# CMU-SAFARI/PyGim

Measured on AMD Instinct MI355X. Metric: SpMM GFLOP/s, Reddit-shaped CSR h=256 fp32, higher is better.
Workload: dtype f32

## Files before the change

### include/pygim_hip.h

```cpp
#ifndef PYGIM_HIP_H
#define PYGIM_HIP_H

#include <stdint.h>

#ifdef __cplusplus
extern "C" {
#endif

typedef enum {
    PYGIM_OK = 0,
    PYGIM_ERR_INVALID = 1,
    PYGIM_ERR_NO_DEVICE = 2,
    PYGIM_ERR_HIP = 3,
    PYGIM_ERR_UNSORTED = 4
} pygim_status;

typedef enum {
    PYGIM_INT8 = 0,
    PYGIM_INT16 = 1,
    PYGIM_INT32 = 2,
    PYGIM_INT64 = 3,
    PYGIM_FLT32 = 4,
    PYGIM_DBL64 = 5
} pygim_dtype;
// ... 3 lines not shown
int pygim_init_ranks(int64_t nr_ranks, int64_t *units_per_rank);
int pygim_init_units(int64_t nr_units, int64_t *units_per_rank, int64_t *nr_ranks_out);
int pygim_release(void);
int64_t pygim_generation(void);
int pygim_group_serial(int64_t handle, int64_t *out);
int pygim_is_initialized(void);
const char *pygim_last_error(void);
int pygim_device_info(char *name, int name_len, int *cu_count, int64_t *hbm_bytes);

int pygim_group_create(int format, int dtype, int n_parts,
                       const int32_t *const *idx0, const int32_t *const *colind,
                       const void *const *values, const int64_t *nrows, const int64_t *ncols,
                       const int64_t *nnz, const int64_t *n_dense, const int64_t *dense_cols,
                       int64_t h_size, int64_t *out_handle);
int pygim_group_free(int64_t handle);
int pygim_group_create_transposed(int format, int dtype, int n_parts,
                                  const int32_t *const *idx0, const int32_t *const *colind,
                                  const void *const *values, const int64_t *nrows, const int64_t *ncols,
                                  const int64_t *nnz, const int64_t *n_dense, const int64_t *dense_cols,
                                  int64_t h_size, int64_t *out_handle);

int pygim_spmm_run_group(int64_t handle, const void *const *B_parts, void *out, void *stream);
int pygim_spmm_run_group_x(int64_t handle, const void *const *B_parts, void *out, int x_unchanged,
                           void *stream);
int pygim_grande_run_group(int64_t handle, const void *const *B_windows, const int64_t *window_ld,
                           void *out, void *stream);
int pygim_spmv_run_group(int64_t handle, const void *const *B_vectors, void *out, void *stream);

int pygim_block_run(int64_t handle, int part, const void *X, int64_t ldx, void *C, int64_t ldc,
                    int64_t width, int accumulate, void *stream);
int pygim_block_run_x(int64_t handle, int part, const void *X, int64_t ldx, void *C, int64_t ldc,
                      int64_t width, int accumulate, int x_unchanged, void *stream);

int pygim_quant_spmm_run(int64_t handle, const float *X, int64_t ldx, float *out, float *scale_out, void *stream);
int pygim_quant_spmm_run_post(int64_t handle, const float *X, int64_t ldx, float *out, float *scale_out,
                              const float *col_mul, const float *col_add, int relu, void *stream);

int pygim_quant_absmax(const float *X, int64_t ldx, int64_t rows, int64_t width, uint32_t *absmax_bits, void *stream);
int pygim_quantize(int dtype, const float *X, int64_t ldx, int64_t rows, int64_t width, const uint32_t *absmax_bits,
                   void *Xq, float *scale_out, void *stream);
int pygim_dequantize(int dtype, const void *Q, int64_t n, const uint32_t *absmax_bits, float *out, void *stream);
int pygim_spmm_run_dequant(int64_t handle, const void *Xq, int64_t ldx, float *out, const uint32_t *absmax_bits, void *stream);

int pygim_sddmm(int dtype, int64_t nrows, const int32_t *rowptr, const int32_t *colind, int64_t nnz, const void *G,
                int64_t ldg, const void *X, int64_t ldx, int64_t h, void *out, void *stream);

int64_t pygim_spmm_values_workspace(int dtype, int64_t nrows, int64_t nnz, int64_t h, int64_t heads);
int pygim_spmm_values(int dtype, int64_t nrows, const int32_t *rowptr, const int32_t *colind, int64_t nnz, const void *values,
                      int64_t heads, const void *X, int64_t ldx, int64_t h, void *out, int64_t ldo, void *workspace,
                      int64_t workspace_bytes, void *stream);
int64_t pygim_edge_softmax_workspace(int dtype, int64_t nrows, int64_t nnz, int64_t heads);
int pygim_edge_softmax(int dtype, int64_t nrows, const int32_t *rowptr, int64_t nnz, const void *scores, int64_t heads, void *out,
                       void *workspace, int64_t workspace_bytes, void *stream);
int pygim_edge_softmax_backward(int dtype, int64_t nrows, const int32_t *rowptr, int64_t nnz, const void *P, const void *dP,
                                int64_t heads, void *out, void *workspace, int64_t workspace_bytes, void *stream);
int64_t pygim_gat_aggregate_workspace(int dtype, int64_t nrows, int64_t nnz, int64_t h, int64_t heads);
int pygim_gat_aggregate(int dtype, int64_t nrows, const int32_t *rowptr, const int32_t *colind, int64_t nnz,
                        const void *a_dst , const void *a_src , int64_t heads,
                        double negative_slope, const void *X, int64_t ldx, int64_t h, void *out, int64_t ldo,
                        void *lse , void *workspace, int64_t workspace_bytes, void *stream);

#define PYGIM_REDUCE_MEAN 1
#define PYGIM_REDUCE_MAX 2
#define PYGIM_REDUCE_MIN 3
int64_t pygim_spmm_reduce_workspace(int dtype, int op, int64_t nrows, int64_t nnz, int64_t h);
int pygim_spmm_reduce(int dtype, int op, int64_t nrows, const int32_t *rowptr, const int32_t *colind, int64_t nnz,
                      const void *values , const void *X, int64_t ldx, int64_t h, void *out, int64_t ldo,
                      int32_t *arg , void *workspace, int64_t workspace_bytes, void *stream);
int pygim_spmm_reduce_backward(int dtype, int64_t ncols, const int32_t *rowptr_t, const int32_t *rows_t, const int32_t *perm,
                               int64_t nnz, const void *values , const void *G, int64_t ldg,
                               const int32_t *arg, int64_t h, void *dX, int64_t ldd, void *stream);

int pygim_group_timers(int64_t handle, double out_ms[5]);
int pygim_group_info(int64_t handle, int64_t out[8]);
int pygim_group_kernel_ms(int64_t handle, double *sum_ms, int64_t *count, int reset);
int pygim_group_kernel_events(int64_t handle, int on);
int pygim_group_plan(int64_t handle, int64_t out[8]);
int pygim_group_lds_plan(int64_t handle, int64_t out[4]);
int pygim_group_lds_code(int64_t handle, int64_t out[4]);
int pygim_group_lds_tiles(int64_t handle, int64_t out[4]);
int pygim_group_lds_runs(int64_t handle, int64_t *out);
int pygim_group_host_windows(int64_t handle, int64_t *windows, int64_t *direct);
int pygim_group_lds_geometry(int64_t handle, int64_t out[8]);
int pygim_group_lds_note(int64_t handle, char *out, int64_t cap);
int64_t pygim_set_tunable(const char *name, int64_t value);

#ifdef __cplusplus
}
#endif
#endif
```

### pygim_amd/_lib.py

```python
import ctypes
import os

_HERE = os.path.dirname(os.path.abspath(__file__))
LIB_PATH = os.environ.get("PYGIM_HIP_LIB", os.path.join(_HERE, "libpygim_hip.so"))

EXPORTS = [
    "pygim_init_ranks", "pygim_init_units", "pygim_release", "pygim_is_initialized", "pygim_last_error",
    "pygim_device_info", "pygim_group_create", "pygim_group_free", "pygim_spmm_run_group",
    "pygim_grande_run_group", "pygim_spmv_run_group", "pygim_block_run", "pygim_group_timers",
    "pygim_group_info", "pygim_set_tunable", "pygim_group_kernel_ms", "pygim_quant_spmm_run",
    "pygim_quant_absmax", "pygim_quantize", "pygim_dequantize", "pygim_spmm_run_group_x", "pygim_block_run_x",
    "pygim_group_kernel_events", "pygim_group_plan", "pygim_spmm_run_dequant",
    "pygim_quant_spmm_run_post", "pygim_generation", "pygim_group_lds_plan", "pygim_group_lds_code", "pygim_group_lds_geometry", "pygim_group_lds_note",
    "pygim_group_lds_tiles", "pygim_group_lds_runs", "pygim_group_serial", "pygim_group_host_windows",
    "pygim_group_create_transposed", "pygim_sddmm",
    "pygim_spmm_values", "pygim_spmm_values_workspace", "pygim_edge_softmax", "pygim_edge_softmax_workspace", "pygim_edge_softmax_backward",
    "pygim_gat_aggregate", "pygim_gat_aggregate_workspace",
    "pygim_spmm_reduce", "pygim_spmm_reduce_workspace", "pygim_spmm_reduce_backward",
]

OK, ERR_INVALID, ERR_NO_DEVICE, ERR_HIP, ERR_UNSORTED = 0, 1, 2, 3, 4
INT8, INT16, INT32, INT64, FLT32, DBL64 = range(6)
CSR, COO = 0, 1
REDUCE_MEAN, REDUCE_MAX, REDUCE_MIN = 1, 2, 3


class PygimError(RuntimeError):
    def __init__(self, code, msg):
        super().__init__(f"pygim_hip error {code}: {msg}")
        self.code = code


_lib = None


def lib():
    global _lib
    if _lib is None:
        if not os.path.exists(LIB_PATH):
            raise ImportError(
                f"{LIB_PATH} not found: build the HIP extension first "
                f"(`make -C pygim_amd/csrc` or `python -c 'import __graft_entry__ as g; g.build()'`). "
                f"This backend has no CPU fallback.")
        import torch

        L = ctypes.CDLL(LIB_PATH)
        c_i64, c_int, vp = ctypes.c_int64, ctypes.c_int, ctypes.c_void_p
        p_i64 = ctypes.POINTER(ctypes.c_int64)
        L.pygim_last_error.restype = ctypes.c_char_p
        L.pygim_init_ranks.argtypes = [c_i64, p_i64]
        L.pygim_init_units.argtypes = [c_i64, p_i64, p_i64]
        L.pygim_device_info.argtypes = [ctypes.c_char_p, c_int, ctypes.POINTER(c_int), p_i64]
        L.pygim_group_create.argtypes = [c_int, c_int, c_int, vp, vp, vp, p_i64, p_i64, p_i64, p_i64, p_i64, c_i64,
                                         p_i64]
        L.pygim_group_create_transposed.argtypes = list(L.pygim_group_create.argtypes)
        L.pygim_sddmm.argtypes = [c_int, c_i64, vp, vp, c_i64, vp, c_i64, vp, c_i64, c_i64, vp, vp]
        L.pygim_spmm_values.argtypes = [c_int, c_i64, vp, vp, c_i64, vp, c_i64, vp, c_i64, c_i64, vp, c_i64, vp, c_i64, vp]
        L.pygim_spmm_values_workspace.argtypes = [c_int, c_i64, c_i64, c_i64, c_i64]
        L.pygim_spmm_values_workspace.restype = c_i64
        L.pygim_edge_softmax.argtypes = [c_int, c_i64, vp, c_i64, vp, c_i64, vp, vp, c_i64, vp]
        L.pygim_edge_softmax_backward.argtypes = [c_int, c_i64, vp, c_i64, vp, vp, c_i64, vp, vp, c_i64, vp]
        L.pygim_edge_softmax_workspace.argtypes = [c_int, c_i64, c_i64, c_i64]
        L.pygim_edge_softmax_workspace.restype = c_i64
        L.pygim_gat_aggregate.argtypes = [c_int, c_i64, vp, vp, c_i64, vp, vp, c_i64, ctypes.c_double, vp, c_i64, c_i64, vp, c_i64, vp, vp, c_i64, vp]
        L.pygim_gat_aggregate_workspace.argtypes = [c_int, c_i64, c_i64, c_i64, c_i64]
        L.pygim_gat_aggregate_workspace.restype = c_i64
        L.pygim_spmm_reduce.argtypes = [c_int, c_int, c_i64, vp, vp, c_i64, vp, vp, c_i64, c_i64, vp, c_i64, vp, vp, c_i64, vp]
        L.pygim_spmm_reduce_workspace.argtypes = [c_int, c_int, c_i64, c_i64, c_i64]
        L.pygim_spmm_reduce_workspace.restype = c_i64
        L.pygim_spmm_reduce_backward.argtypes = [c_int, c_i64, vp, vp, vp, c_i64, vp, vp, c_i64, vp, c_i64, vp, c_i64, vp]
        L.pygim_group_free.argtypes = [c_i64]
        L.pygim_group_serial.argtypes = [c_i64, p_i64]
        L.pygim_spmm_run_group.argtypes = [c_i64, vp, vp, vp]
        L.pygim_spmm_run_group_x.argtypes = [c_i64, vp, vp, c_int, vp]
        L.pygim_grande_run_group.argtypes = [c_i64, vp, p_i64, vp, vp]
        L.pygim_spmv_run_group.argtypes = [c_i64, vp, vp, vp]
        L.pygim_block_run.argtypes = [c_i64, c_int, vp, c_i64, vp, c_i64, c_i64, c_int, vp]
        L.pygim_block_run_x.argtypes = [c_i64, c_int, vp, c_i64, vp, c_i64, c_i64, c_int, c_int, vp]
        L.pygim_group_timers.argtypes = [c_i64, ctypes.POINTER(ctypes.c_double)]
        L.pygim_group_info.argtypes = [c_i64, p_i64]
        L.pygim_group_kernel_ms.argtypes = [c_i64, ctypes.POINTER(ctypes.c_double), p_i64, c_int]
        L.pygim_group_kernel_events.argtypes = [c_i64, c_int]
        L.pygim_group_plan.argtypes = [c_i64, p_i64]
        L.pygim_group_lds_plan.argtypes = [c_i64, p_i64]
        L.pygim_group_lds_code.argtypes = [c_i64, p_i64]
        L.pygim_group_lds_geometry.argtypes = [c_i64, p_i64]
        L.pygim_group_lds_note.argtypes = [c_i64, ctypes.c_char_p, c_i64]
        L.pygim_group_lds_tiles.argtypes = [c_i64, p_i64]
        L.pygim_group_lds_runs.argtypes = [c_i64, p_i64]
        L.pygim_group_host_windows.argtypes = [c_i64, p_i64, p_i64]
        L.pygim_generation.restype = c_i64
        L.pygim_quant_spmm_run.argtypes = [c_i64, vp, c_i64, vp, vp, vp]
        L.pygim_quant_spmm_run_post.argtypes = [c_i64, vp, c_i64, vp, vp, vp, vp, c_int, vp]
        L.pygim_quant_absmax.argtypes = [vp, c_i64, c_i64, c_i64, vp, vp]
        L.pygim_quantize.argtypes = [c_int, vp, c_i64, c_i64, c_i64, vp, vp, vp, vp]
        L.pygim_dequantize.argtypes = [c_int, vp, c_i64, vp, vp, vp]
        L.pygim_spmm_run_dequant.argtypes = [c_i64, vp, c_i64, vp, vp, vp]
        L.pygim_set_tunable.argtypes = [ctypes.c_char_p, c_i64]
        L.pygim_set_tunable.restype = c_i64
        _lib = L
    return _lib


def check(rc):
    if rc != 0:
        raise PygimError(rc, lib().pygim_last_error().decode())


def i64_array(values):
    return (ctypes.c_int64 * len(values))(*[int(v) for v in values])


def ptr_array(ptrs):
    return (ctypes.c_void_p * len(ptrs))(*[ctypes.c_void_p(int(p) if p else None) for p in ptrs])


def _env_tunables():
    for kv in filter(None, os.environ.get("PYGIM_TUNE", "").split(",")):
        name, _, value = kv.partition("=")
        if set_tunable(name.strip(), int(value)) == -1:
            raise ValueError(f"PYGIM_TUNE: unknown tunable {name!r}")


def init_ranks(nr_ranks, want_units=False):
    out = (ctypes.c_int64 * max(int(nr_ranks), 1))()
    check(lib().pygim_init_ranks(int(nr_ranks), out))
    _env_tunables()
    return list(out)[: int(nr_ranks)] if want_units else None


def init_units(nr_units):
    n = max((int(nr_units) + 7) // 8, 1)
    out = (ctypes.c_int64 * n)()
    ranks = ctypes.c_int64(0)
    check(lib().pygim_init_units(int(nr_units), out, ctypes.byref(ranks)))
    return list(out)[: ranks.value]


def release():
    check(lib().pygim_release())


def is_initialized():
    return bool(lib().pygim_is_initialized())


def device_info():
    name = ctypes.create_string_buffer(256)
    cu = ctypes.c_int(0)
    mem = ctypes.c_int64(0)
    check(lib().pygim_device_info(name, 256, ctypes.byref(cu), ctypes.byref(mem)))
    return name.value.decode(), cu.value, mem.value


def group_create(fmt, dtype, idx0_ptrs, col_ptrs, val_ptrs, nrows, ncols, nnz, n_dense, dense_cols, h):
    n = len(col_ptrs)
    handle = ctypes.c_int64(0)
    vals = None if val_ptrs is None else ptr_array(val_ptrs)
    check(lib().pygim_group_create(fmt, dtype, n, ptr_array(idx0_ptrs), ptr_array(col_ptrs), vals, i64_array(nrows),
                                   i64_array(ncols), i64_array(nnz), i64_array(n_dense), i64_array(dense_cols),
                                   int(h), ctypes.byref(handle)))
    return handle.value


def group_create_transposed(fmt, dtype, idx0_ptrs, col_ptrs, val_ptrs, nrows, ncols, nnz, n_dense, dense_cols, h):
    n = len(col_ptrs)
    handle = ctypes.c_int64(0)
    vals = None if val_ptrs is None else ptr_array(val_ptrs)
    check(lib().pygim_group_create_transposed(fmt, dtype, n, ptr_array(idx0_ptrs), ptr_array(col_ptrs), vals, i64_array(nrows),
# ... 71 lines not shown
    check(lib().pygim_spmm_reduce_backward(int(dtype), int(ncols), _vp(rowptr_t_ptr), _vp(rows_t_ptr), _vp(perm_ptr), int(nnz), _vp(val_ptr),
                                           _vp(g_ptr), int(ldg), _vp(arg_ptr), int(h), _vp(dx_ptr), int(ldd), _vp(stream)))


def group_free(handle):
    check(lib().pygim_group_free(int(handle)))


def spmm_run_group(handle, b_ptrs, out_ptr, stream=0, x_unchanged=False):
    check(lib().pygim_spmm_run_group_x(int(handle), ptr_array(b_ptrs), ctypes.c_void_p(out_ptr),
                                       1 if x_unchanged else 0, ctypes.c_void_p(stream or None)))


def grande_run_group(handle, b_ptrs, lds, out_ptr, stream=0):
    check(lib().pygim_grande_run_group(int(handle), ptr_array(b_ptrs), i64_array(lds), ctypes.c_void_p(out_ptr),
                                       ctypes.c_void_p(stream or None)))


def spmv_run_group(handle, b_ptrs, out_ptr, stream=0):
    check(lib().pygim_spmv_run_group(int(handle), ptr_array(b_ptrs), ctypes.c_void_p(out_ptr),
                                     ctypes.c_void_p(stream or None)))


def block_run(handle, part, x_ptr, ldx, c_ptr, ldc, width, accumulate=False, stream=0, x_unchanged=False):
    check(lib().pygim_block_run_x(int(handle), int(part), ctypes.c_void_p(x_ptr), int(ldx), ctypes.c_void_p(c_ptr),
                                  int(ldc), int(width), 1 if accumulate else 0, 1 if x_unchanged else 0,
                                  ctypes.c_void_p(stream or None)))


def group_timers(handle):
    out = (ctypes.c_double * 5)()
    check(lib().pygim_group_timers(int(handle), out))
    return list(out)


def group_kernel_events(handle, on=True):
    check(lib().pygim_group_kernel_events(int(handle), 1 if on else 0))


def group_plan(handle):
    out = (ctypes.c_int64 * 8)()
    check(lib().pygim_group_plan(int(handle), out))
    keys = ["n_panels", "panel_cols", "n_items", "col16", "n_coop_items", "n_segment_tasks", "merged", "has_extra"]
    return dict(zip(keys, [int(v) for v in out]))


def group_lds_plan(handle):
    out = (ctypes.c_int64 * 4)()
    check(lib().pygim_group_lds_plan(int(handle), out))
    return dict(zip(["tiles", "chunk_fills", "tokens", "nnz"], [int(v) for v in out]))


def group_lds_code(handle):
    out = (ctypes.c_int64 * 4)()
    check(lib().pygim_group_lds_code(int(handle), out))
    return dict(zip(["code_bytes", "paired_entries", "active", "device_generated"], [int(v) for v in out[:4]]))


def group_lds_tiles(handle):
    out = (ctypes.c_int64 * 4)()
    check(lib().pygim_group_lds_tiles(int(handle), out))
    return dict(zip(["similarity", "labels", "largest_label_rows", "sweep_locality"], [int(v) for v in out[:4]]))


def group_lds_runs(handle):
    out = ctypes.c_int64(0)
    check(lib().pygim_group_lds_runs(int(handle), ctypes.byref(out)))
    return int(out.value)


def group_host_windows(handle):
    return group_host_call(handle)["windows"]


def group_host_call(handle):
    w, d = ctypes.c_int64(0), ctypes.c_int64(0)
    check(lib().pygim_group_host_windows(int(handle), ctypes.byref(w), ctypes.byref(d)))
    return {"windows": int(w.value), "direct": int(d.value)}


def group_lds_geometry(handle):
    out = (ctypes.c_int64 * 8)()
    check(lib().pygim_group_lds_geometry(int(handle), out))
    return dict(zip(["waves", "acc_per_wave", "chunk_cols", "buffers", "group", "x_sets", "shared_entries", "col_splits"], [int(v) for v in out]))


def group_lds_note(handle):
    buf = ctypes.create_string_buffer(1024)
    check(lib().pygim_group_lds_note(int(handle), buf, 1024))
    return buf.value.decode()


def generation():
    return int(lib().pygim_generation())


def group_serial(handle):
    out = ctypes.c_int64(0)
    check(lib().pygim_group_serial(int(handle), ctypes.byref(out)))
    return int(out.value)


def group_info(handle):
    out = (ctypes.c_int64 * 8)()
    check(lib().pygim_group_info(int(handle), out))
    keys = ["total_rows", "total_cols", "h", "n_parts", "n_long_rows", "all_ones", "n_panels", "n_items"]
    return dict(zip(keys, list(out)))


def set_tunable(name, value):
    return int(lib().pygim_set_tunable(name.encode(), int(value)))


def group_kernel_ms(handle, reset=True):
    ms = ctypes.c_double(0)
    n = ctypes.c_int64(0)
    check(lib().pygim_group_kernel_ms(int(handle), ctypes.byref(ms), ctypes.byref(n), 1 if reset else 0))
    return ms.value, n.value


def quant_absmax(x_ptr, ldx, rows, width, bits_ptr, stream=0):
    check(lib().pygim_quant_absmax(ctypes.c_void_p(x_ptr or None), int(ldx), int(rows), int(width), ctypes.c_void_p(bits_ptr),
                                   ctypes.c_void_p(stream or None)))


def quantize(dtype, x_ptr, ldx, rows, width, bits_ptr, xq_ptr, scale_ptr=0, stream=0):
    check(lib().pygim_quantize(int(dtype), ctypes.c_void_p(x_ptr or None), int(ldx), int(rows), int(width),
                               ctypes.c_void_p(bits_ptr), ctypes.c_void_p(xq_ptr or None), ctypes.c_void_p(scale_ptr or None),
                               ctypes.c_void_p(stream or None)))


def dequantize(dtype, q_ptr, n, bits_ptr, out_ptr, stream=0):
    check(lib().pygim_dequantize(int(dtype), ctypes.c_void_p(q_ptr or None), int(n), ctypes.c_void_p(bits_ptr),
                                 ctypes.c_void_p(out_ptr or None), ctypes.c_void_p(stream or None)))


def spmm_run_dequant(handle, xq_ptr, ldx, out_ptr, bits_ptr, stream=0):
    check(lib().pygim_spmm_run_dequant(int(handle), ctypes.c_void_p(xq_ptr), int(ldx), ctypes.c_void_p(out_ptr),
                                       ctypes.c_void_p(bits_ptr), ctypes.c_void_p(stream or None)))


def quant_spmm_run(handle, x_ptr, ldx, out_ptr, scale_ptr=0, stream=0, col_mul_ptr=0, col_add_ptr=0, relu=False):
    check(lib().pygim_quant_spmm_run_post(int(handle), ctypes.c_void_p(x_ptr), int(ldx), ctypes.c_void_p(out_ptr),
                                          ctypes.c_void_p(scale_ptr or None), ctypes.c_void_p(col_mul_ptr or None),
                                          ctypes.c_void_p(col_add_ptr or None), 1 if relu else 0,
                                          ctypes.c_void_p(stream or None)))
```

### pygim_amd/autotune.py

```python
from __future__ import annotations

import math
from dataclasses import dataclass

RATE_PANEL = 17.0e12
RATE_GATHER_FAR = 4.8e12
RATE_GATHER_MALL = 7.0e12
RATE_STREAM = 5.0e12
XGMI_IN = 7 * 45e9
PANEL_BYTES = 4 << 20
LAUNCH = 6e-6
CUS = 256
LDS_ROWS_MAX = 8 * 228
LDS_NS_PER_COLUMN = 3.43
LDS_NS_PER_ENTRY = 0.26
LDS_NS_PER_ENTRY_HALF = 0.5
LDS_NS_PER_COLUMN_FLOOR = 4.4
LDS_COL_SPLIT = True
LDS_ROW_TAIL = 3
TAIL_S = 30e-6
LDS_MIN_LANES = 5
LDS_MIN_REUSE_NARROW = 0.75
LDS_HALF_SPLIT = True
LDS_MIN_REUSE = 0.75


@dataclass
class Choice:
    row_parts: int
    feat_parts: int
    seconds: float
    product_s: float
    collective_s: float
    panel: bool


def lds_rows_per_tile(nrows, nslices, rmax=LDS_ROWS_MAX, cus=CUS):
    tiles = -(-nrows // rmax)
    wgs = tiles * nslices
    rounds = -(-wgs // cus)
    if rounds > 8:
        return rmax
    if wgs % cus == 0:
        return -(-nrows // tiles)
    tiles2 = rounds * cus // nslices
    if tiles2 <= tiles:
        return rmax
    return min(rmax, max(16, -(-nrows // tiles2)))


def lds_product_seconds(nrows, ncols, nnz, h, es):
    if es != 4 or h < LDS_MIN_LANES or nrows == 0 or nnz == 0:
        return None
    nsl = -(-h // 64)
    pack_s = ncols * h * es * 2 / RATE_STREAM
    cols_x = ncols
    ns_entry = LDS_NS_PER_ENTRY
    if LDS_HALF_SPLIT and h * es <= 128 and ncols >= 4 * 128:
        cols_x = -(-ncols // 2)
        ns_entry = LDS_NS_PER_ENTRY_HALF
    min_reuse = LDS_MIN_REUSE if h * es > 128 else max(LDS_MIN_REUSE, LDS_MIN_REUSE_NARROW * (1.6 if cols_x != ncols else 1.0))
    tall = -(-int(nrows) // LDS_ROWS_MAX)
    split = min(8, CUS // (tall * nsl)) if tall * nsl * 2 <= CUS else 1
    tail_rows = 0
    if LDS_COL_SPLIT and nnz >= (1 << 20):
        for s2 in range(8, split, -1):
            tall_s = CUS // (nsl * s2)
            if not tall_s:
                continue
            covered = tall_s * LDS_ROWS_MAX
            if covered >= nrows:
                break
            if (nrows - covered) * 100 <= nrows * LDS_ROW_TAIL and tall_s * nsl * s2 * 10 >= CUS * 9:
                split, tall, tail_rows = s2, tall_s, nrows - covered
                break
    if LDS_COL_SPLIT and nnz >= (1 << 20) and split > 1:
        if nnz / (tall * cols_x) < min_reuse:
            return None
        tall2 = CUS // (nsl * split)
        if not tail_rows and tall < tall2 <= 2 * tall:
            tall = tall2
        per_wg = max(cols_x / split * LDS_NS_PER_COLUMN + nnz / tall / split * ns_entry, cols_x / split * LDS_NS_PER_COLUMN_FLOOR) * 1e-9
        reduce_s = (split + 1) * nrows * h * es / RATE_STREAM
        return per_wg + reduce_s + pack_s + 2 * LAUNCH + (TAIL_S if tail_rows else 0.0)
    rpt = lds_rows_per_tile(int(nrows), nsl)
    tiles = -(-int(nrows) // rpt)
    if nnz / (tiles * cols_x) < min_reuse:
        return None
    per_wg = max(cols_x * LDS_NS_PER_COLUMN + nnz / tiles * ns_entry, cols_x * LDS_NS_PER_COLUMN_FLOOR) * 1e-9
    rounds = -(-tiles * nsl // CUS)
    return rounds * per_wg + pack_s + LAUNCH


def product_seconds(nrows, ncols, nnz, h, es):
    if nrows == 0 or nnz == 0 or h == 0:
        return 0.0, False
    t_lds = lds_product_seconds(nrows, ncols, nnz, h, es)
    if t_lds is not None:
        return t_lds, True
    row_bytes = h * es
    line_bytes = max(row_bytes, 128) if row_bytes < 128 else row_bytes
    gather = nnz * line_bytes
    npanels = max(1, math.ceil(ncols * 128 / PANEL_BYTES))
    panel = row_bytes >= 64 and (npanels == 1 or nnz / (nrows * npanels) >= 8)
    if panel:
        nsl = math.ceil(row_bytes / 128)
        t = gather / RATE_PANEL + npanels * (2 * nrows * row_bytes) / RATE_STREAM / 8 + nsl * 4 * nnz / RATE_STREAM / 8
        t += npanels * LAUNCH + ncols * row_bytes * 2 / RATE_STREAM
    else:
        x_bytes = ncols * row_bytes
        rate = RATE_GATHER_MALL if x_bytes <= 300e6 else RATE_GATHER_FAR
        t = gather / rate + LAUNCH
    return t, panel


def price(nrows, ncols, nnz, h, es, row_parts, feat_parts):
    hp = math.ceil(h / feat_parts)
    t, panel = product_seconds(math.ceil(nrows / row_parts), ncols, nnz / row_parts, hp, es)
    gpus = row_parts * feat_parts
    coll = 0.0 if gpus == 1 else (nrows * h * es) * (1 - 1 / gpus) / XGMI_IN
    return Choice(row_parts, feat_parts, t + coll, t, coll, panel)


def choose(nrows, ncols, nnz, h, elem_bytes, n_gpus):
    table = []
    for r in range(1, n_gpus + 1):
        if n_gpus % r:
            continue
        f = n_gpus // r
        if f > h:
            continue
        table.append(price(nrows, ncols, nnz, h, elem_bytes, r, f))
    best = min(table, key=lambda c: c.seconds)
    return best, table


def autotune(nrows, ncols, nnz, hidden_size, elem_bytes=4, n_gpus=8):
    best, _ = choose(nrows, ncols, nnz, hidden_size, elem_bytes, n_gpus)
    return [best.row_parts, best.feat_parts, "nnz", "nnz", None]


def autotune_dataset(datadir, dataset, hidden_size, split_set, blnc_set=(0, 2), elem_bytes=4):
    from . import datasets, synth

    assert len(split_set) > 0 and len(blnc_set) > 0
    got = datasets.load_adjacency(datadir, dataset)
    if got is not None:
        nrows, nnz = int(got[2]), int(len(got[1]))
    else:
        nrows, nnz, _ = synth.DATASETS[dataset]
    best = None
    for sp, ds in split_set:
        if sp < 1 or ds < 1 or ds > hidden_size:
            continue
        c = price(nrows, nrows, nnz, hidden_size, elem_bytes, sp, ds)
        if best is None or c.seconds < best.seconds:
            best = c
    if best is None:
        return [None, None, None, None, None]
    return [best.row_parts, best.feat_parts, "nnz", "nnz", None]
```

### pygim_amd/csrc/kernels.hpp

```cpp
#pragma once
#include <hip/hip_runtime.h>
#include <stdint.h>
#include <type_traits>

namespace pygim {

template <typename T> struct AccOf { using type = T; };
template <> struct AccOf<int8_t> { using type = uint32_t; };
template <> struct AccOf<int16_t> { using type = uint32_t; };
template <> struct AccOf<int32_t> { using type = uint32_t; };
template <> struct AccOf<int64_t> { using type = uint64_t; };

template <typename T> __device__ __forceinline__ typename AccOf<T>::type to_acc(T v) {
    using A = typename AccOf<T>::type;
    if constexpr (std::is_floating_point<T>::value) return v;
    else if constexpr (sizeof(T) == 8) return (A)v;
    else return (A)(int32_t)v;
}
template <typename T> __device__ __forceinline__ T from_acc(typename AccOf<T>::type a) {
    if constexpr (std::is_floating_point<T>::value) return a;
    else return (T)a;
}

__device__ __forceinline__ uint32_t rfl(uint32_t v) { return __builtin_amdgcn_readfirstlane(v); }
// ... 721 lines not shown
    const uint32_t f = (uint32_t)(i % w);
    using A = typename AccOf<T>::type;
    A acc = (A)part[r * ldp + f];
    for (uint32_t c = 1; c < splits; c++) acc = (A)(acc + (A)part[((uint64_t)c * nrows + r) * ldp + f]);
    float y = (float)(T)acc * (1.0f * quant_scale(*absmax_bits, log2_range));
    if (post_mul) {
        y = post_mul[f] * y + post_add[f];
        if (post_relu) y = fmaxf(y, 0.0f);
    }
    out[r * ldo + f] = y;
}

template <typename T, bool DEQ>
__global__ void k_lds_reduce_v4(const T *__restrict__ part, uint32_t splits, uint64_t nrows, uint32_t w, uint64_t ldp, void *__restrict__ C, int64_t ldc, int accumulate,
                                const uint32_t *__restrict__ absmax_bits, int log2_range, const float *__restrict__ post_mul, const float *__restrict__ post_add, int post_relu) {
    static_assert(sizeof(T) == 4, "4-byte element types");
    using A = typename AccOf<T>::type;
    const uint32_t w4 = w >> 2;
    const uint64_t i = (uint64_t)blockIdx.x * blockDim.x + threadIdx.x;
    if (i >= nrows * w4) return;
    const uint64_t r = i / w4;
    const uint32_t f = (uint32_t)(i % w4) * 4;
    T v[4];
    load_vec<T, 4>(part + r * ldp + f, v);
    A acc[4];
#pragma unroll
    for (int k = 0; k < 4; k++) acc[k] = to_acc<T>(v[k]);
    for (uint32_t c = 1; c < splits; c++) {
        load_vec<T, 4>(part + ((uint64_t)c * nrows + r) * ldp + f, v);
#pragma unroll
        for (int k = 0; k < 4; k++) acc[k] = (A)(acc[k] + to_acc<T>(v[k]));
    }
    if constexpr (DEQ) {
        const float scale = 1.0f * quant_scale(*absmax_bits, log2_range);
        float y[4];
#pragma unroll
        for (int k = 0; k < 4; k++) {
            y[k] = (float)from_acc<T>(acc[k]) * scale;
            if (post_mul) {
                y[k] = post_mul[f + k] * y[k] + post_add[f + k];
                if (post_relu) y[k] = fmaxf(y[k], 0.0f);
            }
        }
        store_vec<float, 4>((float *)C + r * ldc + f, y);
    } else {
        T *c = (T *)C + r * ldc + f;
        if (accumulate) {
            load_vec<T, 4>(c, v);
#pragma unroll
            for (int k = 0; k < 4; k++) acc[k] = (A)(to_acc<T>(v[k]) + acc[k]);
        }
#pragma unroll
        for (int k = 0; k < 4; k++) v[k] = from_acc<T>(acc[k]);
        store_vec<T, 4>(c, v);
    }
}

template <int MODE>
__global__ void k_lds_reduce16(const int16_t *__restrict__ part, uint32_t splits, uint64_t nrows, uint32_t w, uint64_t ldp, void *__restrict__ C, int64_t ldc, int accumulate,
                               const uint32_t *__restrict__ absmax_bits, int log2_range, const float *__restrict__ post_mul, const float *__restrict__ post_add, int post_relu) {
    const uint64_t i = (uint64_t)blockIdx.x * blockDim.x + threadIdx.x;
    if (i >= nrows * w) return;
    const uint64_t r = i / w;
    const uint32_t f = (uint32_t)(i % w);
    uint32_t acc = (uint32_t)(int32_t)part[r * ldp + f];
    for (uint32_t c = 1; c < splits; c++) acc += (uint32_t)(int32_t)part[((uint64_t)c * nrows + r) * ldp + f];
    if constexpr (MODE == 0) {
        int8_t *c8 = (int8_t *)C + (int64_t)r * ldc + f;
        if (accumulate) acc += (uint32_t)(int32_t)*c8;
        *c8 = (int8_t)acc;
    } else {
        float y = (float)(MODE == 1 ? (int32_t)(int8_t)acc : (int32_t)(int16_t)acc) * (1.0f * quant_scale(*absmax_bits, log2_range));
        if (post_mul) {
            y = post_mul[f] * y + post_add[f];
            if (post_relu) y = fmaxf(y, 0.0f);
        }
        ((float *)C)[(int64_t)r * ldc + f] = y;
    }
}

constexpr uint32_t LDS_TAIL_SEG = 256;
template <typename T>
__global__ __launch_bounds__(512) void k_lds_tail_seg(const uint32_t *__restrict__ segs, uint32_t nseg, const uint32_t *__restrict__ colind, const char *__restrict__ xs,
                                                      uint64_t slice_stride, typename AccOf<T>::type *__restrict__ parked) {
    static_assert(sizeof(T) == 4, "4-byte element types");
    using A = typename AccOf<T>::type;
    __shared__ A partial[8][64];
    const uint32_t seg = blockIdx.x, slice = blockIdx.y;
    const uint32_t wave = threadIdx.x >> 6, lane = threadIdx.x & 63;
    const uint32_t e0 = segs[nseg + seg], e1 = segs[2 * nseg + seg];
    const char *xsl = xs + (uint64_t)slice * slice_stride + lane * 4;
    static_assert(LDS_TAIL_SEG == 256, "32 entries per wave");
    uint32_t cols[32];
#pragma unroll
    for (int k = 0; k < 32; k++) {
        const uint32_t e = e0 + wave + 8u * k;
        cols[k] = e < e1 ? colind[e] : 0xFFFFFFFFu;
    }
    T x[32];
#pragma unroll
    for (int k = 0; k < 32; k++) x[k] = cols[k] != 0xFFFFFFFFu ? *(const T *)(xsl + (uint64_t)cols[k] * 256) : (T)0;
    A acc = 0;
#pragma unroll
    for (int k = 0; k < 32; k++) acc = (A)(acc + to_acc<T>(x[k]));
    partial[wave][lane] = acc;
    __syncthreads();
    if (wave != 0) return;
    A sum = partial[0][lane];
#pragma unroll
    for (int v = 1; v < 8; v++) sum = (A)(sum + partial[v][lane]);
    parked[((uint64_t)seg * gridDim.y + slice) * 64 + lane] = sum;
}
template <typename T, bool DEQ>
__global__ __launch_bounds__(64) void k_lds_tail_fin(const uint32_t *__restrict__ rowseg, uint32_t row0, const typename AccOf<T>::type *__restrict__ parked, uint32_t w_lanes,
                                                     void *__restrict__ C, int64_t ldc_bytes, int accumulate, const uint32_t *__restrict__ absmax_bits, int log2_range,
                                                     const float *__restrict__ post_mul, const float *__restrict__ post_add, int post_relu) {
    using A = typename AccOf<T>::type;
    const uint32_t t = blockIdx.x, slice = blockIdx.y, lane = threadIdx.x;
    const uint32_t f = slice * 64 + lane;
    if (f >= w_lanes) return;
    A sum = 0;
    for (uint32_t s = rowseg[t]; s < rowseg[t + 1]; s++) sum = (A)(sum + parked[((uint64_t)s * gridDim.y + slice) * 64 + lane]);
    const uint64_t row = (uint64_t)row0 + t;
    if constexpr (DEQ) {
        float y = (float)from_acc<T>(sum) * (1.0f * quant_scale(*absmax_bits, log2_range));
        if (post_mul) {
            y = post_mul[f] * y + post_add[f];
            if (post_relu) y = fmaxf(y, 0.0f);
        }
        *(float *)((char *)C + (int64_t)row * ldc_bytes + (size_t)f * 4) = y;
    } else {
        T *c = (T *)((char *)C + (int64_t)row * ldc_bytes + (size_t)f * 4);
        if (accumulate) sum = (A)(to_acc<T>(*c) + sum);
        *c = from_acc<T>(sum);
    }
}

__global__ void k_copy16(const u32x4_t *__restrict__ src, u32x4_t *__restrict__ dst, uint64_t n) {
    const uint64_t i = (uint64_t)blockIdx.x * blockDim.x + threadIdx.x;
    if (i < n) dst[i] = src[i];
}

template <typename T>
__global__ void k_narrow_vals(const T *__restrict__ vals, uint64_t n, typename NarrowOf<T>::type *__restrict__ narrow, int *flag) {
    using NT = typename NarrowOf<T>::type;
    const uint64_t i = (uint64_t)blockIdx.x * blockDim.x + threadIdx.x;
    if (i >= n) return;
    const T v = vals[i];
    const NT q = (NT)v;
    bool same;
    if constexpr (std::is_same<T, double>::value) same = __double_as_longlong((double)q) == __double_as_longlong(v);
    else same = (T)q == v;
    narrow[i] = q;
    if (!same) atomicOr(flag, 1);
}

template <typename T>
__global__ void k_widen_vals(const T *__restrict__ vals, uint64_t n, uint32_t *__restrict__ wide) {
    const uint64_t i = (uint64_t)blockIdx.x * blockDim.x + threadIdx.x;
    if (i < n) wide[i] = (uint32_t)(int32_t)vals[i];
}

template <typename T, int VEC, int LOG_LPR, int AMODE, int HAS_VALS, bool DEQ = false>
__global__ __launch_bounds__(256) void k_csr_panel(const uint32_t *__restrict__ item_row,
                                                   const uint32_t *__restrict__ item_begin,
                                                   const uint32_t *__restrict__ item_len, uint32_t nitems,
                                                   const uint32_t *__restrict__ coop_row,
                                                   const uint32_t *__restrict__ coop_begin,
                                                   const uint32_t *__restrict__ coop_len, uint32_t ncoop,
                                                   uint32_t coop_grid, const uint32_t *__restrict__ colind,
                                                   const T *__restrict__ vals, const T *__restrict__ X,
                                                   int64_t ldx, int64_t slice_stride, T *__restrict__ C,
                                                   int64_t ldc, uint32_t w, uint32_t nslices, int accumulate,
                                                   uint32_t col_base, float *__restrict__ Cf, int64_t ldcf,
                                                   const uint32_t *__restrict__ absmax_bits, int log2_range,
                                                   const float *__restrict__ post_mul, const float *__restrict__ post_add,
                                                   int post_relu) {
    static_assert(LOG_LPR == 3, "lane groups of 8 (one 128-byte line per gathered row slice)");
    if (blockIdx.x < coop_grid)
        panel_sweep<T, VEC, AMODE, HAS_VALS, true, DEQ>(blockIdx.x, coop_row, coop_begin, coop_len, ncoop, colind, vals, X,
                                                        ldx, slice_stride, C, ldc, w, nslices, accumulate, col_base, Cf, ldcf,
                                                        absmax_bits, log2_range, post_mul, post_add, post_relu);
    else
        panel_sweep<T, VEC, AMODE, HAS_VALS, false, DEQ>(blockIdx.x - coop_grid, item_row, item_begin, item_len, nitems,
// ... 675 lines not shown
```

### pygim_amd/csrc/lds_codegen.hpp

```cpp
#pragma once
#include <stdint.h>

#include <algorithm>
#include <stdexcept>
#include <vector>

#include "lds_plan.hpp"

#if defined(__HIPCC__)
#define PYGIM_HD __host__ __device__
#else
#define PYGIM_HD
#endif

namespace pygim {

struct CgParams {
    uint32_t NW = 8, KA = 228, KC = 128, NBUF = 5, RB = 256, RPB = 256, G = 10, NS = 2, XW = 1;
    uint32_t wide = 0, valued = 0;
    uint32_t mulw = 0;
    uint32_t int_inline = 0;
    uint32_t i64_full = 0;
    uint32_t opcode_add = 0x02000000u, addw = 1;
    uint32_t pieces = 4, chunk_bytes = 32768;
    uint32_t nrows = 0, ncols = 0, nchunks = 0, ntiles = 0, nstreams = 0;
    uint32_t S = 1, row_tiles = 0;
    uint32_t col_bits = 1;
    uint32_t half_H = 0;
    uint32_t x0 = 6, acc0 = 28, vbase0 = 1, vbase1 = 2, vbase2 = 3, vl16 = 4, vtouch = 4, vjunk = 5;
    uint32_t s_xs = 80, s_ldsw = 82, s_cb = 84, s_ret = 86, s_pa = 92;
    PYGIM_HD uint32_t vbase(uint32_t blk) const { return blk == 0 ? vbase0 : blk == 1 ? vbase1 : vbase2; }
};

constexpr uint32_t CG_TOUCH_EVERY_DW = 256;

inline CgParams cg_params(const LdsGeometry &geo, uint32_t opcode_add, bool valued, uint32_t nrows, uint32_t ncols, uint32_t gsize = 0, uint32_t nsets = 0,
                          bool int_inline = false, bool i64_full = false, uint32_t half_H = 0) {
    if (geo.NBUF >= 3 && !geo.boundary) throw std::runtime_error("lds codegen: the mid-slot hand-off takes the host encoder");
    CgParams P;
    const bool wide = geo.row_bytes == 512;
    if (geo.row_bytes != 256 && geo.row_bytes != 512) throw std::runtime_error("lds codegen: rows of 256 or 512 bytes");
    if (wide != (opcode_add == LDS_CODE_ADD_F64 || opcode_add == LDS_CODE_ADD_U64)) throw std::runtime_error("lds codegen: 512-byte rows are the 8-byte element types'");
    const LdsCodeRegs R = lds_code_regs(geo.NW, gsize, nsets, wide);
    P.NW = geo.NW; P.KA = geo.KA; P.KC = geo.KC; P.NBUF = geo.NBUF; P.RB = geo.row_bytes; P.RPB = 65536 / geo.row_bytes;
    P.G = R.gsize; P.NS = R.nsets; P.XW = wide ? 2 : 1; P.wide = wide; P.valued = valued;
    if (R.x0 + R.nx() > R.acc0 || R.acc0 + P.KA * P.XW > 256 || P.G > 12 || (P.NS - 1) * P.G > 15 || P.NS > 8)
        throw std::runtime_error("lds codegen: the geometry does not fit the register map");
    if (P.KA > 255) throw std::runtime_error("lds codegen: more than 255 accumulators per wave");
    P.opcode_add = opcode_add;
    P.i64_full = (valued && opcode_add == LDS_CODE_ADD_U64 && i64_full) ? 1 : 0;
    P.int_inline = (valued && (opcode_add == 0x68000000u || opcode_add == LDS_CODE_ADD_U64 || opcode_add == LDS_CODE_PK_ADD_U16) && int_inline && !P.i64_full) ? 1 : 0;
    P.mulw = !valued ? 0 : opcode_add == LDS_CODE_ADD_F64 ? 6 : opcode_add == LDS_CODE_ADD_U64 ? (P.i64_full ? 12 : P.int_inline ? 6 : 8) : ((opcode_add == 0x68000000u || opcode_add == LDS_CODE_PK_ADD_U16) && !int_inline) ? 4 : 2;
    P.addw = (opcode_add == LDS_CODE_PK_ADD_U16 || opcode_add == LDS_CODE_ADD_F64 || opcode_add == LDS_CODE_ADD_U64) ? 2 : 1;
    if (valued && opcode_add == LDS_CODE_ADD_U64) P.addw = 0;
    P.pieces = (geo.KC * geo.row_bytes / 1024) / geo.NW;
    if (P.pieces * geo.NW * 1024 != geo.KC * geo.row_bytes) throw std::runtime_error("lds codegen: a chunk is not a whole number of pieces per wave");
    P.chunk_bytes = geo.KC * geo.row_bytes;
    if ((geo.KC * geo.NBUF + P.RPB - 1) / P.RPB > 3) throw std::runtime_error("lds codegen: the ring is larger than three 64 KiB blocks");
    if (geo.NBUF > 12) throw std::runtime_error("lds codegen: more than 12 ring buffers");
    if ((geo.half_split != 0) != (half_H != 0)) throw std::runtime_error("lds codegen: a half-split plan names its H (and only such a plan does)");
    if (half_H && (valued || wide || half_H % geo.KC || ncols != half_H)) throw std::runtime_error("lds codegen: half-split plans are unit-weight plans of 4-byte types over H = whole chunks of virtual columns");
    P.half_H = half_H;
    P.nrows = nrows; P.ncols = ncols;
    P.nchunks = (ncols + geo.KC - 1) / geo.KC;
    const uint32_t R_rows = geo.rows_per_tile ? std::min(geo.rows_per_tile, geo.NW * geo.KA) : geo.NW * geo.KA;
    P.S = std::max(1u, geo.col_splits);
    P.row_tiles = (nrows + R_rows - 1) / R_rows;
    P.ntiles = P.row_tiles * P.S;
    P.nstreams = P.ntiles * geo.NW;
    if ((uint64_t)nrows * P.S >= (1ull << 32)) throw std::runtime_error("lds codegen: rows x column ranges beyond 32 bits");
    P.col_bits = 1;
    while (P.col_bits < 32 && (1ull << P.col_bits) < (uint64_t)ncols) P.col_bits++;
    uint32_t sb = 1;
    while ((1ull << sb) < (uint64_t)P.nstreams) sb++;
    if (sb + P.col_bits + 8 > 64) throw std::runtime_error("lds codegen: key wider than 64 bits");
    P.x0 = R.x0; P.acc0 = R.acc0; P.vbase0 = R.vbase[0]; P.vbase1 = R.vbase[1]; P.vbase2 = R.vbase[2];
    P.vl16 = R.vl16; P.vtouch = R.vtouch; P.vjunk = R.vjunk;
    P.s_xs = R.s_xs; P.s_ldsw = R.s_ldsw; P.s_cb = R.s_cb; P.s_ret = R.s_ret; P.s_pa = R.s_pa;
    return P;
}
inline uint32_t cg_key_bits(const CgParams &P) {
    uint32_t sb = 1;
    while ((1ull << sb) < (uint64_t)P.nstreams) sb++;
    return sb + P.col_bits + 8;
}

struct CgRows {
    std::vector<uint32_t> rowinfo;
    std::vector<uint32_t> rowmap_rt;
    std::vector<uint32_t> tnnz;
    std::vector<uint32_t> tile_pos;
    std::vector<uint32_t> rowmap;
    std::vector<uint32_t> tile_row0, tile_nnz;
};
inline void cg_deal_rows_a(const uint32_t *rowptr, const LdsGeometry &geo, const CgParams &P, CgRows &out, const uint32_t *rorder = nullptr) {
    auto rid = [&](uint32_t pos) { return rorder ? rorder[pos] : pos; };
    auto rlen = [&](uint32_t pos) { const uint32_t r = rid(pos); return rowptr[r + 1] - rowptr[r]; };
    const uint32_t NW = geo.NW, KA = geo.KA, KAS = geo.ka_stride(), RS = NW * KAS;
    const uint32_t R = geo.rows_per_tile ? std::min(geo.rows_per_tile, NW * KA) : NW * KA;
    const uint32_t nrows = P.nrows, nrt = P.row_tiles;
    out.rowinfo.assign(nrows, 0);
    out.rowmap_rt.assign((size_t)nrt * RS, 0xFFFFFFFFu);
    out.tnnz.assign((size_t)nrt * P.S, 0);
    lds_parallel_for(nrt, 0, [&](uint32_t rt) {
        std::vector<uint32_t> order;
        const uint32_t r0 = rt * R, r1 = std::min(nrows, r0 + R), nr = r1 - r0;
        if (P.S == 1) {
            if (!rorder) out.tnnz[rt] = rowptr[r1] - rowptr[r0];
            else
                for (uint32_t q = r0; q < r1; q++) out.tnnz[rt] += rlen(q);
        }
        order.resize(nr);
        for (uint32_t i = 0; i < nr; i++) order[i] = i;
        std::stable_sort(order.begin(), order.end(), [&](uint32_t a, uint32_t b) { return rlen(r0 + a) > rlen(r0 + b); });
        for (uint32_t i = 0; i < nr; i++) {
            const uint32_t round = i / NW, p = i % NW;
            const uint32_t w = (round & 1) ? NW - 1 - p : p;
            out.rowinfo[rid(r0 + order[i])] = ((rt * NW + w) << 8) | round;
            out.rowmap_rt[((size_t)rt * NW + w) * KAS + round] = rid(r0 + order[i]);
        }
    });
}
inline void cg_deal_rows_b(const LdsGeometry &geo, const CgParams &P, CgRows &out) {
    const uint32_t NW = geo.NW, KAS = geo.ka_stride(), RS = NW * KAS;
    const uint32_t R = geo.rows_per_tile ? std::min(geo.rows_per_tile, NW * geo.KA) : NW * geo.KA;
    const uint32_t ntiles = P.ntiles;
    std::vector<uint32_t> ord(ntiles);
    for (uint32_t t = 0; t < ntiles; t++) ord[t] = t;
    if (!geo.keep_tile_order) std::stable_sort(ord.begin(), ord.end(), [&](uint32_t a, uint32_t b) { return out.tnnz[a] > out.tnnz[b]; });
    out.tile_pos.assign(ntiles, 0);
    for (uint32_t i = 0; i < ntiles; i++) out.tile_pos[ord[i]] = i;
    out.rowmap.assign((size_t)ntiles * RS, 0xFFFFFFFFu);
    out.tile_row0.assign(ntiles, 0);
    out.tile_nnz.assign(ntiles, 0);
    for (uint32_t t = 0; t < ntiles; t++) {
        const uint32_t rt = t / P.S, cs = t % P.S, ti = out.tile_pos[t];
        out.tile_row0[ti] = rt * R;
        out.tile_nnz[ti] = out.tnnz[t];
        for (uint32_t q = 0; q < RS; q++) {
            const uint32_t r = out.rowmap_rt[(size_t)rt * RS + q];
            if (r != 0xFFFFFFFFu) out.rowmap[(size_t)ti * RS + q] = r + cs * P.nrows;
        }
    }
}

// ... 124 lines not shown
    }
    const uint32_t ch = T.chunks[T.choff[s / P.NW] + j];
    const uint64_t target = ((uint64_t)s << (P.col_bits + 8)) | ((uint64_t)ch * P.KC << 8);
    uint64_t lo = 0, hi = T.nnz;
    while (lo < hi) {
        const uint64_t mid = (lo + hi) >> 1;
        if (T.keys[mid] < target) lo = mid + 1;
        else hi = mid;
    }
    T.slot_firstcol[sj] = lo < T.nnz ? T.colx[lo] : T.ncols_total;
}
PYGIM_HD inline void cg_slot_ngroups(const CgParams &P, const CgTables &T, uint32_t sj) {
    const uint32_t m = T.slot_firstcol[sj + 1] - T.slot_firstcol[sj];
    T.slot_ng[sj] = (m + P.G - 1) / P.G;
}
PYGIM_HD inline unsigned long long cg_slot_groups(const CgParams &P, const CgTables &T, uint32_t sj) {
    const uint32_t c0 = T.slot_firstcol[sj], c1 = T.slot_firstcol[sj + 1];
    uint32_t g = T.slot_firstgroup[sj];
    unsigned long long pairs = 0;
    for (uint32_t c = c0; c < c1; c += P.G, g++) {
        const uint32_t ce = c + P.G < c1 ? c + P.G : c1;
        uint32_t nlds = 0;
        for (uint32_t u = 0; c + u < ce; u++) {
            T.col_g[c + u] = (g << 4) | u;
            if (P.wide) { nlds++; continue; }
            if ((u & 1) == 0) {
                const bool paired = c + u + 1 < c1 && (T.col_lrow[c + u + 1] / P.RPB) == (T.col_lrow[c + u] / P.RPB);
                if (paired) {
                    nlds++;
                    pairs += (unsigned long long)(T.col_first[c + u + 2] - T.col_first[c + u]);
                } else {
                    nlds += (c + u + 1 < ce) ? 2 : 1;
                }
            }
        }
        T.g_first[g] = T.col_first[c];
        T.g_nent[g] = T.col_first[ce] - T.col_first[c];
        if (P.half_H) {
            uint32_t n0 = 0;
            for (uint32_t i = T.col_first[c]; i < T.col_first[ce]; i++) n0 += T.vals[i] == 0u;
            T.g_n0[g] = n0;
        }
        T.g_firstcol[g] = c;
        T.g_nlds[g] = (uint8_t)nlds;
        T.g_ncols[g] = (uint8_t)(ce - c);
    }
    return pairs;
}

struct CgEmit {
    uint32_t *out;
    uint64_t n;
    uint32_t since_touch;
    uint64_t vm_touch;
    PYGIM_HD void put(uint32_t a) {
        if (out) out[n] = a;
        n++;
    }
    PYGIM_HD void op(uint32_t a) { put(a); since_touch++; }
    PYGIM_HD void op(uint32_t a, uint32_t b) { put(a); put(b); since_touch += 2; }
    PYGIM_HD void skip(uint32_t dw) { n += dw; since_touch += dw; }
};

PYGIM_HD inline void cg_stream_pass(const CgParams &P, const CgTables &T, uint32_t s, bool write) {
    const uint32_t ti = s / P.NW;
    const uint32_t nch = T.nch[ti];
    const uint32_t *chunk_ids = T.chunks + T.choff[ti];
    const uint32_t sj0 = cg_sbase(P, T, s);
    CgEmit e;
    const uint64_t base_dw = write ? T.start[s] / 4 : 0;
    e.out = write ? T.code + base_dw : nullptr;
    e.n = 0;
    e.since_touch = 0;
    e.vm_touch = 0;
    auto s_add_lit = [&](uint32_t sdst, uint32_t ssrc, uint32_t lit) { e.op(0x80000000u | (sdst << 16) | (0xFFu << 8) | ssrc, lit); };
    auto s_addc0 = [&](uint32_t sdst, uint32_t ssrc) { e.op(0x82000000u | (sdst << 16) | (0x80u << 8) | ssrc); };
    auto touch = [&]() {
        s_add_lit(P.s_cb, P.s_cb, (e.since_touch + 5) * 4);
        s_addc0(P.s_cb + 1, P.s_cb + 1);
        e.op(0xDC508000u, (P.vjunk << 24) | (P.s_cb << 16) | P.vtouch);
        e.since_touch = 0;
        e.vm_touch++;
    };
    auto dma = [&](uint32_t cid, uint32_t buf) {
        s_add_lit(P.s_pa, P.s_xs, cid * P.chunk_bytes);
        s_addc0(P.s_pa + 1, P.s_xs + 1);
        for (uint32_t i = 0; i < P.pieces; i++) {
            if (i % 4 == 0) {
                if (i) {
                    s_add_lit(P.s_pa, P.s_pa, 0x1000);
                    s_addc0(P.s_pa + 1, P.s_pa + 1);
                }
                s_add_lit(124 , P.s_ldsw, buf * P.chunk_bytes + (i / 4) * 0x1000);
                e.op(0xBF800000u);
            }
            e.op(0xDDF48000u | ((i % 4) * 1024), (P.s_pa << 16) | P.vl16);
        }
    };
    uint64_t dma_issued = 0;
    uint64_t landed_mark[16];
    for (int q = 0; q < 16; q++) landed_mark[q] = 0;
    auto vm_now = [&]() { return dma_issued + e.vm_touch; };
    auto dma_chunk = [&](uint32_t j) {
        dma(chunk_ids[j], j % P.NBUF);
        dma_issued += P.pieces;
        landed_mark[j & 15] = vm_now();
    };
    auto wait_landed = [&](uint32_t j) {
        const uint64_t younger = vm_now() - landed_mark[j & 15];
        const uint32_t nn = (uint32_t)(younger < 63 ? younger : 63);
        e.op(0xBF8C0F70u | (nn & 15) | (((nn >> 4) & 3) << 14));
    };
    auto wait_lgkm = [&](uint32_t n) { e.op(0xBF8CC07Fu | ((n < 15u ? n : 15u) << 8)); };
    uint32_t pend_g[10], pend_nlds[10], npend = 0;
    uint32_t gcount = 0;
    auto consume_oldest = [&]() {
        uint32_t younger = 0;
        for (uint32_t q = 1; q < npend; q++) younger += pend_nlds[q];
        wait_lgkm(younger);
        const uint32_t g = pend_g[0];
        if (write) T.g_apos[g] = (uint32_t)(base_dw + e.n);
        e.skip(T.g_nent[g] * (P.mulw + P.addw));
        if (P.half_H) e.skip((T.g_n0[g] > 0 ? 1u : 0u) + (T.g_n0[g] < T.g_nent[g] ? 1u : 0u) + 1u);
        for (uint32_t q = 1; q < npend; q++) {
            pend_g[q - 1] = pend_g[q];
            pend_nlds[q - 1] = pend_nlds[q];
        }
        npend--;
    };
    if (nch) {
        for (uint32_t j = 0; j + 1 < P.NBUF && j < nch; j++) dma_chunk(j);
        wait_landed(0);
        e.op(0xBF8A0000u);
    }
    for (uint32_t j = 0; j < nch; j++) {
        bool dma_due = j + P.NBUF - 1 < nch;
        const uint32_t g0 = T.slot_firstgroup[sj0 + j], g1 = T.slot_firstgroup[sj0 + j + 1];
        for (uint32_t g = g0; g < g1; g++) {
            const uint32_t nlds = T.g_nlds[g];
            if (write) {
                T.g_rpos[g] = (uint32_t)(base_dw + e.n);
                T.g_xset[g] = (uint8_t)(gcount % P.NS);
            }
            e.skip(2 * nlds);
            pend_g[npend] = g;
            pend_nlds[npend] = nlds;
            npend++;
            gcount++;
            if (dma_due) {
                dma_chunk(j + P.NBUF - 1);
                dma_due = false;
            }
            if (npend >= P.NS) consume_oldest();
            if (e.since_touch >= CG_TOUCH_EVERY_DW) touch();
        }
        if (dma_due) dma_chunk(j + P.NBUF - 1);
        while (npend > 1) consume_oldest();
        wait_lgkm(0);
        if (j + 1 < nch) wait_landed(j + 1);
        e.op(0xBF8A0000u);
    }
    while (npend) consume_oldest();
    e.op(0xBF8C0F70u);
    e.op(0xBE801D00u | P.s_ret);
    while (e.n % 64) e.put(0xBF800000u);
    if (!write) T.stream_dw[s] = (uint32_t)e.n;
}

PYGIM_HD inline void cg_emit_reads(const CgParams &P, const CgTables &T, uint32_t g) {
    if (P.half_H) {
        uint32_t *a = T.code + T.g_apos[g];
        const uint32_t n0 = T.g_n0[g], n1 = T.g_nent[g] - n0;
        uint32_t at = 0;
        if (n0) { a[at] = 0xBEFE0100u | 76u; at += 1 + n0 * P.addw; }
        if (n1) { a[at] = 0xBEFE0100u | 78u; at += 1 + n1 * P.addw; }
        a[at] = 0xBEFE01C1u;
    }
    const uint32_t c0 = T.g_firstcol[g], nc = T.g_ncols[g];
    const uint32_t xb = P.x0 + P.G * P.XW * T.g_xset[g];
    uint32_t *w = T.code + T.g_rpos[g];
    for (uint32_t u = 0; u < nc;) {
        const uint32_t r0 = T.col_lrow[c0 + u], blk = r0 / P.RPB;
        if (P.wide) {
            *w++ = 0xD8EC0000u | ((r0 % P.RPB) * P.RB);
            *w++ = ((xb + u * 2) << 24) | P.vbase(blk);
            u++;
        } else if ((u & 1) == 0 && u + 1 < nc && (T.col_lrow[c0 + u + 1] / P.RPB) == blk) {
            const uint32_t r1 = T.col_lrow[c0 + u + 1];
// ... 196 lines not shown
```

### pygim_amd/csrc/lds_plan.hpp

```cpp
#pragma once
#include <stdint.h>
#if defined(__HIPCC__)
#define PYGIM_LDS_HD_INLINE __host__ __device__ inline
#else
#define PYGIM_LDS_HD_INLINE inline
#endif

#include <algorithm>
#include <atomic>
#include <cstdio>
#include <cstdlib>
#include <memory>
#include <stdexcept>
#include <thread>
#include <vector>

namespace pygim {

struct LdsTile {
    uint32_t nch;
    uint32_t chunk_off;
    uint32_t nb_off;
    uint32_t row0;
    uint32_t nnz;
    uint32_t chunk0;
    uint32_t pad[2];
    uint32_t tokstart[16];
};

constexpr uint32_t LDS_TOK_SLACK = 4096 + 64;

constexpr uint32_t LDS_HDR_SHIFT = 18, LDS_HDR_MAX = 0x3FFFu;

struct LdsGeometry {
    uint32_t NW = 8;
    uint32_t KA = 208;
    uint32_t KC = 320;
    uint32_t BATCH = 16;
    uint32_t rows_per_tile = 0;
    uint32_t keep_tile_order = 0;
    uint32_t col_splits = 1;
    uint32_t ka_stride() const { return (KA + 7) & ~7u; }
    uint32_t row_bytes = 256;
    uint32_t boundary = 0;
    uint32_t half_split = 0;
    uint32_t NBUF = 2;
};

struct LdsPlanHost {
    LdsGeometry geo;
    uint32_t ntiles = 0, nchunks = 0;
    uint64_t ntokens = 0;
    uint64_t slots = 0;
    std::vector<uint32_t> tok;
    std::vector<uint32_t> wts;
    std::vector<uint32_t> nb, chunks, rowmap;
    std::vector<LdsTile> tiles;
    std::atomic<bool> header_overflow{false};
};

inline unsigned lds_default_threads() {
    static const unsigned cached = [] {
        unsigned hw = std::max(1u, std::thread::hardware_concurrency());
        long long quota = -1, period = 100000;
        if (FILE *f = fopen("/sys/fs/cgroup/cpu.max", "r")) {
            char q[32] = {0};
            if (fscanf(f, "%31s %lld", q, &period) == 2 && q[0] != 'm') quota = atoll(q);
            fclose(f);
        } else if (FILE *g = fopen("/sys/fs/cgroup/cpu/cpu.cfs_quota_us", "r")) {
            if (fscanf(g, "%lld", &quota) != 1) quota = -1;
            fclose(g);
            if (FILE *h = fopen("/sys/fs/cgroup/cpu/cpu.cfs_period_us", "r")) {
                if (fscanf(h, "%lld", &period) != 1) period = 100000;
                fclose(h);
            }
        }
        if (quota > 0 && period > 0) hw = (unsigned)std::min<long long>(hw, std::max<long long>(1, (quota + period - 1) / period));
        return hw;
    }();
    return cached;
}

template <typename F> inline void lds_parallel_for(uint32_t n, unsigned threads, F &&fn) {
    if (threads == 0) threads = lds_default_threads();
    threads = std::min<unsigned>(threads, std::max(1u, n));
    std::atomic<uint32_t> next(0);
    std::atomic<bool> failed(false);
    auto body = [&]() {
        try {
            for (;;) {
                const uint32_t i = next.fetch_add(1);
                if (i >= n || failed.load(std::memory_order_relaxed)) return;
                fn(i);
            }
        } catch (...) {
            failed.store(true);
        }
    };
    std::vector<std::thread> pool;
    try {
        for (unsigned i = 1; i < threads; i++) pool.emplace_back(body);
    } catch (...) {
    }
    body();
    for (auto &th : pool) th.join();
    if (failed.load()) throw std::runtime_error("lds plan: a worker failed (out of memory?)");
}

inline void lds_plan_build(const uint32_t *rowptr, const uint32_t *col, uint32_t nrows, uint32_t ncols, const LdsGeometry &geo,
                           LdsPlanHost &out, unsigned threads = 0, const uint32_t *vals = nullptr, const uint32_t *rorder = nullptr) {
    auto rid = [&](uint32_t pos) { return rorder ? rorder[pos] : pos; };
    auto rlen = [&](uint32_t pos) { const uint32_t r = rid(pos); return rowptr[r + 1] - rowptr[r]; };
    const uint32_t NW = geo.NW, KA = geo.KA, KC = geo.KC, B = geo.BATCH;
    const uint32_t KAS = geo.ka_stride();
    const uint32_t RS = NW * KAS;
    const uint32_t R = geo.rows_per_tile ? std::min(geo.rows_per_tile, NW * KA) : NW * KA;
    const uint32_t S = std::max(1u, geo.col_splits);
    const uint32_t ntiles = ((nrows + R - 1) / R) * S;
    const uint32_t nchunks = (ncols + KC - 1) / KC;
    out.geo = geo;
    out.ntiles = ntiles;
    out.nchunks = nchunks;
    out.tiles.assign(ntiles, LdsTile());
    out.rowmap.assign((size_t)ntiles * RS, 0xFFFFFFFFu);

    struct TileTmp {
        std::vector<uint32_t> chunk_ids;
        std::vector<uint32_t> cnt;
        std::vector<uint8_t> wave_of;
        std::vector<uint16_t> k_of;
        uint64_t batches[16] = {0, 0, 0, 0, 0, 0, 0, 0, 0, 0, 0, 0, 0, 0, 0, 0};
    };
    std::vector<TileTmp> tmp(ntiles);
    auto run = [&](auto &&fn) { lds_parallel_for(ntiles, threads, fn); };
    run([&](uint32_t t) {
        TileTmp &tt = tmp[t];
        const uint32_t rt = t / S, cs = t % S;
        const uint32_t ch_lo = (uint32_t)((uint64_t)nchunks * cs / S), ch_hi = (uint32_t)((uint64_t)nchunks * (cs + 1) / S);
        const uint32_t r0 = rt * R, r1 = std::min(nrows, r0 + R), nr = r1 - r0;
        std::vector<uint32_t> order(nr);
        for (uint32_t i = 0; i < nr; i++) order[i] = i;
        std::stable_sort(order.begin(), order.end(), [&](uint32_t a, uint32_t b) {
            return rlen(r0 + a) > rlen(r0 + b);
        });
        tt.wave_of.resize(nr);
        tt.k_of.resize(nr);
        for (uint32_t i = 0; i < nr; i++) {
            const uint32_t round = i / NW, pos = i % NW;
            const uint32_t w = (round & 1) ? NW - 1 - pos : pos;
            tt.wave_of[order[i]] = (uint8_t)w;
            tt.k_of[order[i]] = (uint16_t)round;
            out.rowmap[((size_t)t * NW + w) * KAS + round] = rid(r0 + order[i]) + cs * nrows;
        }
        std::vector<uint32_t> cnt((size_t)nchunks * NW, 0);
        for (uint32_t i = 0; i < nr; i++) {
            const uint32_t w = tt.wave_of[i];
            for (uint32_t e = rowptr[rid(r0 + i)]; e < rowptr[rid(r0 + i) + 1]; e++) {
                const uint32_t ch = col[e] / KC;
                if (ch >= ch_lo && ch < ch_hi) cnt[(size_t)ch * NW + w]++;
            }
        }
        uint32_t nnz_range = 0;
        for (uint32_t c = 0; c < nchunks; c++) {
            uint32_t any = 0;
            for (uint32_t w = 0; w < NW; w++) any |= cnt[(size_t)c * NW + w];
            if (!any) continue;
            tt.chunk_ids.push_back(c);
            for (uint32_t w = 0; w < NW; w++) {
                const uint32_t n = cnt[(size_t)c * NW + w];
                nnz_range += n;
                tt.cnt.push_back(n);
                tt.batches[w] += std::max<uint32_t>(1, (n + B - 1) / B);
            }
        }
        out.tiles[t].nch = (uint32_t)tt.chunk_ids.size();
        out.tiles[t].chunk0 = tt.chunk_ids.empty() ? 0 : tt.chunk_ids[0];
        out.tiles[t].row0 = r0;
        out.tiles[t].nnz = nnz_range;
    });
    uint64_t tokb = 0, nbo = 0, cho = 0, slots = 0;
    for (uint32_t t = 0; t < ntiles; t++) {
        LdsTile &d = out.tiles[t];
        d.chunk_off = (uint32_t)cho;
        d.nb_off = (uint32_t)nbo;
        cho += d.nch + 2;
        nbo += (uint64_t)(d.nch + 2) * NW;
        slots += d.nch;
        for (uint32_t w = 0; w < NW; w++) {
            d.tokstart[w] = (uint32_t)tokb;
            tokb += tmp[t].batches[w];
        }
    }
    out.slots = slots;
    out.ntokens = tokb * B;
    out.tok.assign((size_t)out.ntokens + LDS_TOK_SLACK, KA);
    if (vals) out.wts.assign(out.tok.size(), 0u);
    else out.wts.clear();
    out.nb.assign((size_t)nbo + 256, 0);
    out.chunks.assign((size_t)cho + 128, 0);
    run([&](uint32_t t) {
        TileTmp &tt = tmp[t];
        const LdsTile &d = out.tiles[t];
        const uint32_t rt = t / S, cs = t % S;
        const uint32_t r0 = rt * R, r1 = std::min(nrows, r0 + R), nr = r1 - r0, nch = d.nch;
        for (uint32_t j = 0; j < nch + 2; j++) out.chunks[(size_t)d.chunk_off + j] = nch ? tt.chunk_ids[std::min(j, nch - 1)] : 0;
// ... 3 lines not shown
        for (uint32_t w = 0; w < NW; w++) {
            uint64_t at = (uint64_t)d.tokstart[w] * B;
            for (uint32_t j = 0; j < nch; j++) {
                cursor[(size_t)j * NW + w] = at;
                const uint32_t nbat = std::max<uint32_t>(1, (tt.cnt[(size_t)j * NW + w] + B - 1) / B);
                out.nb[(size_t)d.nb_off + (size_t)j * NW + w] = nbat;
                at += (uint64_t)nbat * B;
            }
        }
        auto batches_of = [&](uint32_t j, uint32_t w) { return j < nch ? std::max<uint32_t>(1, (tt.cnt[(size_t)j * NW + w] + B - 1) / B) : 0u; };
        for (uint32_t k = 0; k < KA; k++)
            for (uint32_t w = 0; w < NW; w++) {
                const uint32_t rowm = out.rowmap[((size_t)t * NW + w) * KAS + k];
                if (rowm == 0xFFFFFFFFu) continue;
                const uint32_t row = rowm - cs * nrows;
                for (uint32_t e = rowptr[row]; e < rowptr[row + 1]; e++) {
                    const uint32_t c = col[e];
                    const uint32_t j = slot_of[c / KC];
                    if (j == 0xFFFFFFFFu) continue;
                    const uint64_t at = cursor[(size_t)j * NW + w]++;
                    out.tok[at] = (((c % KC) + (j % geo.NBUF) * KC) << 8) | k;
                    if (vals) out.wts[at] = vals[e];
                }
            }
        for (uint32_t w = 0; w < NW; w++) {
            uint64_t at = (uint64_t)d.tokstart[w] * B;
            for (uint32_t j = 0; j < nch; j++) {
                const uint32_t nbj = batches_of(j, w), nbn = batches_of(j + 1, w), cidn = j + 1 < nch ? tt.chunk_ids[j + 1] : 0;
                if (nbj > LDS_HDR_MAX || nbn > LDS_HDR_MAX || cidn > LDS_HDR_MAX) out.header_overflow = true;
                out.tok[at] |= nbj << LDS_HDR_SHIFT;
                out.tok[at + 1] |= nbn << LDS_HDR_SHIFT;
                out.tok[at + 2] |= cidn << LDS_HDR_SHIFT;
                at += (uint64_t)nbj * B;
            }
        }
        (void)nr;
    });
    std::vector<uint32_t> ord(ntiles);
    for (uint32_t t = 0; t < ntiles; t++) ord[t] = t;
    if (!geo.keep_tile_order) std::stable_sort(ord.begin(), ord.end(), [&](uint32_t a, uint32_t b) { return out.tiles[a].nnz > out.tiles[b].nnz; });
    std::vector<LdsTile> tiles2(ntiles);
    std::vector<uint32_t> rowmap2(out.rowmap.size());
    for (uint32_t i = 0; i < ntiles; i++) {
        tiles2[i] = out.tiles[ord[i]];
        std::copy(out.rowmap.begin() + (size_t)ord[i] * RS, out.rowmap.begin() + (size_t)(ord[i] + 1) * RS, rowmap2.begin() + (size_t)i * RS);
    }
    out.tiles.swap(tiles2);
    out.rowmap.swap(rowmap2);
}

inline uint32_t lds_rows_per_tile(uint32_t nrows, uint32_t rmax, uint32_t nslices, uint32_t cus) {
    if (!nrows || !nslices || !cus) return rmax;
    const uint64_t tiles = (nrows + rmax - 1) / rmax, wgs = tiles * nslices;
    const uint64_t rounds = (wgs + cus - 1) / cus;
    if (rounds > 8) return rmax;
    if (wgs % cus == 0) return (uint32_t)((nrows + tiles - 1) / tiles);
    const uint64_t tiles2 = rounds * cus / nslices;
    if (tiles2 <= tiles) return rmax;
    return (uint32_t)std::min<uint64_t>(rmax, std::max<uint64_t>(16, (nrows + tiles2 - 1) / tiles2));
}

inline double lds_plan_uniform_reuse(uint64_t nnz, uint32_t nrows, uint32_t ncols, const LdsGeometry &geo) {
    const uint64_t R = geo.rows_per_tile ? geo.rows_per_tile : (uint64_t)geo.NW * geo.KA;
    const uint64_t ntiles = (nrows + R - 1) / R;
    if (!ntiles || !ncols) return 0;
    return (double)nnz / ((double)ntiles * (double)ncols);
}


struct LdsCodeRegs {
    uint32_t vbase[3] = {0, 0, 0};
    uint32_t vl16 = 0;
    uint32_t vtouch = 0;
    uint32_t vjunk = 0;
    uint32_t x0 = 0;
    uint32_t gsize = 0, nsets = 0;
    uint32_t acc0 = 0;
    uint32_t s_xs = 80;
    uint32_t s_ldsw = 82;
    uint32_t s_cb = 84;
    uint32_t s_ret = 86;
    uint32_t s_pa = 92;
    uint32_t wide = 0;
    constexpr uint32_t nx() const { return gsize * nsets * (wide ? 2 : 1); }
};
constexpr LdsCodeRegs lds_code_regs(uint32_t NW, uint32_t gsize = 0, uint32_t nsets = 0, bool wide = false) {
    LdsCodeRegs r;
    r.wide = wide ? 1 : 0;
    if (NW == 16) {
        r.vbase[0] = 4; r.vbase[1] = 5; r.vbase[2] = 10;
        r.vl16 = 6; r.vtouch = 11; r.vjunk = 9; r.x0 = 12; r.acc0 = 28;
        r.gsize = gsize ? gsize : 8;
        r.nsets = nsets ? nsets : 2;
    } else {
        r.vbase[0] = 1; r.vbase[1] = 2; r.vbase[2] = 3;
        r.vl16 = 4; r.vtouch = 4; r.vjunk = 5; r.x0 = 6; r.acc0 = 28;
        r.gsize = gsize ? gsize : (wide ? 5 : 10);
        r.nsets = nsets ? nsets : 2;
    }
    if (!wide && (r.gsize & 1)) r.gsize--;
    if (r.gsize < 2) r.gsize = 2;
    if (r.nsets < 2) r.nsets = 2;
    while (r.x0 + r.nx() > r.acc0 && r.gsize > 2) r.gsize -= wide ? 1 : 2;
    return r;
}
constexpr uint32_t LDS_CODE_AUTO_WAVES = 8, LDS_CODE8_AUTO_NBUF = 5;
constexpr uint32_t LDS_CODE8_KA64 = 114;
constexpr uint32_t LDS_CODE8_KA = 228;

struct LdsWords {
    std::unique_ptr<uint32_t[]> p;
    size_t n = 0;
    void alloc(size_t words) { p.reset(new uint32_t[words]); n = words; }
    uint32_t *data() { return p.get(); }
    const uint32_t *data() const { return p.get(); }
    size_t size() const { return n; }
    uint32_t &operator[](size_t i) { return p[i]; }
    const uint32_t &operator[](size_t i) const { return p[i]; }
};

struct LdsCodeHost {
    LdsWords code;
    std::vector<uint64_t> start;
    uint64_t entries = 0;
    uint64_t pairs = 0;
    uint64_t shared = 0;
    LdsCodeRegs regs;
};

constexpr uint32_t LDS_CODE_PK_ADD_U16 = 0xFFFFFFFFu;
constexpr uint32_t LDS_CODE_ADD_F64 = 0xFFFFFFFEu, LDS_CODE_ADD_U64 = 0xFFFFFFFDu;
constexpr uint32_t LDS_CODE_S_VAL = 94;
inline bool lds_int_values_inline(const uint32_t *vals, uint64_t n) {
    for (uint64_t i = 0; i < n; i++) {
        const int32_t v = (int32_t)vals[i];
        if (v < -16 || v > 64) return false;
    }
    return true;
}
PYGIM_LDS_HD_INLINE uint32_t lds_inline_int(int32_t v) { return v >= 0 ? 128u + (uint32_t)v : 192u + (uint32_t)(-v); }
inline void lds_code_from_plan(const LdsPlanHost &plan, uint32_t opcode_add, LdsCodeHost &out, unsigned threads = 0, uint32_t gsize = 0,
                               uint32_t nsets = 0, uint32_t experiment = 0, const uint64_t *vals64 = nullptr) {
    const LdsGeometry &geo = plan.geo;
    const uint32_t NW = geo.NW, KA = geo.KA, B = geo.BATCH, KC = geo.KC;
    const uint32_t RB = geo.row_bytes;
    const bool wide = RB == 512;
    if (RB != 256 && RB != 512) throw std::runtime_error("lds code: rows of 256 or 512 bytes");
    if (wide != (opcode_add == LDS_CODE_ADD_F64 || opcode_add == LDS_CODE_ADD_U64)) throw std::runtime_error("lds code: 512-byte rows are the 8-byte element types'");
    if (!plan.wts.empty() && (opcode_add == LDS_CODE_ADD_F64 || opcode_add == LDS_CODE_ADD_U64) && !vals64)
        throw std::runtime_error("lds code: valued entries of this element type");
    const LdsCodeRegs R = lds_code_regs(NW, gsize, nsets, wide);
    out.regs = R;
    const uint32_t G = R.gsize, NS = R.nsets;
    if (R.x0 + R.nx() > R.acc0 || R.acc0 + KA * (wide ? 2 : 1) > 256 || G > 12 || (NS - 1) * G > 15)
        throw std::runtime_error("lds code: the geometry does not fit the register map");
    const uint32_t pieces = (KC * RB / 1024) / NW;
    if (pieces * NW * 1024 != KC * RB) throw std::runtime_error("lds code: a chunk is not a whole number of pieces per wave");
    const uint32_t chunk_bytes = KC * RB;
    const uint32_t RPB = 65536 / RB;
    if ((KC * geo.NBUF + RPB - 1) / RPB > 3) throw std::runtime_error("lds code: the ring is larger than three 64 KiB blocks");
    const uint32_t ntiles = plan.ntiles;
    constexpr uint32_t TOUCH_EVERY_DW = 256;

    struct Emit {
        uint32_t *out = nullptr;
        size_t n = 0;
        uint32_t since_touch = 0;
        uint64_t vm_touch = 0;
        void put(uint32_t a) {
            if (out) out[n] = a;
            n++;
        }
        void op(uint32_t a) { put(a); since_touch++; }
        void op(uint32_t a, uint32_t b) { put(a); put(b); since_touch += 2; }
    };
    struct Grp {
        uint32_t nx = 0, nlds = 0, xb = 0;
        std::vector<uint32_t> k, xr, v;
    };
    const LdsCodeRegs Rr = R;
    bool int_inline = (opcode_add == 0x68000000u || opcode_add == LDS_CODE_PK_ADD_U16) && !plan.wts.empty() && lds_int_values_inline(plan.wts.data(), plan.wts.size());
    bool i64_full = false;
    if (opcode_add == LDS_CODE_ADD_U64 && !plan.wts.empty()) {
        int_inline = true;
        for (uint64_t i = 0; i < plan.ntokens; i++) {
            if ((plan.tok[i] & 0xFF) >= KA) continue;
            const int64_t v = (int64_t)vals64[plan.wts[i]];
            if (v != (int64_t)(int32_t)v) i64_full = true;
            if (v < -16 || v > 64) int_inline = false;
        }
        if (i64_full) int_inline = false;
    }
    auto emit_stream = [&](uint32_t ti, uint32_t wv, Emit &e, uint64_t &n_entries, uint64_t &n_pairs, uint64_t &n_shared) {
        const LdsTile &t = plan.tiles[ti];
        auto s_add_lit = [&](uint32_t sdst, uint32_t ssrc, uint32_t lit) { e.op(0x80000000u | (sdst << 16) | (0xFFu << 8) | ssrc, lit); };
        auto s_addc0 = [&](uint32_t sdst, uint32_t ssrc) { e.op(0x82000000u | (sdst << 16) | (0x80u << 8) | ssrc); };
        auto touch = [&]() {
            s_add_lit(Rr.s_cb, Rr.s_cb, (e.since_touch + 5) * 4);
            s_addc0(Rr.s_cb + 1, Rr.s_cb + 1);
            e.op(0xDC508000u, (Rr.vjunk << 24) | (Rr.s_cb << 16) | Rr.vtouch);
            e.since_touch = 0;
            e.vm_touch++;
        };
        auto dma = [&](uint32_t cid, uint32_t buf) {
            s_add_lit(Rr.s_pa, Rr.s_xs, cid * chunk_bytes);
            s_addc0(Rr.s_pa + 1, Rr.s_xs + 1);
            for (uint32_t i = 0; i < pieces; i++) {
                if (i % 4 == 0) {
                    if (i) {
                        s_add_lit(Rr.s_pa, Rr.s_pa, 0x1000);
                        s_addc0(Rr.s_pa + 1, Rr.s_pa + 1);
                    }
                    s_add_lit(124 , Rr.s_ldsw, buf * chunk_bytes + (i / 4) * 0x1000);
                    e.op(0xBF800000u);
                }
                if (!(experiment & 2)) e.op(0xDDF48000u | ((i % 4) * 1024), (Rr.s_pa << 16) | Rr.vl16);
            }
        };
        uint64_t at = (uint64_t)t.tokstart[wv] * B;
        const uint32_t NBUF = geo.NBUF;
        const bool mid = NBUF >= 3 && !geo.boundary;
        uint64_t dma_issued = 0;
        auto vm_now = [&]() { return dma_issued + e.vm_touch; };
        std::vector<uint64_t> landed_mark(t.nch + NBUF + 1, 0);
        auto dma_chunk = [&](uint32_t j) {
            dma(plan.chunks[t.chunk_off + j], j % NBUF);
            dma_issued += (experiment & 2) ? 0 : pieces;
            landed_mark[j] = vm_now();
        };
        const bool spread = (experiment & 4) && pieces <= 4 && !mid;
        uint32_t dma_left = 0, dma_j = 0;
        auto dma_begin = [&](uint32_t j) {
            const uint32_t cid = plan.chunks[t.chunk_off + j], buf = j % NBUF;
            s_add_lit(Rr.s_pa, Rr.s_xs, cid * chunk_bytes);
            s_addc0(Rr.s_pa + 1, Rr.s_xs + 1);
            s_add_lit(124 , Rr.s_ldsw, buf * chunk_bytes);
            e.op(0xBF800000u);
            dma_left = pieces;
            dma_j = j;
        };
        auto dma_piece = [&]() {
            const uint32_t i = pieces - dma_left;
            e.op(0xDDF48000u | (i * 1024), (Rr.s_pa << 16) | Rr.vl16);
            dma_issued++;
            if (!--dma_left) landed_mark[dma_j] = vm_now();
        };
        auto wait_landed = [&](uint32_t j) {
            const uint64_t younger = vm_now() - landed_mark[j];
            const uint32_t nn = (uint32_t)std::min<uint64_t>(younger, 63);
            e.op(0xBF8C0F70u | (nn & 15) | (((nn >> 4) & 3) << 14));
        };
        auto wait_lgkm = [&](uint32_t n) { e.op(0xBF8CC07Fu | (std::min(n, 15u) << 8)); };
        const bool halves = geo.half_split != 0;
        const bool valued = !plan.wts.empty() && !halves;
        std::vector<Grp> ring(NS + 1);
        std::vector<uint32_t> pend;
        uint32_t gcount = 0;
        uint32_t lds_this_slot = 0;
        bool older_reads = false;
        auto consume_oldest = [&]() {
            uint32_t younger = 0;
            for (size_t q = 1; q < pend.size(); q++) younger += ring[pend[q]].nlds;
            wait_lgkm(younger);
            if (younger <= lds_this_slot) older_reads = false;
            const Grp &g = ring[pend.front()];
            if (valued && opcode_add == LDS_CODE_ADD_U64) {
                for (size_t q = 0; q < g.k.size(); q++) {
                    const uint64_t v64 = vals64[g.v[q]];
                    const int32_t v = (int32_t)(uint32_t)v64;
                    const uint32_t xl = g.xr[q], xh = g.xr[q] + 1, al = Rr.acc0 + g.k[q] * 2, ah = al + 1;
                    const uint32_t src = int_inline ? lds_inline_int(v) : LDS_CODE_S_VAL;
                    if (!int_inline) e.op(0xBE8000FFu | (LDS_CODE_S_VAL << 16), (uint32_t)v);
                    if (i64_full) e.op(0xBE8000FFu | ((LDS_CODE_S_VAL + 1) << 16), (uint32_t)(v64 >> 32));
                    e.op(0xD2850000u | xh, src | ((256 + xh) << 9));
                    if (!i64_full) e.op(v < 0 ? (0x6A000000u | (xh << 17) | (xl << 9) | (256 + xh)) : 0xBF800000u);
                    e.op(0x68000000u | (ah << 17) | (ah << 9) | (256 + xh));
                    if (i64_full) {
                        e.op(0xD2850000u | xh, (LDS_CODE_S_VAL + 1) | ((256 + xl) << 9));
                        e.op(0x68000000u | (ah << 17) | (ah << 9) | (256 + xh));
                    }
                    e.op(0xD1E86A00u | al, src | ((256 + xl) << 9) | ((256 + al) << 18));
                }
            } else if (valued && opcode_add == LDS_CODE_ADD_F64) {
                for (size_t q = 0; q < g.k.size(); q++) {
                    const uint64_t v = vals64[g.v[q]];
                    e.op(0xBE8000FFu | (LDS_CODE_S_VAL << 16), (uint32_t)v);
                    e.op(0xBE8000FFu | ((LDS_CODE_S_VAL + 1) << 16), (uint32_t)(v >> 32));
                    e.op(0xD2810000u | g.xr[q], LDS_CODE_S_VAL | ((256 + g.xr[q]) << 9));
                }
            } else if (valued && opcode_add == LDS_CODE_PK_ADD_U16) {
                for (size_t q = 0; q < g.k.size(); q++) {
                    if (!int_inline) e.op(0xBE8000FFu | (LDS_CODE_S_VAL << 16), g.v[q]);
                    e.op(0xD3814000u | g.xr[q], 0x10000000u | ((256 + g.xr[q]) << 9) | (int_inline ? lds_inline_int((int32_t)g.v[q]) : LDS_CODE_S_VAL));
                }
            } else if (valued && opcode_add == 0x68000000u) {
                for (size_t q = 0; q < g.k.size(); q++) {
                    if (int_inline) e.op(0xD2850000u | g.xr[q], lds_inline_int((int32_t)g.v[q]) | ((256 + g.xr[q]) << 9));
                    else {
                        e.op(0xBE8000FFu | (LDS_CODE_S_VAL << 16), g.v[q]);
                        e.op(0xD2850000u | g.xr[q], LDS_CODE_S_VAL | ((256 + g.xr[q]) << 9));
                    }
                }
            } else if (valued)
                for (size_t q = 0; q < g.k.size(); q++) e.op(0x0A0000FFu | (g.xr[q] << 17) | (g.xr[q] << 9), g.v[q]);
            for (uint32_t pass = 0; pass < (halves ? 2u : 1u); pass++) {
            if (halves) {
                bool any = false;
                for (size_t q = 0; q < g.k.size() && !any; q++) any = (g.v[q] & 1u) == pass;
                if (!any) continue;
                e.op(0xBEFE0100u | (pass ? 78u : 76u));
// ... 160 lines not shown
```

### pygim_amd/csrc/pygim_hip.hip

```cpp
#include "../../include/pygim_hip.h"
#include "kernels.hpp"
#ifdef PYGIM_LDS_ABLATE
#include "lds_kernel_gen_ablate.hpp"
#else
#include "lds_kernel_gen.hpp"
#include "lds_codegen_dev.hpp"
#include "lds_reorder_dev.hpp"
#include "lds_hybrid_dev.hpp"
#endif
#include "transpose_dev.hpp"
#include "sddmm_dev.hpp"
#include "row_gather_dev.hpp"
#include "edge_softmax_dev.hpp"
#include "gat_aggregate_dev.hpp"
#include "spmm_reduce_dev.hpp"
#include <hsa/hsa.h>
#include <hsa/hsa_ext_amd.h>

static inline uint64_t lds_rows_pad(uint64_t ncols, uint32_t kc) {
    const uint64_t k = kc ? kc : 320;
    return ((ncols + k - 1) / k * k + 63) / 64 * 64;
}

#include <algorithm>
// ... 73 lines not shown
}

int64_t pygim_generation(void) { return g_ctx.generation; }

int pygim_device_info(char *name, int name_len, int *cu_count, int64_t *hbm_bytes) {
    int dev = 0;
    hipError_t e = hipGetDevice(&dev);
    if (e != hipSuccess) {
        (void)hipGetLastError();
        return fail(PYGIM_ERR_NO_DEVICE, "no HIP device visible");
    }
    hipDeviceProp_t prop;
    HIP_TRY(hipGetDeviceProperties(&prop, dev));
    if (name && name_len > 0) {
        std::snprintf(name, (size_t)name_len, "%s (%s)", prop.name, prop.gcnArchName);
    }
    if (cu_count) *cu_count = prop.multiProcessorCount;
    if (hbm_bytes) *hbm_bytes = (int64_t)prop.totalGlobalMem;
    return 0;
}

int64_t pygim_set_tunable(const char *name, int64_t value) {
    int64_t *slot = nullptr;
    std::string n = name ? name : "";
    if (n == "long_row_threshold") slot = &g_tune.long_row_threshold;
    else if (n == "long_segment") slot = &g_tune.long_segment;
    else if (n == "force_vec_bytes") slot = &g_tune.force_vec_bytes;
    else if (n == "csr_kernel") slot = &g_tune.csr_kernel;
    else if (n == "coo_chunk") slot = &g_tune.coo_chunk;
    else if (n == "coo_via_rowptr") slot = &g_tune.coo_via_rowptr;
    else if (n == "kernel_events") slot = &g_tune.kernel_events;
    else if (n == "host_windows") slot = &g_tune.host_windows;
    else if (n == "host_direct") slot = &g_tune.host_direct;
    else if (n == "panel_mode") slot = &g_tune.panel_mode;
    else if (n == "panel_bytes") slot = &g_tune.panel_bytes;
    else if (n == "panel_min_seg") slot = &g_tune.panel_min_seg;
    else if (n == "panel_pack") slot = &g_tune.panel_pack;
    else if (n == "panel_coop") slot = &g_tune.panel_coop;
    else if (n == "panel_block") slot = &g_tune.panel_block;
    else if (n == "slice_group_bytes") slot = &g_tune.slice_group_bytes;
    else if (n == "fuse_windows") slot = &g_tune.fuse_windows;
    else if (n == "panel_col16") slot = &g_tune.panel_col16;
    else if (n == "panel_locality") slot = &g_tune.panel_locality;
    else if (n == "split_unit_pattern") slot = &g_tune.split_unit_pattern;
    else if (n == "narrow_vals") slot = &g_tune.narrow_vals;
    else if (n == "merge_parts") slot = &g_tune.merge_parts;
    else if (n == "vec_kernel") slot = &g_tune.vec_kernel;
    else if (n == "vec_lds") slot = &g_tune.vec_lds;
    else if (n == "panel_lds_pad") slot = &g_tune.panel_lds_pad;
    else if (n == "vec_lds_min_seg") slot = &g_tune.vec_lds_min_seg;
    else if (n == "lds_mode") slot = &g_tune.lds_mode;
    else if (n == "lds_min_reuse_x100") slot = &g_tune.lds_min_reuse_x100;
    else if (n == "lds_min_width") slot = &g_tune.lds_min_width;
    else if (n == "lds_min_width8") slot = &g_tune.lds_min_width8;
    else if (n == "lds_min_reuse_narrow_x100") slot = &g_tune.lds_min_reuse_narrow_x100;
    else if (n == "lds_threads") slot = &g_tune.lds_threads;
    else if (n == "lds_waves") slot = &g_tune.lds_waves;
    else if (n == "lds_ablate") slot = &g_tune.lds_ablate;
    else if (n == "lds_round_tiles") slot = &g_tune.lds_round_tiles;
    else if (n == "lds_code") slot = &g_tune.lds_code;
    else if (n == "lds_code_nbuf") slot = &g_tune.lds_code_nbuf;
    else if (n == "lds_code_waves") slot = &g_tune.lds_code_waves;
    else if (n == "lds_fail") slot = &g_tune.lds_fail;
    else if (n == "lds_stamp") slot = &g_tune.lds_stamp;
    else if (n == "lds_code_exp") slot = &g_tune.lds_code_exp;
    else if (n == "lds_hybrid") slot = &g_tune.lds_hybrid;
    else if (n == "lds_hybrid_min") slot = &g_tune.lds_hybrid_min;
    else if (n == "lds_hybrid_contig") slot = &g_tune.lds_hybrid_contig;
    else if (n == "lds_code_boundary") slot = &g_tune.lds_code_boundary;
    else if (n == "lds_xcd_slices") slot = &g_tune.lds_xcd_slices;
    else if (n == "lds_codegen") slot = &g_tune.lds_codegen;
    else if (n == "lds_tile_order") slot = &g_tune.lds_tile_order;
    else if (n == "lds_lp_rounds") slot = &g_tune.lds_lp_rounds;
    else if (n == "lds_code_kc") slot = &g_tune.lds_code_kc;
    else if (n == "lds_code_gsize") slot = &g_tune.lds_code_gsize;
    else if (n == "lds_code_nsets") slot = &g_tune.lds_code_nsets;
    else if (n == "lds_col_split") slot = &g_tune.lds_col_split;
    else if (n == "lds_col_split_f32") slot = &g_tune.lds_col_split_f32;
    else if (n == "lds_fill_tiles") slot = &g_tune.lds_fill_tiles;
    else if (n == "lds_row_tail") slot = &g_tune.lds_row_tail;
    else if (n == "lds_split_order") slot = &g_tune.lds_split_order;
    else if (n == "lds_half_split") slot = &g_tune.lds_half_split;
    else if (n == "lds_direct_x") slot = &g_tune.lds_direct_x;
    else if (n == "lds_long_slots") slot = &g_tune.lds_long_slots;
    if (!slot) {
        fail(PYGIM_ERR_INVALID, "unknown tunable: " + n);
        return -1;
    }
    const int64_t old = *slot;
    if (slot == &g_tune.panel_lds_pad) value = std::min<int64_t>(std::max<int64_t>(value, 0), 64 << 10);
    *slot = value;
    return old;
}

}

static int group_create(int format, int dtype, int n_parts, const int32_t *const *idx0, const int32_t *const *colind,
                        const void *const *values, const int64_t *nrows, const int64_t *ncols, const int64_t *nnz,
                        const int64_t *n_dense, const int64_t *dense_cols, int64_t h_size, int64_t *out_handle, bool adopt) {
    bool adopted = false;
    auto drop_adopted = [&]() {
        if (!adopt || adopted) return;
        adopted = true;
        (void)hipFree(const_cast<int32_t *>(idx0[0]));
        (void)hipFree(const_cast<int32_t *>(colind[0]));
        if (values && values[0]) (void)hipFree(const_cast<void *>(values[0]));
    };
    if (int rc = need_init()) return drop_adopted(), rc;
    if (format != PYGIM_CSR && format != PYGIM_COO) return fail(PYGIM_ERR_INVALID, "format must be CSR(0) or COO(1)");
    const size_t es = dtype_size(dtype);
    if (es == 0) return fail(PYGIM_ERR_INVALID, "unknown dtype");
    if (n_parts <= 0 || !idx0 || !colind || !nrows || !ncols || !nnz || !n_dense || !dense_cols || !out_handle)
        return fail(PYGIM_ERR_INVALID, "null argument or n_parts <= 0");
    if (h_size <= 0) return fail(PYGIM_ERR_INVALID, "h_size must be positive");
    const double t0 = now_ms();
    Group *g = new Group;
    g->format = format;
    g->dtype = dtype;
    t_plan_dtype = dtype;
    g->h = h_size;
    g->total_rows = nrows[0];
    g->parts.resize(n_parts);
    hipStream_t st = nullptr;
    int rc = 0;
    auto bail = [&](int code) {
        (void)hipDeviceSynchronize();
        drop_adopted();
        free_group(g);
        return code;
    };
    if (hipMalloc((void **)&g->d_flags, 8 * sizeof(int)) != hipSuccess) return bail(fail(PYGIM_ERR_HIP, "hipMalloc flags"));
    if (hipMemsetAsync(g->d_flags, 0, 8 * sizeof(int), st) != hipSuccess) return bail(fail(PYGIM_ERR_HIP, "memset flags"));
    if (hipStreamCreateWithFlags(&g->side, hipStreamNonBlocking) != hipSuccess ||
        hipEventCreateWithFlags(&g->ev_fork, hipEventDisableTiming) != hipSuccess ||
        hipEventCreateWithFlags(&g->ev_join, hipEventDisableTiming) != hipSuccess)
        return bail(fail(PYGIM_ERR_HIP, "side stream / events"));
    size_t dpos = 0;
    for (int i = 0; i < n_parts; i++) {
        Part &p = g->parts[i];
        p.nrows = nrows[i];
        p.ncols = ncols[i];
        p.nnz = nnz[i];
        if (p.nrows != g->total_rows) return bail(fail(PYGIM_ERR_INVALID, "all sparse parts must have the same number of rows"));
        if (p.nrows < 0 || p.ncols < 0 || p.nnz < 0 || p.nnz > 0xFFFFFFFFll || p.nrows >= 0xFFFFFFFFll ||
            p.ncols > 0xFFFFFFFFll)
            return bail(fail(PYGIM_ERR_INVALID, "part sizes must fit 32-bit indices (the reference's uint32 matrices)"));
        if (n_dense[i] <= 0) return bail(fail(PYGIM_ERR_INVALID, "n_dense must be positive"));
        int64_t sum = 0;
        for (int64_t j = 0; j < n_dense[i]; j++) {
            if (dense_cols[dpos + j] < 0) return bail(fail(PYGIM_ERR_INVALID, "negative dense width"));
            p.dense_cols.push_back(dense_cols[dpos + j]);
            sum += dense_cols[dpos + j];
        }
        dpos += (size_t)n_dense[i];
        if (sum != h_size) return bail(fail(PYGIM_ERR_INVALID, "dense widths of a part must add up to h_size"));
        g->total_cols += p.ncols;
        if (!idx0[i] && (format == PYGIM_CSR || p.nnz > 0)) return bail(fail(PYGIM_ERR_INVALID, "null index array"));
        if (!colind[i] && p.nnz > 0) return bail(fail(PYGIM_ERR_INVALID, "null colind"));

        if ((rc = to_device<uint32_t>(colind[i], (size_t)p.nnz * 4, &p.colind, &p.own_colind, st))) return bail(rc);
        const void *v = values ? values[i] : nullptr;
        if (v) {
            if ((rc = to_device<void>(v, (size_t)p.nnz * es, &p.vals, &p.own_vals, st))) return bail(rc);
        }
        if (format == PYGIM_CSR) {
            if ((rc = to_device<uint32_t>(idx0[i], (size_t)(p.nrows + 1) * 4, &p.rowptr, &p.own_rowptr, st))) return bail(rc);
// ... 539 lines not shown
    out[3] = p.col16 ? 1 : 0;
    out[4] = ncoop;
    out[5] = p.lp_panel.n_tasks;
    out[6] = (g->merged && g->parts.size() > 1) ? 1 : 0;
    out[7] = p.extra ? 1 : 0;
    return 0;
}

int pygim_group_lds_plan(int64_t handle, int64_t out[4]) {
    Group *g = lookup(handle);
    if (!g) return fail(PYGIM_ERR_INVALID, "unknown group handle");
    const Part &p = (g->merged && g_tune.merge_parts && g->parts.size() > 1) ? *g->merged : g->parts[0];
    out[0] = p.lds_tiles ? (int64_t)p.lds_ntiles : 0;
    out[1] = (int64_t)p.lds_slots;
    out[2] = (int64_t)p.lds_tokens;
    out[3] = p.nnz;
    return 0;
}

int pygim_group_lds_code(int64_t handle, int64_t out[4]) {
    Group *g = lookup(handle);
    if (!g) return fail(PYGIM_ERR_INVALID, "unknown group handle");
    const Part &p = (g->merged && g_tune.merge_parts && g->parts.size() > 1) ? *g->merged : g->parts[0];
    out[0] = p.lds_code ? (int64_t)p.lds_code_bytes : 0;
    out[1] = p.lds_code ? (int64_t)p.lds_code_pairs : 0;
    bool all_code = p.lds_is_code && g_tune.lds_code;
    if (!(g->merged && g_tune.merge_parts && g->parts.size() > 1))
        for (const Part &q : g->parts) all_code = all_code && q.lds_is_code;
    out[2] = all_code ? 1 : 0;
    out[3] = (p.lds_code && p.lds_codegen_device) ? 1 : 0;
    return 0;
}

int pygim_group_lds_tiles(int64_t handle, int64_t out[4]) {
    Group *g = lookup(handle);
    if (!g) return fail(PYGIM_ERR_INVALID, "unknown group handle");
    const Part &p = (g->merged && g_tune.merge_parts && g->parts.size() > 1) ? *g->merged : g->parts[0];
    out[0] = p.lds_tile_labels ? 1 : 0;
    out[1] = p.lds_tile_labels;
    out[2] = p.lds_tile_largest;
    out[3] = p.panel_locality_used ? p.sim_kind : 0;
    return 0;
}

int pygim_group_serial(int64_t handle, int64_t *out) {
    Group *g = lookup(handle);
    if (!g || !out) return fail(PYGIM_ERR_INVALID, "unknown group handle");
    *out = g->serial;
    return 0;
}

int pygim_group_lds_runs(int64_t handle, int64_t *out) {
    Group *g = lookup(handle);
    if (!g || !out) return fail(PYGIM_ERR_INVALID, "unknown group handle");
    *out = g->lds_runs;
    return 0;
}

int pygim_group_host_windows(int64_t handle, int64_t *windows, int64_t *direct) {
    Group *g = lookup(handle);
    if (!g || !windows) return fail(PYGIM_ERR_INVALID, "unknown group handle");
    *windows = g->host_windows_used;
    if (direct) *direct = g->host_direct_used;
    return 0;
}

int pygim_group_lds_geometry(int64_t handle, int64_t out[8]) {
    Group *g = lookup(handle);
    if (!g) return fail(PYGIM_ERR_INVALID, "unknown group handle");
    const Part &p = (g->merged && g_tune.merge_parts && g->parts.size() > 1) ? *g->merged : g->parts[0];
    for (int i = 0; i < 8; i++) out[i] = 0;
    if (!p.lds_tiles) return 0;
    out[0] = p.lds_nw;
    out[1] = p.lds_ka;
    out[2] = p.lds_kc;
    out[3] = p.lds_nbuf;
    out[4] = p.lds_is_code ? p.lds_code_gsize : 0;
    out[5] = p.lds_is_code ? p.lds_code_nsets : 0;
    out[6] = p.lds_is_code ? (int64_t)p.lds_code_shared : 0;
    out[7] = p.lds_col_splits;
    return 0;
}

int pygim_group_lds_note(int64_t handle, char *out, int64_t cap) {
    Group *g = lookup(handle);
    if (!g) return fail(PYGIM_ERR_INVALID, "unknown group handle");
    if (!out || cap <= 0) return fail(PYGIM_ERR_INVALID, "no buffer");
    std::string text;
    if ((g->merged && g_tune.merge_parts && g->parts.size() > 1) || g->parts.size() == 1) {
        text = ((g->merged && g_tune.merge_parts && g->parts.size() > 1) ? *g->merged : g->parts[0]).lds_note;
    } else {
        text = g->parts[0].lds_note;
        for (size_t i = 1; i < g->parts.size(); i++)
            if (g->parts[i].lds_note != g->parts[0].lds_note) text += "; part " + std::to_string(i) + ": " + g->parts[i].lds_note;
    }
    for (size_t i = 0; i < g->parts.size(); i++)
        if (!g->parts[i].hy_note.empty()) text += "; part " + std::to_string(i) + ": " + g->parts[i].hy_note;
    const size_t n = std::min<size_t>(text.size(), (size_t)cap - 1);
    std::memcpy(out, text.data(), n);
    out[n] = 0;
    return 0;
}

int pygim_group_info(int64_t handle, int64_t out[8]) {
    Group *g = lookup(handle);
    if (!g) return fail(PYGIM_ERR_INVALID, "unknown group handle");
    out[0] = g->total_rows;
    out[1] = g->total_cols;
    out[2] = g->h;
    out[3] = (int64_t)g->parts.size();
    int64_t nl = 0;
    for (auto &p : g->parts) nl += p.lp_base.n_long;
    out[4] = nl;
    out[5] = g->all_ones ? 1 : 0;
    out[6] = g->parts[0].d_items ? (int64_t)g->parts[0].npanels : 0;
    out[7] = (int64_t)g->parts[0].n_items;
    return 0;
}

int pygim_block_run_x(int64_t handle, int part, const void *X, int64_t ldx, void *C, int64_t ldc, int64_t width,
                      int accumulate, int x_unchanged, void *stream) {
    if (int rc = need_init()) return rc;
    Group *g = lookup(handle);
    if (!g) return fail(PYGIM_ERR_INVALID, "unknown group handle");
    if (part < 0 || part >= (int)g->parts.size()) return fail(PYGIM_ERR_INVALID, "part index out of range");
    if (!X || !C || width <= 0 || ldx < width || ldc < width) return fail(PYGIM_ERR_INVALID, "bad X/C/width/stride");
    if (!is_device_ptr(X) || !is_device_ptr(C)) return fail(PYGIM_ERR_INVALID, "pygim_block_run needs device pointers");
    g->x_unchanged = x_unchanged != 0;
    const int rc = launch_block_any(g, g->parts[part], X, ldx, C, ldc, width, accumulate != 0, (hipStream_t)stream);
    g->x_unchanged = false;
    return rc;
}

int pygim_block_run(int64_t handle, int part, const void *X, int64_t ldx, void *C, int64_t ldc, int64_t width,
                    int accumulate, void *stream) {
    return pygim_block_run_x(handle, part, X, ldx, C, ldc, width, accumulate, 0, stream);
}

int pygim_spmm_run_group_x(int64_t handle, const void *const *B_parts, void *out, int x_unchanged, void *stream) {
    if (int rc = need_init()) return rc;
    Group *g = lookup(handle);
    if (!g) return fail(PYGIM_ERR_INVALID, "unknown group handle");
    for (auto &p : g->parts)
        if (p.dense_cols != g->parts[0].dense_cols)
            return fail(PYGIM_ERR_INVALID, "spmm_run_group needs the same dense split for every sparse part");
    g->x_unchanged = x_unchanged != 0;
    const int rc = run_group_common(g, B_parts, nullptr, false, out, (hipStream_t)stream);
    g->x_unchanged = false;
    return rc;
}

int pygim_spmm_run_group(int64_t handle, const void *const *B_parts, void *out, void *stream) {
    return pygim_spmm_run_group_x(handle, B_parts, out, 0, stream);
}

int pygim_grande_run_group(int64_t handle, const void *const *B_windows, const int64_t *window_ld, void *out,
                           void *stream) {
    if (int rc = need_init()) return rc;
    Group *g = lookup(handle);
    if (!g) return fail(PYGIM_ERR_INVALID, "unknown group handle");
    if (!window_ld) return fail(PYGIM_ERR_INVALID, "window_ld is required");
    return run_group_common(g, B_windows, window_ld, true, out, (hipStream_t)stream);
}

int pygim_spmv_run_group(int64_t handle, const void *const *B_vectors, void *out, void *stream) {
    if (int rc = need_init()) return rc;
// ... 95 lines not shown
```

### pygim_amd/csrc/rt_launch.inc

```
int pick_vec_bytes(size_t es, const void *X, int64_t ldx, const void *C, int64_t ldc) {
    auto ok = [&](size_t vb) {
        return ((uintptr_t)X % vb == 0) && ((uintptr_t)C % vb == 0) && ((size_t)ldx * es % vb == 0) &&
               ((size_t)ldc * es % vb == 0);
    };
    size_t cap = g_tune.force_vec_bytes > 0 ? (size_t)g_tune.force_vec_bytes : 16;
    for (size_t vb : {(size_t)16, (size_t)8})
        if (vb <= cap && vb > es && ok(vb)) return (int)vb;
    return (int)es;
}

struct KernelTimer {
    Group *g;
    hipStream_t st;
    hipEvent_t a = nullptr, b = nullptr;
    KernelTimer(Group *g_, hipStream_t st_, bool on = true) : g(g_), st(st_) {
        if (on && (g_tune.kernel_events || g->kernel_events) && hipEventCreate(&a) == hipSuccess && hipEventCreate(&b) == hipSuccess)
            (void)hipEventRecord(a, st);
        else
            a = b = nullptr;
    }
    void stop() {
        if (!a) return;
        (void)hipEventRecord(b, st);
        g->ev_pending.emplace_back(a, b);
// ... 165 lines not shown
                       (AM == 3 ? (const uint32_t *)p.col16 : p.colind), vals, Xs0, ldg,                                  \
                       slice_stride, Cs0, ldc, ws, ns, (accumulate ? 1 : 0) | (p.panel_locality_used ? 2 : 0), q * p.panel_cols,   \
                       g->deq_out ? g->deq_out + (size_t)s0 * F : nullptr, g->deq_ld, g->deq_amax, g->deq_log2,                  \
                       g->post_mul ? g->post_mul + (size_t)s0 * F : nullptr, g->post_add ? g->post_add + (size_t)s0 * F : nullptr, \
                       g->post_relu)
#define PYGIM_LAUNCH_PANEL(AM, HV) PYGIM_LAUNCH_PANEL_D(AM, HV, false)
                int amode = !off32 ? 0 : ((size_t)ldg * sizeof(T) == 128 ? 2 : 1);
                if (amode == 2 && p.col16 && g_tune.panel_col16) amode = 3;
                if constexpr (DeqType<T>::ok) {
                    if (g->deq_out && amode >= 2 && !vals) {
                        if (amode == 3) PYGIM_LAUNCH_PANEL_D(3, 0, true);
                        else PYGIM_LAUNCH_PANEL_D(2, 0, true);
                        continue;
                    }
                }
                if (g->deq_out) return fail(PYGIM_ERR_INVALID, "internal: fused dequantisation on an unsupported sweep");
                if constexpr (sizeof(T) == 8) {
                    if (vals && p.vals_narrow && g_tune.narrow_vals) {
                        const T *vals = (const T *)p.vals_narrow;
                        if (amode == 3) PYGIM_LAUNCH_PANEL(3, 2);
                        else if (amode == 2) PYGIM_LAUNCH_PANEL(2, 2);
                        else if (amode == 1) PYGIM_LAUNCH_PANEL(1, 2);
                        else PYGIM_LAUNCH_PANEL(0, 2);
                        continue;
                    }
                }
                if (amode == 3 && vals) PYGIM_LAUNCH_PANEL(3, 1);
                else if (amode == 3) PYGIM_LAUNCH_PANEL(3, 0);
                else if (amode == 2 && vals) PYGIM_LAUNCH_PANEL(2, 1);
                else if (amode == 2) PYGIM_LAUNCH_PANEL(2, 0);
                else if (amode == 1 && vals) PYGIM_LAUNCH_PANEL(1, 1);
                else if (amode == 1) PYGIM_LAUNCH_PANEL(1, 0);
                else if (vals) PYGIM_LAUNCH_PANEL(0, 1);
                else PYGIM_LAUNCH_PANEL(0, 0);
#undef PYGIM_LAUNCH_PANEL
#undef PYGIM_LAUNCH_PANEL_D
            }
            }
            kt.stop();
            return join();
        }
    }
    bool wide = lanes_needed > 32;
    if (g_tune.csr_kernel == 1) wide = true;
    if (g_tune.csr_kernel == 2 && lanes_needed <= 32) wide = false;
    if (nrows > 0) {
        KernelTimer kt(g, st, !p.is_extra || p.timed);
        if (wide) {
            dim3 grid((nrows + 3) / 4, (lanes_needed + 63) / 64);
            hipLaunchKernelGGL((k_csr_wide<T, VEC>), grid, dim3(256), 0, st, p.rowptr, p.colind, vals, X, ldx, C,
                               ldc, nrows, w, lp.thresh, accumulate ? 1 : 0);
        } else {
            int log_lpr = 0;
            while ((1u << log_lpr) < lanes_needed) log_lpr++;
            const uint32_t rows_per_wave = 64u >> log_lpr;
            const uint32_t waves = (nrows + rows_per_wave - 1) / rows_per_wave;
            hipLaunchKernelGGL((k_csr_sub<T, VEC>), dim3((waves + 3) / 4), dim3(256), 0, st, p.rowptr, p.colind,
                               vals, X, ldx, C, ldc, nrows, w, lp.thresh, accumulate ? 1 : 0, log_lpr);
        }
        kt.stop();
    }
    return join();
}

template <typename T>
int launch_lds(Group *g, Part &p, const T *X, int64_t ldx, T *C, int64_t ldc, uint32_t w, bool accumulate, hipStream_t st,
               const void *lds_xs = nullptr, const uint32_t *deq_amax = nullptr, int deq_log2 = 0) {
    constexpr bool WIDE8 = sizeof(T) == 1;
    constexpr bool EL8 = sizeof(T) == 8;
    constexpr uint32_t ROWB = EL8 ? 512 : 256;
    constexpr uint32_t EPS = WIDE8 ? 128 : ROWB / sizeof(T);
    constexpr int PVEC = WIDE8 ? 8 : 16 / (int)sizeof(T);
    const bool split16 = p.lds_col_splits > 1 && (WIDE8 || (sizeof(T) == 2 && deq_amax != nullptr));
    const uint32_t w_lanes = split16 ? (uint32_t)(((size_t)w * 2 + 3) / 4)
                                     : (WIDE8 || EL8 || (sizeof(T) == 2 && deq_amax)) ? w : (uint32_t)(((size_t)w * sizeof(T) + 3) / 4);
    const bool HS = p.lds_half != 0;
    if (HS && (sizeof(T) != 4 || w > 32 || lds_xs || deq_amax)) return fail(PYGIM_ERR_INVALID, "internal: a half-split LDS plan serves plain 4-byte products of at most 32 lanes");
    const uint32_t nslices = HS ? 1u : (w + EPS - 1) / EPS;
    const uint64_t rows_pad = HS ? (uint64_t)p.lds_half : lds_rows_pad((uint64_t)p.ncols, p.lds_kc);
    const size_t need = (size_t)rows_pad * nslices * ROWB;
    KernelTimer kt(g, st, !p.is_extra || p.timed);
    XsPin pin;
    void *xs_use = const_cast<void *>(lds_xs);
    if (!xs_use && g_tune.lds_direct_x && nslices == 1 && !HS && !WIDE8 && !p.lds_col_order && (size_t)ldx * sizeof(T) == ROWB && (size_t)w * sizeof(T) == ROWB &&
        ((uintptr_t)X & 255) == 0) {
        void *base = nullptr;
        size_t size = 0;
        if (hipMemGetAddressRange((hipDeviceptr_t *)&base, &size, (hipDeviceptr_t)X) == hipSuccess && base && (const char *)X + (size_t)rows_pad * ROWB <= (const char *)base + size)
            xs_use = const_cast<void *>((const void *)X);
        else
            (void)hipGetLastError();
    }
    if (!xs_use) {
        std::lock_guard<std::mutex> lk(g_ctx.mu);
        if (g->x_unchanged) {
            int dev = 0;
            (void)hipGetDevice(&dev);
            Context::XsBuf *hit = nullptr;
            for (auto &kv : g_ctx.xs_bufs) {
                Context::XsBuf &b = kv.second;
                if (kv.first.first == dev && b.ptr && b.src == (const void *)X && b.ld == ldx && b.rows == p.ncols && b.w == (int64_t)w &&
                    b.es == sizeof(T) && b.kind == (HS ? 5 : WIDE8 ? 3 : 1) && b.rows_pad == rows_pad && b.order == (const void *)p.lds_col_order && b.bytes >= need &&
                    (!hit || b.stamp > hit->stamp))
                    hit = &b;
            }
            if (hit) {
                hit->stamp = ++g_ctx.xs_clock;
                hit->in_use++;
                xs_use = hit->ptr;
                pin.hold(xs_use);
            }
        }
        if (!xs_use) {
            Context::XsBuf *b = nullptr;
            if (int rc = xs_buffer_locked(st, std::max<size_t>(need, 256), &b)) return rc;
            xs_use = b->ptr;
            pin.hold(xs_use);
            b->src = X;
            b->ld = ldx;
            b->rows = p.ncols;
            b->w = (int64_t)w;
            b->es = sizeof(T);
            b->kind = HS ? 5 : WIDE8 ? 3 : 1;
            b->rows_pad = rows_pad;
            b->order = p.lds_col_order;
            const uint64_t threads = (uint64_t)p.ncols * nslices * 16;
            if (HS) {
                if constexpr (sizeof(T) == 4) {
                    const uint64_t th = rows_pad * 16;
                    hipLaunchKernelGGL((k_slice_pack_hs<T>), dim3((unsigned)((th + 255) / 256)), dim3(256), 0, st, X, ldx, (uint32_t)p.ncols, w, (uint32_t)rows_pad, (T *)xs_use);
                }
            } else if constexpr (WIDE8) {
                if (threads > 0)
                    hipLaunchKernelGGL(k_slice_pack_widen8, dim3((unsigned)((threads + 255) / 256)), dim3(256), 0, st, (const int8_t *)X, ldx,
                                       (uint32_t)p.ncols, w, nslices, (int16_t *)xs_use, (uint32_t)rows_pad, (const uint32_t *)p.lds_col_order);
            } else if constexpr (EL8) {
                const uint64_t th8 = (uint64_t)p.ncols * nslices * 32;
                if (th8 > 0)
                    hipLaunchKernelGGL((k_slice_pack<T, 2, 5>), dim3((unsigned)((th8 + 255) / 256)), dim3(256), 0, st, X, ldx,
                                       (uint32_t)p.ncols, w, nslices, (T *)xs_use, (uint32_t)rows_pad, (const uint32_t *)p.lds_col_order);
            } else if (threads > 0) {
                hipLaunchKernelGGL((k_slice_pack<T, PVEC, 4>), dim3((unsigned)((threads + 255) / 256)), dim3(256), 0, st, X, ldx,
                                   (uint32_t)p.ncols, w, nslices, (T *)xs_use, (uint32_t)rows_pad, (const uint32_t *)p.lds_col_order);
            }
        }
    }
    LdsArgs a{};
    a.tok = p.lds_tok;
    a.tiles = p.lds_tiles;
    a.rowmap = p.lds_rowmap;
    a.xs = (const char *)xs_use;
    a.c = (char *)C;
    a.slice_stride = rows_pad * ROWB;
    a.ldc_bytes = (uint32_t)((size_t)ldc * (((WIDE8 || sizeof(T) == 2) && deq_amax) ? 4 : sizeof(T)));
    a.w = w_lanes;
    a.nslices = nslices;
    a.ntiles = p.lds_ntiles;
    a.accumulate = accumulate ? 1 : 0;
    const uint32_t S = p.lds_col_splits;
    const uint64_t ldp = split16 ? (uint64_t)w_lanes * 2 : (uint64_t)w_lanes * 4 / sizeof(T);
    const size_t part_es = split16 ? 2 : sizeof(T);
    const uint64_t lds_rows = p.lds_rows ? p.lds_rows : (uint64_t)p.nrows;
    const bool deq_at_reduce = S > 1 && deq_amax != nullptr;
    if (S > 1) {
        const size_t need = (((size_t)S * (size_t)lds_rows * ldp * part_es + 255) & ~(size_t)255) + (size_t)p.lds_tail_nseg * nslices * 64 * 8;
        if (int rc = ensure(&g->scratch, &g->scratch_bytes, std::max<size_t>(need, 256))) return rc;
        a.c = (char *)g->scratch;
        a.ldc_bytes = (uint32_t)(ldp * part_es);
        a.accumulate = 0;
    }
    const uint32_t *kernel_amax = (deq_at_reduce || split16) ? nullptr : deq_amax;
    a.wdelta = p.lds_wdelta;
    a.deq_amax = kernel_amax;
    a.deq_log2 = deq_log2;
    a.post_mul = kernel_amax ? g->post_mul : nullptr;
    a.post_add = kernel_amax ? g->post_add : nullptr;
    a.post_relu = kernel_amax ? g->post_relu : 0;
    a.xcd_group = (nslices == 1 || nslices == 2 || nslices == 4 || nslices == 8) ? 8 / nslices : 0;
    a.xcd_sx = 1;
    if (a.xcd_group && p.lds_is_code && nslices > 1) {
        uint32_t sx = (uint32_t)std::max<int64_t>(0, g_tune.lds_xcd_slices);
        if (sx == 0) {
            const uint64_t nchunks = ((uint64_t)p.ncols + p.lds_kc - 1) / std::max(1u, p.lds_kc);
            const double fill = p.lds_ntiles && nchunks ? (double)p.lds_slots / ((double)p.lds_ntiles * (double)nchunks) : 1.0;
            sx = fill < 0.3 ? std::min(nslices, 4u) : (EL8 ? 1u : 2u);
        }
        if (sx > 1 && sx <= nslices && nslices % sx == 0) {
            a.xcd_sx = sx;
            a.xcd_group *= sx;
        }
    }
    a.half_split = HS ? 1u : 0u;
    a.xcd_contig = (a.xcd_group && p.lds_contig_tiles) ? (p.lds_ntiles + a.xcd_group - 1) / a.xcd_group : 0;
    const uint32_t grid = a.xcd_group ? 8 * ((p.lds_ntiles + a.xcd_group - 1) / a.xcd_group) * a.xcd_sx : p.lds_ntiles * nslices;
    using KernelFn = void (*)(LdsArgs);
    KernelFn fn = nullptr;
    const bool long16 = p.lds_nw == 16 && p.lds_batch == LDS_L16_BATCH;
    if (p.lds_is_code) {
        if (!g_tune.lds_code || g_tune.lds_ablate) return fail(PYGIM_ERR_INVALID, "this group's LDS plan is a code stream: lds_code was switched off (or lds_ablate on) after it was created");
        const bool w8 = p.lds_nw == 8;
        if constexpr (EL8) {
            if (!w8 || kernel_amax || S > 1 || p.lds_row_bytes != 512) return fail(PYGIM_ERR_INVALID, "internal: 8-byte LDS-staged product on an unsupported plan");
            if constexpr (std::is_same<T, double>::value) fn = k_lds_code8_f64;
            else fn = k_lds_code8_i64;
        } else if constexpr (sizeof(T) == 1) {
            if (!w8 || (accumulate && S <= 1)) return fail(PYGIM_ERR_INVALID, "internal: INT8 LDS-staged product on an unsupported plan");
            fn = split16 ? k_lds_code8_i16 : kernel_amax ? k_lds_code8_i8_deq : k_lds_code8_i8;
        } else if constexpr (sizeof(T) == 2) {
            if ((kernel_amax || split16) && !w8) return fail(PYGIM_ERR_INVALID, "internal: dequantising LDS-staged product on an unsupported plan");
            fn = kernel_amax ? k_lds_code8_i16_deq : (w8 ? k_lds_code8_i16 : k_lds_code_i16);
        } else if constexpr (std::is_same<T, float>::value) {
            fn = kernel_amax ? (w8 ? k_lds_code8_f32_deq : k_lds_code_f32_deq) : (w8 ? k_lds_code8_f32 : k_lds_code_f32);
        } else {
            fn = kernel_amax ? (w8 ? k_lds_code8_i32_deq : k_lds_code_i32_deq) : (w8 ? k_lds_code8_i32 : k_lds_code_i32);
        }
        if (g_tune.lds_stamp && fn == k_lds_code8_f32) {
            fn = k_lds_code8_f32_ts;
            a.stamps = (uint64_t *)(uintptr_t)g_tune.lds_stamp;
        }
        a.code = p.lds_code;
        a.code_start = p.lds_code_start;
        a.piece_bytes = p.lds_code_piece;
    } else if constexpr (sizeof(T) == 1 || sizeof(T) == 8) {
        return fail(PYGIM_ERR_INVALID, "internal: the INT8 / INT64 / DBL64 LDS-staged product exists in the code-stream form only");
    } else if (kernel_amax) {
        if (p.lds_nw != 16 || p.lds_wdelta || sizeof(T) != 4) return fail(PYGIM_ERR_INVALID, "internal: dequantising LDS-staged product on an unsupported plan");
        if constexpr (std::is_same<T, float>::value) fn = long16 ? k_lds_spmm_f32_w16b_deq : k_lds_spmm_f32_w16_deq;
        else if constexpr (std::is_same<T, int32_t>::value) fn = long16 ? k_lds_spmm_i32_w16b_deq : k_lds_spmm_i32_w16_deq;
    } else if constexpr (sizeof(T) == 2) {
        if (p.lds_nw != 16) return fail(PYGIM_ERR_INVALID, "internal: INT16 LDS-staged product needs the 16-wave plan");
        fn = long16 ? k_lds_spmm_i16_w16b : (p.lds_wdelta ? k_lds_spmm_i16_w16_val : k_lds_spmm_i16_w16);
    } else if (long16) {
        if constexpr (std::is_same<T, float>::value) fn = k_lds_spmm_f32_w16b;
        else fn = k_lds_spmm_i32_w16b;
    } else if constexpr (std::is_same<T, float>::value) {
        fn = p.lds_nw == 16 ? (p.lds_wdelta ? k_lds_spmm_f32_w16_val : k_lds_spmm_f32_w16) : k_lds_spmm_f32_w8;
#ifdef PYGIM_LDS_ABLATE
        if (p.lds_nw == 16 && !p.lds_wdelta && !long16) {
            switch (g_tune.lds_ablate) {
                case 6: fn = k_lds_spmm_f32_w16_ab6; break;
                case 7: fn = k_lds_spmm_f32_w16_ab7; break;
                case 10: fn = k_lds_spmm_f32_w16_ab10; break;
                case 11: fn = k_lds_spmm_f32_w16_ab11; break;
                case 12: fn = k_lds_spmm_f32_w16_ab12; break;
                case 15: fn = k_lds_spmm_f32_w16_ab15; break;
                case 16: fn = k_lds_spmm_f32_w16_ab16; break;
                case 17: fn = k_lds_spmm_f32_w16_ab17; break;
                case 18: fn = k_lds_spmm_f32_w16_ab18; break;
                case 19: fn = k_lds_spmm_f32_w16_ab19; break;
                default: break;
            }
        }
#else
        if (g_tune.lds_ablate) return fail(PYGIM_ERR_INVALID, "lds_ablate needs the ablation build (make -C pygim_amd/csrc ablate)");
#endif
    } else {
        fn = p.lds_nw == 16 ? (p.lds_wdelta ? k_lds_spmm_i32_w16_val : k_lds_spmm_i32_w16) : k_lds_spmm_i32_w8;
    }
    if (kernel_amax && g_tune.lds_ablate) return fail(PYGIM_ERR_INVALID, "lds_ablate is a timing experiment of the plain kernel");
    if (!fn) return fail(PYGIM_ERR_INVALID, "internal: no LDS-staged kernel for this plan");
    {
        static std::set<std::pair<int, KernelFn>> attr_done;
        int dev = 0;
        HIP_TRY(hipGetDevice(&dev));
        std::lock_guard<std::mutex> lk(g_ctx.mu);
        if (!attr_done.count({dev, fn})) {
            HIP_TRY(hipFuncSetAttribute((const void *)fn, hipFuncAttributeMaxDynamicSharedMemorySize, (int)LDS_BYTES));
            attr_done.insert({dev, fn});
        }
    }
    hipLaunchKernelGGL(fn, dim3(grid), dim3(p.lds_nw * 64), LDS_BYTES, st, a);
    g->lds_runs++;
    if (split16 && lds_rows > 0 && w > 0) {
        const uint64_t total = lds_rows * w;
        const dim3 rg((unsigned)((total + 255) / 256));
        if (!deq_amax)
            hipLaunchKernelGGL((k_lds_reduce16<0>), rg, dim3(256), 0, st, (const int16_t *)g->scratch, S, lds_rows, w, ldp, (void *)C, ldc, accumulate ? 1 : 0, nullptr, 0, nullptr, nullptr, 0);
        else if (WIDE8)
            hipLaunchKernelGGL((k_lds_reduce16<1>), rg, dim3(256), 0, st, (const int16_t *)g->scratch, S, lds_rows, w, ldp, (void *)C, ldc, 0, deq_amax, deq_log2, g->post_mul, g->post_add, g->post_relu);
        else
            hipLaunchKernelGGL((k_lds_reduce16<2>), rg, dim3(256), 0, st, (const int16_t *)g->scratch, S, lds_rows, w, ldp, (void *)C, ldc, 0, deq_amax, deq_log2, g->post_mul, g->post_add, g->post_relu);
    } else if (S > 1 && lds_rows > 0 && w > 0 && sizeof(T) == 4 && (w & 3) == 0 && (ldp & 3) == 0 && (ldc & 3) == 0 && ((uintptr_t)C & 15) == 0) {
        if constexpr (sizeof(T) == 4) {
            const uint64_t total4 = lds_rows * (w >> 2);
            const dim3 rg((unsigned)((total4 + 255) / 256));
            if (deq_at_reduce)
                hipLaunchKernelGGL((k_lds_reduce_v4<T, true>), rg, dim3(256), 0, st, (const T *)g->scratch, S, lds_rows, w, ldp, (void *)C, ldc, 0, deq_amax, deq_log2, g->post_mul,
                                   g->post_add, g->post_relu);
            else
                hipLaunchKernelGGL((k_lds_reduce_v4<T, false>), rg, dim3(256), 0, st, (const T *)g->scratch, S, lds_rows, w, ldp, (void *)C, ldc, accumulate ? 1 : 0, nullptr, 0, nullptr,
                                   nullptr, 0);
        }
    } else if (S > 1 && lds_rows > 0 && w > 0) {
        const uint64_t total = lds_rows * w;
        if constexpr (sizeof(T) == 4) {
            if (deq_at_reduce)
                hipLaunchKernelGGL((k_lds_reduce_deq<T>), dim3((unsigned)((total + 255) / 256)), dim3(256), 0, st, (const T *)g->scratch, S, lds_rows, w, ldp, (float *)C, ldc,
                                   deq_amax, deq_log2, g->post_mul, g->post_add, g->post_relu);
        }
        if (!deq_at_reduce)
            hipLaunchKernelGGL((k_lds_reduce<T>), dim3((unsigned)((total + 255) / 256)), dim3(256), 0, st, (const T *)g->scratch, S, lds_rows, w, ldp, C,
                               ldc, accumulate ? 1 : 0);
    }
    if (lds_rows < (uint64_t)p.nrows && w > 0) {
        if constexpr (sizeof(T) == 4) {
            using A = typename AccOf<T>::type;
            if (!p.lds_tail_segs || !p.lds_tail_rowseg) return fail(PYGIM_ERR_INVALID, "internal: an LDS plan that leaves rows out has no segment table for them");
            const uint32_t ntail = (uint32_t)((uint64_t)p.nrows - lds_rows);
            const size_t split_bytes = S > 1 ? (((size_t)S * (size_t)lds_rows * ldp * sizeof(T) + 255) & ~(size_t)255) : 0;
            const size_t park_bytes = (size_t)p.lds_tail_nseg * nslices * 64 * sizeof(A);
            if (int rc = ensure(&g->scratch, &g->scratch_bytes, std::max<size_t>(split_bytes + park_bytes, 256))) return rc;
            A *parked = (A *)((char *)g->scratch + split_bytes);
            if (p.lds_tail_nseg > 0)
                hipLaunchKernelGGL((k_lds_tail_seg<T>), dim3(p.lds_tail_nseg, nslices), dim3(512), 0, st, p.lds_tail_segs, p.lds_tail_nseg, p.colind, (const char *)xs_use,
                                   (uint64_t)(rows_pad * ROWB), parked);
            const int64_t ldc_b = (int64_t)ldc * 4;
            if (deq_amax)
                hipLaunchKernelGGL((k_lds_tail_fin<T, true>), dim3(ntail, nslices), dim3(64), 0, st, p.lds_tail_rowseg, (uint32_t)lds_rows, parked, w, (void *)C, ldc_b, 0, deq_amax,
                                   deq_log2, g->post_mul, g->post_add, g->post_relu);
            else
                hipLaunchKernelGGL((k_lds_tail_fin<T, false>), dim3(ntail, nslices), dim3(64), 0, st, p.lds_tail_rowseg, (uint32_t)lds_rows, parked, w, (void *)C, ldc_b,
                                   accumulate ? 1 : 0, nullptr, 0, nullptr, nullptr, 0);
        } else {
            return fail(PYGIM_ERR_INVALID, "internal: an LDS plan that leaves rows to the tail kernels exists for 4-byte element types only");
        }
    }
    kt.stop();
    HIP_TRY(hipGetLastError());
    return 0;
}

template <typename T> bool want_lds(const Group *g, const Part &p, uint32_t w, int64_t ldc, const void *C, bool accumulate = false) {
    if constexpr (sizeof(T) == 8) {
        if (!p.lds_is_code || p.lds_nw != 8 || p.lds_row_bytes != 512 || p.lds_col_splits > 1 || false) return false;
    } else if (p.lds_row_bytes == 512) return false;
    if constexpr (sizeof(T) == 1) {
        if (!p.lds_is_code || p.lds_nw != 8 || (accumulate && p.lds_col_splits <= 1)) return false;
        if ((int64_t)(w / 2) < g_tune.lds_min_width) return false;
    }
    if constexpr (sizeof(T) == 2) {
        if ((w & 1) || (ldc & 1) || ((uintptr_t)C & 3) || (p.lds_nw != 16 && !p.lds_is_code)) return false;
    }
    if (!p.lds_tiles || g_tune.lds_mode == 2 || (!p.lds_is_code && (p.vals != nullptr) != (p.lds_wdelta != 0)) || g->deq_out || g->pre_xs) return false;
    if (p.lds_half && (sizeof(T) != 4 || w > 32)) return false;
    if (p.lds_is_code && (!g_tune.lds_code || g_tune.lds_ablate)) return false;
    if (g_tune.lds_mode == 0 && (g_tune.panel_mode == 1 || g_tune.csr_kernel != 0 || g_tune.force_vec_bytes != 0)) return false;
    if (sizeof(T) > 1 && (int64_t)(sizeof(T) == 8 ? (size_t)w : (size_t)w * sizeof(T) / 4) < (sizeof(T) == 8 ? g_tune.lds_min_width8 : g_tune.lds_min_width)) return false;
    if ((uint64_t)ldc * sizeof(T) >= (1ull << 32)) return false;
    return true;
}

template <typename T>
int launch_block(Group *g, Part &p, const void *X, int64_t ldx, void *C, int64_t ldc, int64_t w, bool accumulate,
                 hipStream_t st) {
    const T *x = (const T *)X;
    T *c = (T *)C;
    const uint32_t ww = (uint32_t)w;
    if (want_lds<T>(g, p, ww, ldc, C, accumulate)) return launch_lds<T>(g, p, x, ldx, c, ldc, ww, accumulate, st);
    if (ww <= 4 && g_tune.vec_kernel && g_tune.force_vec_bytes == 0 && g_tune.csr_kernel == 0 && p.rowptr && p.nrows > 0) {
        using A = typename AccOf<T>::type;
        constexpr size_t LDS_TOTAL = 160 * 1024 - 64;
        const size_t panel_lds = (((((size_t)p.panel_cols + 1) * ww * sizeof(T)) + 15) & ~(size_t)15) + 16;
        const size_t per_entry = 4 + (size_t)ww * sizeof(A);
        const bool lds_rule = g_tune.vec_lds && g_tune.panel_mode != 2 && p.d_items && p.col16 && p.lp_panel.n_tasks == 0 && !p.panel_locality_used &&
                              p.npanels >= 1 && p.panel_long128.size() == 4 * (size_t)p.npanels && (uint64_t)p.nnz < (1ull << 31) &&
                              (double)p.nnz >= (double)g_tune.vec_lds_min_seg * (double)p.nrows * (double)p.npanels;
        if (lds_rule && panel_lds + 64 * 12 * per_entry <= LDS_TOTAL) {
            const size_t stage_budget = std::min<size_t>(32 * 1024, LDS_TOTAL - panel_lds);
            uint32_t F16 = (uint32_t)(stage_budget / (64 * per_entry)) / 24 * 24;
            const int merge4 = F16 == 0 ? 1 : 0;
            if (merge4) F16 = (uint32_t)(stage_budget / (64 * per_entry)) / 12 * 12;
            const size_t shmem = panel_lds + 64 * (size_t)F16 * per_entry;
            const uint32_t cu = (uint32_t)std::max(g_ctx.cu_count, 1);
            if (!p.d_spmv_units) {
                std::vector<uint32_t> act;
                double wsum = 0;
                for (uint32_t q = 0; q < p.npanels; q++)
                    if (p.panel_off[q + 1] > p.panel_off[q]) {
                        act.push_back(q);
                        wsum += (double)std::max<uint64_t>(p.panel_nnz[q], p.panel_off[q + 1] - p.panel_off[q]);
                    }
                if (!act.empty()) {
                    std::vector<uint32_t> nb(act.size(), 1);
                    if (act.size() < cu) {
                        uint32_t left = cu - (uint32_t)act.size();
                        std::vector<std::pair<double, size_t>> rem;
                        uint32_t given = 0;
                        for (size_t k = 0; k < act.size(); k++) {
                            const uint32_t q = act[k];
                            const double share = (double)left * (double)std::max<uint64_t>(p.panel_nnz[q], p.panel_off[q + 1] - p.panel_off[q]) / wsum;
                            const uint32_t fl = (uint32_t)share;
                            nb[k] += fl;
                            given += fl;
                            rem.emplace_back(share - fl, k);
                        }
                        std::sort(rem.begin(), rem.end(), [](const std::pair<double, size_t> &x, const std::pair<double, size_t> &y) { return x.first > y.first; });
                        for (size_t k = 0; given < left && k < rem.size(); k++, given++) nb[rem[k].second]++;
                    }
// ... 154 lines not shown
```

### pygim_amd/csrc/rt_plans.inc

```
template <typename T> void launch_check_ones(const void *v, uint32_t n, int *flag, hipStream_t st) {
    hipLaunchKernelGGL((k_check_ones<T>), dim3((n + 255) / 256), dim3(256), 0, st, (const T *)v, n, flag);
}

void plan_long_rows(const uint32_t *rowptr, int64_t nrows, uint32_t thresh, uint32_t seg, const std::vector<char> *flags,
                    std::vector<uint32_t> &tasks, std::vector<uint32_t> &desc) {
    for (int64_t r = 0; r < nrows; r++) {
        const uint32_t s = rowptr[r], e = rowptr[r + 1];
        const bool is_long = flags ? (*flags)[(size_t)r] != 0 : (e - s > thresh);
        if (!is_long || e == s) continue;
        const uint32_t first = (uint32_t)(tasks.size() / 3);
        uint32_t n = 0;
        for (uint32_t a = s; a < e; a += seg, n++) {
            tasks.push_back((uint32_t)r);
            tasks.push_back(a);
            tasks.push_back(std::min(e, a + seg));
        }
        desc.push_back((uint32_t)r);
        desc.push_back(first);
        desc.push_back(n);
    }
}

int build_lds_plan(Part &p, size_t es, int *d_flag_sorted, hipStream_t st, const std::vector<uint32_t> &h_rowptr, int64_t h_hint);
double now_ms();
// ... 125 lines not shown
                    if (hi[r] > lo[r] || (q == 0 && deg == 0 && !p.is_extra)) order.push_back((uint32_t)r);
                }
                {
                    uint32_t longest = 0;
                    for (uint32_t r : order) longest = std::max(longest, hi[r] - lo[r]);
                    std::vector<size_t> start((size_t)longest + 2, 0);
                    for (uint32_t r : order) start[(size_t)(longest - (hi[r] - lo[r])) + 1]++;
                    for (size_t k = 1; k < start.size(); k++) start[k] += start[k - 1];
                    std::vector<uint32_t> sorted(order.size());
                    for (uint32_t r : order) sorted[start[(size_t)(longest - (hi[r] - lo[r]))]++] = r;
                    order.swap(sorted);
                }
                uint32_t nco = 0;
                for (uint32_t r : order) nco += (hi[r] - lo[r] > coop_cap) ? 1u : 0u;
                if (!loc_rank.empty() && order.size() > nco) {
                    const uint32_t nblk = (uint32_t)((nr + 2047) / 2048);
                    std::vector<size_t> bstart((size_t)nblk + 1, 0);
                    for (size_t k = nco; k < order.size(); k++) bstart[(size_t)(loc_rank[order[k]] >> 11) + 1]++;
                    for (size_t k = 1; k < bstart.size(); k++) bstart[k] += bstart[k - 1];
                    std::vector<uint32_t> byblk(order.size() - nco);
                    for (size_t k = nco; k < order.size(); k++) byblk[bstart[loc_rank[order[k]] >> 11]++] = order[k];
                    std::copy(byblk.begin(), byblk.end(), order.begin() + nco);
                }
                p.panel_coop.push_back(nco);
                uint32_t n256 = 0, n128 = 0, n64 = 0, n32 = 0;
                uint64_t pn = 0;
                for (uint32_t r : order) {
                    const uint32_t l = hi[r] - lo[r];
                    n256 += l > 256u ? 1u : 0u;
                    n128 += l > 128u ? 1u : 0u;
                    n64 += l > 64u ? 1u : 0u;
                    n32 += l > 32u ? 1u : 0u;
                    pn += l;
                }
                p.panel_long128.push_back(n256);
                p.panel_long128.push_back(n128);
                p.panel_long128.push_back(n64);
                p.panel_long128.push_back(n32);
                p.panel_nnz.push_back(pn);
                for (uint32_t r : order) {
                    rows_v.push_back(r);
                    beg_v.push_back(lo[r]);
                    const uint32_t first = (lo[r] == rp[r]) ? 0x80000000u : 0u;
                    const uint32_t last = (hi[r] == rp[r + 1]) ? 0x40000000u : 0u;
                    len_v.push_back((hi[r] - lo[r]) | first | last);
                }
                p.panel_off.push_back(rows_v.size());
            }
            p.n_items = rows_v.size();
            if (p.n_items > 0) {
                if (hipMalloc((void **)&p.d_items, 3 * p.n_items * 4) != hipSuccess ||
                    hipMemcpy(p.d_items, rows_v.data(), p.n_items * 4, hipMemcpyHostToDevice) != hipSuccess ||
                    hipMemcpy(p.d_items + p.n_items, beg_v.data(), p.n_items * 4, hipMemcpyHostToDevice) != hipSuccess ||
                    hipMemcpy(p.d_items + 2 * p.n_items, len_v.data(), p.n_items * 4, hipMemcpyHostToDevice) != hipSuccess)
                    return fail(PYGIM_ERR_HIP, "panel plan upload");
                if (g_tune.panel_col16 && p.panel_cols <= 65536 && p.nnz > 0) {
                    if (hipMalloc((void **)&p.col16, (size_t)p.nnz * 2 + 64) != hipSuccess) return fail(PYGIM_ERR_HIP, "col16 alloc");
                    hipLaunchKernelGGL(k_make_col16, dim3((unsigned)((p.nnz + 255) / 256)), dim3(256), 0, st, p.colind,
                                       (uint64_t)p.nnz, p.panel_cols, p.col16);
                    if (hipStreamSynchronize(st) != hipSuccess) return fail(PYGIM_ERR_HIP, "col16 build");
                }
            }
        }
    }
    return allow_lds ? build_lds_plan(p, es, d_flag_sorted, st, h_rowptr, h_hint) : 0;
}

static int build_lds_plan_form(Part &p, size_t es, int *d_flag_sorted, hipStream_t st, const std::vector<uint32_t> &h_rowptr, int64_t h_hint,
                               bool allow_code);
int build_lds_plan(Part &p, size_t es, int *d_flag_sorted, hipStream_t st, const std::vector<uint32_t> &h_rowptr, int64_t h_hint) {
    p.lds_note.clear();
    int rc = build_lds_plan_form(p, es, d_flag_sorted, st, h_rowptr, h_hint, true);
    if (rc == -1) {
        const std::string why = p.lds_note;
        rc = build_lds_plan_form(p, es, d_flag_sorted, st, h_rowptr, h_hint, false);
        p.lds_note = why + (p.lds_tiles ? "; products take the token form of the LDS-staged kernel (k_lds_spmm_*)" : "; no token plan either: the L2 sweep serves this group");
    }
    if (p.lds_note.empty())
        p.lds_note = p.lds_tiles ? (p.lds_is_code ? (p.lds_codegen_device || p.lds_codegen_why.empty() ? std::string("code-stream form")
                                                                                                         : "code-stream form (written by the host encoder: " + p.lds_codegen_why + ")")
                                                  : std::string("token form of the LDS-staged kernel")) : "no LDS-staged plan (rule, type or width): the L2 sweep serves this group";
    if (p.lds_tiles && p.lds_half)
        p.lds_note += "; half-split plan: two column ranges of " + std::to_string(p.lds_half) + " columns in the two halves of a wave (a row's sum = the sum of its ranges' sums)";
    if (p.lds_tiles && p.lds_rows)
        p.lds_note += "; the plan's tiles hold the first " + std::to_string(p.lds_rows) + " of " + std::to_string(p.nrows) + " rows (one workgroup per compute unit), k_lds_tail the others";
    if (p.lds_tiles && p.lds_col_splits > 1 && t_plan_dtype == PYGIM_FLT32)
        p.lds_note += "; " + std::to_string(p.lds_col_splits) + " column ranges per row tile: a row's FLT32 sum is the sum of its ranges' sums (inside 1e-5 of |A|.|x|, not the "
                      "CPU loop's bits; lds_col_split_f32 = 0 keeps the stored-order form)";
    if (!p.lds_codegen_device && !p.lds_codegen_why.empty() && p.lds_note.find(p.lds_codegen_why) == std::string::npos)
        p.lds_note += " [device code generation not used: " + p.lds_codegen_why + "]";
    return rc;
}

static void code_ring(uint32_t NW, uint32_t row_bytes, uint32_t &NBUF, uint32_t &KC) {
    int64_t nbuf = g_tune.lds_code_nbuf;
    if (nbuf == 0) nbuf = NW == 8 ? LDS_CODE8_AUTO_NBUF : 2;
    nbuf = std::min<int64_t>(std::max<int64_t>(nbuf, 2), 10);
    static const uint32_t kc_of[11] = {0, 0, 320, 192, 160, 128, 96, 64, 64, 64, 64};
    uint32_t kc = g_tune.lds_code_kc > 0 ? (uint32_t)g_tune.lds_code_kc : kc_of[nbuf] * 256 / row_bytes;
    const uint32_t kq = 1024 * NW / row_bytes;
    kc = std::max(kq, kc / kq * kq);
    while ((uint64_t)kc * row_bytes * (uint64_t)nbuf > LDS_BYTES || kc * (uint32_t)nbuf > 640) kc -= kq;
    KC = kc;
    NBUF = (uint32_t)nbuf;
}

static int build_tail_segments(Part &p, const std::vector<uint32_t> &h_rowptr) {
    if (!p.lds_rows || p.lds_rows >= (uint32_t)p.nrows) return 0;
    std::vector<uint32_t> rows, e0, e1, rowseg;
    for (uint32_t r = p.lds_rows; r < (uint32_t)p.nrows; r++) {
        rowseg.push_back((uint32_t)rows.size());
        for (uint32_t e = h_rowptr[r]; e < h_rowptr[r + 1]; e += LDS_TAIL_SEG) {
            rows.push_back(r);
            e0.push_back(e);
            e1.push_back(std::min<uint32_t>(e + LDS_TAIL_SEG, h_rowptr[r + 1]));
        }
    }
    rowseg.push_back((uint32_t)rows.size());
    p.lds_tail_nseg = (uint32_t)rows.size();
    std::vector<uint32_t> segs;
    segs.insert(segs.end(), rows.begin(), rows.end());
    segs.insert(segs.end(), e0.begin(), e0.end());
    segs.insert(segs.end(), e1.begin(), e1.end());
    if (hipMalloc((void **)&p.lds_tail_segs, std::max<size_t>(segs.size() * 4, 256)) != hipSuccess ||
        hipMalloc((void **)&p.lds_tail_rowseg, rowseg.size() * 4) != hipSuccess ||
        (!segs.empty() && hipMemcpy(p.lds_tail_segs, segs.data(), segs.size() * 4, hipMemcpyHostToDevice) != hipSuccess) ||
        hipMemcpy(p.lds_tail_rowseg, rowseg.data(), rowseg.size() * 4, hipMemcpyHostToDevice) != hipSuccess)
        return fail(PYGIM_ERR_HIP, "segment table of the rows outside the LDS plan");
    return 0;
}

int build_hybrid(Part &p, int dtype, size_t es, int *d_flag_sorted, hipStream_t st, int64_t h_hint) {
    static const bool plan_timing = getenv("PYGIM_PLAN_TIMING") != nullptr;
    p.hy_note.clear();
    if (!g_tune.lds_hybrid || p.is_extra || p.vals || p.lds_tiles || p.sim_kind != 2 || p.nrows != p.ncols || p.nnz < (1 << 20) || !p.rowptr) {
        if (plan_timing && g_tune.lds_hybrid && !p.is_extra)
            fprintf(stderr, "[pygim plan] density split not considered: vals %d, lds plan %d, similarity kind %d, %lld x %lld, nnz %lld, rowptr %d\n", p.vals ? 1 : 0, p.lds_tiles ? 1 : 0,
                    p.sim_kind, (long long)p.nrows, (long long)p.ncols, (long long)p.nnz, p.rowptr ? 1 : 0);
        return 0;
    }
    if (!(dtype == PYGIM_INT32 || dtype == PYGIM_INT16 || (dtype == PYGIM_INT8 && g_tune.lds_hybrid >= 3) || (dtype == PYGIM_FLT32 && g_tune.lds_hybrid >= 2))) return 0;
    if (g_tune.lds_mode == 2 || !g_tune.lds_code || g_tune.lds_waves != 16 || g_tune.lds_code_waves == 16) return 0;
    if (h_hint > 0 && (h_hint * (int64_t)std::max<size_t>(es, 2)) / 4 < g_tune.lds_min_width) return 0;
    const double t0 = now_ms();
    HybridSplit hs;
    const uint32_t min_cell = (uint32_t)std::min<int64_t>(std::max<int64_t>(g_tune.lds_hybrid_min, 1), 1 << 20);
    uint32_t cell_rows = LDS_CODE_AUTO_WAVES * LDS_CODE8_KA, cell_cols = 128, ring_nbuf = 0;
    if (g_tune.lds_round_tiles && h_hint > 0)
        cell_rows = lds_rows_per_tile((uint32_t)p.nrows, cell_rows, (uint32_t)((h_hint * (int64_t)std::max<size_t>(es, 2) + 255) / 256), (uint32_t)std::max(g_ctx.cu_count, 1));
    code_ring(LDS_CODE_AUTO_WAVES, 256, ring_nbuf, cell_cols);
    std::string why = hybrid_split_on_device(p.rowptr, p.colind, (uint32_t)p.nrows, (uint64_t)p.nnz, p.sim_order, cell_rows, cell_cols, min_cell, st, hs);
    if (why.empty() && (double)hs.nnz_d < 0.3 * (double)p.nnz) {
        why = "hybrid: the dense cells hold " + std::to_string(hs.nnz_d) + " of " + std::to_string(p.nnz) + " entries only";
        hs.release();
    }
    if (!why.empty()) {
        p.hy_note = why;
        if (plan_timing) fprintf(stderr, "[pygim plan] density split not used: %s (%.1f ms)\n", why.c_str(), now_ms() - t0);
        return 0;
    }
    std::unique_ptr<Part> d(new Part), sp(new Part);
    for (Part *q : {d.get(), sp.get()}) {
        q->nrows = p.nrows;
        q->ncols = p.ncols;
        q->dense_cols = p.dense_cols;
        q->own_rowptr = q->own_colind = true;
// ... 91 lines not shown
    if (ch.code.size() * 4 != dr.code_bytes) return "code size " + std::to_string(dr.code_bytes) + " against " + std::to_string(ch.code.size() * 4) + " bytes";
    if (plan.ntiles != dr.ntiles || plan.slots != dr.slots) return "tile / slot counts";
    std::vector<uint32_t> d_code(ch.code.size());
    void *stage = nullptr;
    if (hipMalloc(&stage, std::max<size_t>(dr.code_bytes, 256)) != hipSuccess) return "out of device memory for the comparison";
    const uint64_t n16 = dr.code_bytes / 16;
    hipLaunchKernelGGL(k_copy16, dim3((unsigned)((n16 + 255) / 256)), dim3(256), 0, 0, (const u32x4_t *)dr.code, (u32x4_t *)stage, n16);
    const bool got = hipMemcpy(d_code.data(), stage, dr.code_bytes, hipMemcpyDeviceToHost) == hipSuccess;
    (void)hipFree(stage);
    if (!got) return "code D2H failed";
    if (memcmp(d_code.data(), ch.code.data(), dr.code_bytes) != 0) {
        size_t at = 0;
        while (d_code[at] == ch.code[at]) at++;
        size_t s = 0;
        while (s + 1 < ch.start.size() && ch.start[s + 1] / 4 <= at) s++;
        char buf[160];
        snprintf(buf, sizeof buf, "first difference at dword %zu (stream %zu + %zu): %08x against the host's %08x", at, s, at - (size_t)(ch.start[s] / 4), d_code[at], ch.code[at]);
        return buf;
    }
    std::vector<uint64_t> d_start(ch.start.size());
    std::vector<uint32_t> d_rowmap(plan.rowmap.size());
    std::vector<LdsTile> d_tiles(plan.tiles.size());
    if (hipMemcpy(d_start.data(), dr.d_start, d_start.size() * 8, hipMemcpyDeviceToHost) != hipSuccess ||
        hipMemcpy(d_rowmap.data(), dr.d_rowmap, d_rowmap.size() * 4, hipMemcpyDeviceToHost) != hipSuccess ||
        hipMemcpy(d_tiles.data(), dr.d_tiles, d_tiles.size() * sizeof(LdsTile), hipMemcpyDeviceToHost) != hipSuccess)
        return "table D2H failed";
    if (d_start != ch.start) return "stream offsets";
    if (d_rowmap != plan.rowmap) return "row map";
    for (size_t t = 0; t < d_tiles.size(); t++)
        if (d_tiles[t].nch != plan.tiles[t].nch || d_tiles[t].row0 != plan.tiles[t].row0 || d_tiles[t].nnz != plan.tiles[t].nnz || d_tiles[t].chunk0 != plan.tiles[t].chunk0)
            return "tile table";
    if (dr.entries != ch.entries || dr.pairs != ch.pairs || dr.shared != ch.shared) return "statistics";
    return std::string();
}

static int build_lds_plan_form(Part &p, size_t es, int *d_flag_sorted, hipStream_t st, const std::vector<uint32_t> &h_rowptr, int64_t h_hint,
                               bool allow_code) {
    static const bool plan_timing = getenv("PYGIM_PLAN_TIMING") != nullptr;
    double t_mark = now_ms();
    auto lap = [&](const char *what) {
        if (!plan_timing) return;
        const double t = now_ms();
        fprintf(stderr, "[pygim plan] %-34s %8.1f ms\n", what, t - t_mark);
        t_mark = t;
    };
    const size_t val_es = es;
    const bool int8_code = es == 1 && t_plan_dtype == PYGIM_INT8 && allow_code && g_tune.lds_code && g_tune.lds_waves == 16 && g_tune.lds_code_waves != 16;
    if (es == 1) {
        if (!int8_code) return 0;
        es = 2;
    }
    const bool el8_code = es == 8 && (t_plan_dtype == PYGIM_INT64 || t_plan_dtype == PYGIM_DBL64) && allow_code && g_tune.lds_code &&
                          g_tune.lds_waves == 16 && g_tune.lds_code_waves != 16;
    if (es == 8 && !el8_code) return 0;
    if (g_tune.lds_mode == 2 || (es != 4 && es != 2 && es != 8) || p.is_extra || p.nnz == 0 || p.nrows == 0 || p.ncols == 0) return 0;
    if ((p.vals || es == 2) && g_tune.lds_waves != 16) return 0;
    if (h_hint > 0 && (es == 8 ? h_hint : (h_hint * (int64_t)std::max<size_t>(es, 2)) / 4) < (es == 8 ? g_tune.lds_min_width8 : g_tune.lds_min_width)) return 0;
    if ((uint64_t)p.ncols * (es == 8 ? 512ull : 256ull) >= (1ull << 32) - (1ull << 20) || (uint64_t)p.nnz >= (1ull << 31)) return 0;
    LdsGeometry geo;
    geo.NW = g_tune.lds_waves == 16 ? 16 : 8;
    geo.KA = lds_ka(geo.NW);
    geo.KC = LDS_KC;
    geo.BATCH = lds_batch(geo.NW);
    geo.keep_tile_order = p.lds_contig_tiles ? 1u : 0u;
    const bool want_code = allow_code && g_tune.lds_code && geo.NW == 16 &&
                           ((es == 4 && t_plan_dtype == PYGIM_FLT32) || (es == 4 && t_plan_dtype == PYGIM_INT32) ||
                            (es == 2 && t_plan_dtype == PYGIM_INT16) || int8_code || el8_code);
    const int64_t slice_b = es == 8 ? 512 : 256;
    const int64_t nsl_hint = h_hint > 0 ? (h_hint * (int64_t)es + slice_b - 1) / slice_b : 4;
    if (want_code) {
        const int64_t cw = g_tune.lds_code_waves;
        const bool eight = cw == 8 || (cw != 16 && LDS_CODE_AUTO_WAVES == 8) || int8_code || el8_code;
        if (eight) {
            geo.NW = 8;
            geo.KA = el8_code ? LDS_CODE8_KA64 : LDS_CODE8_KA;
            geo.BATCH = 8;
        }
        if (el8_code) geo.row_bytes = 512;
    }
    if (g_tune.lds_round_tiles && h_hint > 0)
        geo.rows_per_tile = lds_rows_per_tile((uint32_t)p.nrows, geo.NW * geo.KA, (uint32_t)nsl_hint, (uint32_t)std::max(g_ctx.cu_count, 1));
    const bool f32_split_ok = g_tune.lds_col_split_f32 == 1 ? p.nnz >= (1 << 20) : g_tune.lds_col_split_f32 != 0;
    uint32_t rows_lds = (uint32_t)p.nrows;
    if (g_tune.lds_col_split != 1 && (geo.NW == 16 || want_code) && !el8_code && (t_plan_dtype != PYGIM_FLT32 || f32_split_ok) && !p.vals) {
        const uint32_t cus = (uint32_t)std::max(g_ctx.cu_count, 1);
        const uint64_t nsl = h_hint > 0 ? (uint64_t)nsl_hint : 1;
        const uint64_t tall = ((uint64_t)p.nrows + geo.NW * geo.KA - 1) / (geo.NW * geo.KA), wgs = tall * nsl;
        uint32_t S = 1;
        if (g_tune.lds_col_split > 1) S = (uint32_t)std::min<int64_t>(g_tune.lds_col_split, 16);
        else if (wgs * 2 <= cus) S = (uint32_t)std::min<uint64_t>(8, cus / wgs);
        if (g_tune.lds_col_split == 0 && g_tune.lds_row_tail > 0 && want_code && es == 4 && !p.lds_forced && (uint64_t)p.nrows * 8 < (1ull << 31)) {
            const uint64_t full = (uint64_t)geo.NW * geo.KA;
            for (uint32_t S2 = 8; S2 > S; S2--) {
                const uint64_t tall2 = cus / (nsl * S2);
                if (!tall2) continue;
                const uint64_t covered = tall2 * full;
                if (covered >= (uint64_t)p.nrows) break;
                if (((uint64_t)p.nrows - covered) * 100 <= (uint64_t)p.nrows * (uint64_t)g_tune.lds_row_tail && tall2 * nsl * S2 * 10 >= (uint64_t)cus * 9) {
                    S = S2;
                    rows_lds = (uint32_t)covered;
                    break;
                }
            }
        }
        if (S > 1 && (uint64_t)p.nrows * S < (1ull << 31)) {
            geo.col_splits = S;
            geo.rows_per_tile = 0;
            if (g_tune.lds_split_order && (((uint64_t)rows_lds + geo.NW * geo.KA - 1) / (geo.NW * geo.KA)) * nsl * S <= cus) geo.keep_tile_order = 1;
            if (g_tune.lds_col_split == 0 && g_tune.lds_fill_tiles && rows_lds == (uint32_t)p.nrows) {
                const uint64_t tall2 = cus / (nsl * S);
                if (tall2 > tall && tall2 <= 2 * tall) geo.rows_per_tile = (uint32_t)std::max<uint64_t>(16, ((uint64_t)p.nrows + tall2 - 1) / tall2);
            }
        }
    }
    if (want_code) {
        code_ring(geo.NW, geo.row_bytes, geo.NBUF, geo.KC);
        geo.boundary = g_tune.lds_code_boundary == 2 ? 0u : 1u;
    }
    const int64_t lanes_hint = h_hint > 0 ? (h_hint * (int64_t)es + 3) / 4 : 0;
    const bool half = want_code && g_tune.lds_half_split && es == 4 && geo.NW == 8 && !p.vals && !p.lds_forced && lanes_hint > 0 && lanes_hint <= 32 &&
                      (t_plan_dtype == PYGIM_INT32 || (t_plan_dtype == PYGIM_FLT32 && f32_split_ok)) && rows_lds == (uint32_t)p.nrows && (uint64_t)p.ncols >= 4ull * geo.KC &&
                      !g_tune.lds_code_exp && !(g_tune.lds_fail & 7);
    uint32_t half_H = 0;
    if (half) {
        half_H = (uint32_t)(((((uint64_t)p.ncols + 1) / 2 + geo.KC - 1) / geo.KC) * geo.KC);
        geo.half_split = 1;
    }
    const bool narrow_hint = es != 8 && lanes_hint > 0 && lanes_hint <= 32;
    const double min_reuse_x100 = !narrow_hint ? (double)g_tune.lds_min_reuse_x100
                                               : std::max((double)g_tune.lds_min_reuse_x100, (double)g_tune.lds_min_reuse_narrow_x100 * (half ? 1.6 : 1.0));
    if (g_tune.lds_mode == 0 && !p.lds_forced &&
        lds_plan_uniform_reuse((uint64_t)p.nnz, (uint32_t)p.nrows, half ? half_H : (uint32_t)p.ncols, geo) * 100.0 < min_reuse_x100)
        return 0;
    if (p.cols_sorted < 0) {
        int unsorted = 0;
        if (hipMemsetAsync(d_flag_sorted, 0, sizeof(int), st) != hipSuccess) return fail(PYGIM_ERR_HIP, "flag reset");
        hipLaunchKernelGGL(k_check_sorted_cols, dim3((unsigned)((p.nrows + 255) / 256)), dim3(256), 0, st, p.rowptr, p.colind,
                           (uint32_t)p.nrows, d_flag_sorted);
        if (hipMemcpy(&unsorted, d_flag_sorted, sizeof(int), hipMemcpyDeviceToHost) != hipSuccess) return fail(PYGIM_ERR_HIP, "sortedness check");
        p.cols_sorted = unsorted ? 0 : 1;
    }
    if (!p.cols_sorted) return 0;
    const uint32_t code_op = t_plan_dtype == PYGIM_FLT32 ? 0x02000000u : t_plan_dtype == PYGIM_INT32 ? 0x68000000u : t_plan_dtype == PYGIM_DBL64 ? LDS_CODE_ADD_F64 :
                             t_plan_dtype == PYGIM_INT64 ? LDS_CODE_ADD_U64 : LDS_CODE_PK_ADD_U16;
    std::vector<uint32_t> rorder;
    if (want_code && p.nrows == p.ncols && rows_lds == (uint32_t)p.nrows && !half &&
        (g_tune.lds_tile_order == 1 || p.lds_forced || (g_tune.lds_tile_order == 2 && p.nnz >= (1 << 20)))) {
        find_similarity(p, st, g_tune.lds_tile_order == 1 || p.lds_forced);
        if (p.sim_kind == 2) {
            rorder = p.sim_order;
            p.lds_tile_labels = p.sim_labels;
            p.lds_tile_largest = p.sim_largest;
        }
        lap("similarity order (label propagation)");
    }
    const uint32_t *ro = rorder.empty() ? nullptr : rorder.data();
    std::string dev_why;
    if (want_code && g_tune.lds_codegen && !(g_tune.lds_fail & 7) && !g_tune.lds_code_exp) {
        CgDeviceResult dr;
        std::string exec_why;
        auto alloc_exec = [&](size_t bytes) -> void * { return exec_alloc(bytes, &exec_why); };
        auto free_exec = [&](void *q) { (void)hsa_amd_memory_pool_free(q); };
        uint32_t *d_vals32 = nullptr;
        if (p.vals && val_es < 4) {
            if (hipMalloc((void **)&d_vals32, std::max<size_t>((size_t)p.nnz * 4, 256)) != hipSuccess) {
                (void)hipGetLastError();
                d_vals32 = nullptr;
            } else if (val_es == 1) hipLaunchKernelGGL((k_widen_vals<int8_t>), dim3((unsigned)(((uint64_t)p.nnz + 255) / 256)), dim3(256), 0, st, (const int8_t *)p.vals, (uint64_t)p.nnz, d_vals32);
            else hipLaunchKernelGGL((k_widen_vals<int16_t>), dim3((unsigned)(((uint64_t)p.nnz + 255) / 256)), dim3(256), 0, st, (const int16_t *)p.vals, (uint64_t)p.nnz, d_vals32);
        }
        struct FreeVals { uint32_t *q; ~FreeVals() { if (q) (void)hipFree(q); } } free_vals{d_vals32};
        g_cg_fail_big_alloc = (g_tune.lds_fail & 8) != 0;
        dev_why = (p.vals && val_es < 4 && !d_vals32) ? std::string("out of device memory for the widened values") :
                  cg_run_on_device(p.rowptr, p.colind, es == 8 ? nullptr : (p.vals && val_es < 4) ? d_vals32 : (const uint32_t *)p.vals, es == 8 ? (const uint64_t *)p.vals : nullptr, h_rowptr.data(), ro, rows_lds,
                                   half ? half_H : (uint32_t)p.ncols, geo, code_op,
                                   (uint32_t)std::max<int64_t>(0, g_tune.lds_code_gsize), (uint32_t)std::max<int64_t>(0, g_tune.lds_code_nsets), st, alloc_exec,
                                   free_exec, dr, [] { return now_ms(); }, half ? half_H : 0u);
        if (dev_why.empty()) {
            if (plan_timing)
                fprintf(stderr, "[pygim plan] device code generation: rows %.1f, chunk lists %.1f, keys + sort %.1f, columns %.1f, slots + groups %.1f, sizes %.1f, emission %.1f, "
                                "whole %.1f ms (%.1f MB of code)\n", dr.ms[0], dr.ms[1], dr.ms[2], dr.ms[3], dr.ms[4], dr.ms[5], dr.ms[6], dr.ms[7], dr.code_bytes / 1e6);
            if (g_tune.lds_codegen == 2) {
                std::string diff = codegen_verify(p, geo, code_op, h_rowptr, ro, dr, d_vals32, rows_lds, half ? half_H : 0u);
                if (!diff.empty()) {
                    (void)hsa_amd_memory_pool_free(dr.code);
                    (void)hipFree(dr.d_start);
                    (void)hipFree(dr.d_rowmap);
                    (void)hipFree(dr.d_tiles);
                    return fail(PYGIM_ERR_INVALID, ("lds_codegen = 2: the device-generated code stream differs from the host encoder's: " + diff).c_str());
                }
            }
            p.lds_code = (char *)dr.code;
            p.lds_code_bytes = dr.code_bytes;
            p.lds_code_start = dr.d_start;
            p.lds_rowmap = dr.d_rowmap;
            p.lds_tiles = dr.d_tiles;
            p.lds_code_pairs = dr.pairs;
            p.lds_code_shared = dr.shared;
            p.lds_is_code = true;
            p.lds_code_piece = geo.KC * geo.row_bytes / geo.NW;
            p.lds_code_gsize = dr.regs.gsize;
            p.lds_code_nsets = dr.regs.nsets;
            p.lds_col_splits = geo.col_splits;
            p.lds_kc = geo.KC;
            p.lds_nbuf = geo.NBUF;
            p.lds_row_bytes = geo.row_bytes;
            p.lds_ka = geo.KA;
            p.lds_ntiles = dr.ntiles;
            p.lds_nw = geo.NW;
            p.lds_batch = geo.BATCH;
            p.lds_slots = dr.slots;
            p.lds_tokens = dr.entries;
            p.lds_codegen_device = true;
            p.lds_rows = rows_lds < (uint32_t)p.nrows ? rows_lds : 0;
            p.lds_half = half ? half_H : 0;
            lap("code stream generated on the device");
            return build_tail_segments(p, h_rowptr);
        }
        (void)hipGetLastError();
        if (plan_timing) fprintf(stderr, "[pygim plan] device code generation not used: %s\n", dev_why.c_str());
        p.lds_codegen_why = dev_why;
    } else if (want_code) {
        p.lds_codegen_why = !g_tune.lds_codegen ? "lds_codegen = 0" : (g_tune.lds_fail & 7) ? "lds_fail set" : "timing experiment";
    }
    std::vector<uint32_t> h_col((size_t)p.nnz);
    if (hipMemcpy(h_col.data(), p.colind, h_col.size() * 4, hipMemcpyDeviceToHost) != hipSuccess) return fail(PYGIM_ERR_HIP, "colind D2H");
    lap("sortedness check + column ids D2H");
    std::vector<uint32_t> h_val;
    std::vector<uint64_t> h_val64;
    if (p.vals) {
        h_val.resize((size_t)p.nnz);
        if (es == 4) {
            if (hipMemcpy(h_val.data(), p.vals, h_val.size() * 4, hipMemcpyDeviceToHost) != hipSuccess) return fail(PYGIM_ERR_HIP, "values D2H");
        } else if (es == 8) {
            h_val64.resize((size_t)p.nnz);
            if (hipMemcpy(h_val64.data(), p.vals, h_val64.size() * 8, hipMemcpyDeviceToHost) != hipSuccess) return fail(PYGIM_ERR_HIP, "values D2H");
            for (size_t i = 0; i < h_val.size(); i++) h_val[i] = (uint32_t)i;
        } else if (val_es == 1) {
            std::vector<int8_t> v8((size_t)p.nnz);
            if (hipMemcpy(v8.data(), p.vals, v8.size(), hipMemcpyDeviceToHost) != hipSuccess) return fail(PYGIM_ERR_HIP, "values D2H");
            for (size_t i = 0; i < v8.size(); i++) h_val[i] = (uint32_t)(int32_t)v8[i];
        } else {
            std::vector<uint16_t> v16((size_t)p.nnz);
            if (hipMemcpy(v16.data(), p.vals, v16.size() * 2, hipMemcpyDeviceToHost) != hipSuccess) return fail(PYGIM_ERR_HIP, "values D2H");
            for (size_t i = 0; i < v16.size(); i++) h_val[i] = want_code ? (uint32_t)(int32_t)(int16_t)v16[i] : (uint32_t)v16[i] * 0x10001u;
        }
    }
    LdsPlanHost plan;
    try {
        if (g_tune.lds_fail & 4) throw std::runtime_error("lds_fail: forced failure of the schedule build");
        if (half) half_split_virtual_matrix(h_rowptr, (uint32_t)p.nrows, half_H, h_col, h_val);
        lds_plan_build(h_rowptr.data(), h_col.data(), rows_lds, half ? half_H : (uint32_t)p.ncols, geo, plan, (unsigned)std::max<int64_t>(0, g_tune.lds_threads),
                       (p.vals || half) ? h_val.data() : nullptr, ro);
    } catch (const std::exception &e) {
        p.lds_note = std::string("the schedule of the LDS-staged product could not be built (") + e.what() + "): the L2 sweep serves this group";
        return 0;
    }
    lap("schedule (tiles, tokens)");
    if (geo.NW == 16 && !p.vals && !want_code && g_tune.lds_long_slots && plan.slots > 0 &&
        (double)plan.ntokens / ((double)plan.slots * geo.NW) >= (double)g_tune.lds_long_slots) {
        LdsGeometry gl = geo;
        gl.KA = LDS_L16_KA;
        gl.BATCH = LDS_L16_BATCH;
        gl.rows_per_tile = geo.col_splits > 1 ? 0 : g_tune.lds_round_tiles && h_hint > 0
                               ? lds_rows_per_tile((uint32_t)p.nrows, gl.NW * gl.KA, (uint32_t)nsl_hint, (uint32_t)std::max(g_ctx.cu_count, 1))
                               : 0;
        const uint32_t r_now = geo.rows_per_tile ? geo.rows_per_tile : geo.NW * geo.KA, r_new = gl.rows_per_tile ? gl.rows_per_tile : gl.NW * gl.KA;
        if (r_new >= r_now) {
            try {
                lds_plan_build(h_rowptr.data(), h_col.data(), (uint32_t)p.nrows, (uint32_t)p.ncols, gl, plan,
                               (unsigned)std::max<int64_t>(0, g_tune.lds_threads), nullptr);
            } catch (const std::exception &e) {
                p.lds_note = std::string("the schedule of the LDS-staged product could not be built (") + e.what() + "): the L2 sweep serves this group";
                return 0;
            }
            geo = gl;
        }
    }
    std::vector<uint32_t>().swap(h_col);
    std::vector<uint32_t>().swap(h_val);
    if (p.vals && !want_code) {
        if ((uint64_t)plan.tok.size() * 8 >= (1ull << 32)) return 0;
        p.lds_wdelta = (uint32_t)(plan.tok.size() * 4);
        plan.tok.insert(plan.tok.end(), plan.wts.begin(), plan.wts.end());
        std::vector<uint32_t>().swap(plan.wts);
    }
    auto up = [&](auto **dst, const auto &v) {
        using E = typename std::remove_reference<decltype(v[0])>::type;
        const size_t bytes = std::max<size_t>(v.size() * sizeof(E), 64);
        if (hipMalloc((void **)dst, bytes) != hipSuccess) return false;
        return v.empty() || hipMemcpy(*dst, v.data(), v.size() * sizeof(E), hipMemcpyHostToDevice) == hipSuccess;
    };
    if (plan.header_overflow) {
        p.lds_note = "the LDS-staged schedule does not fit its slot headers (more than 16 383 batches of one wave in one chunk, or more than 5 M columns): the L2 sweep serves this group";
        return 0;
    }
    if (want_code) {
        LdsCodeHost ch;
        try {
            if (g_tune.lds_fail & 1) throw std::runtime_error("lds_fail: forced failure of the code generation");
            lds_code_from_plan(plan, t_plan_dtype == PYGIM_FLT32 ? 0x02000000u : t_plan_dtype == PYGIM_INT32 ? 0x68000000u : t_plan_dtype == PYGIM_DBL64 ? LDS_CODE_ADD_F64 :
                                     t_plan_dtype == PYGIM_INT64 ? LDS_CODE_ADD_U64 : LDS_CODE_PK_ADD_U16, ch,
                               (unsigned)std::max<int64_t>(0, g_tune.lds_threads), (uint32_t)std::max<int64_t>(0, g_tune.lds_code_gsize),
                               (uint32_t)std::max<int64_t>(0, g_tune.lds_code_nsets), (uint32_t)std::max<int64_t>(0, g_tune.lds_code_exp),
                               h_val64.empty() ? nullptr : h_val64.data());
        } catch (const std::exception &e) {
            p.lds_note = std::string("code-stream form not available: generating the instruction streams failed (") + e.what() + ")";
            return -1;
        }
        lap("code generation");
        std::vector<uint32_t>().swap(plan.tok);
        std::string why_exec;
        void *code = (g_tune.lds_fail & 2) ? nullptr : exec_alloc_upload(ch.code.data(), ch.code.size() * 4, &why_exec);
        if (!code) {
            p.lds_note = "code-stream form not available: " + (why_exec.empty() ? std::string("lds_fail: forced failure of the executable allocation") : why_exec) +
                         " (" + std::to_string(ch.code.size() * 4) + " bytes of code)";
            return -1;
        }
        if (!up(&p.lds_code_start, ch.start) || !up(&p.lds_rowmap, plan.rowmap) || !up(&p.lds_tiles, plan.tiles)) {
            (void)hsa_amd_memory_pool_free(code);
            return fail(PYGIM_ERR_HIP, "code-stream plan upload");
        }
        lap("code + tables upload");
        p.lds_code = (char *)code;
        p.lds_code_bytes = ch.code.size() * 4;
        p.lds_code_pairs = ch.pairs;
        p.lds_is_code = true;
        p.lds_code_piece = geo.KC * geo.row_bytes / geo.NW;
        p.lds_code_gsize = ch.regs.gsize;
        p.lds_code_nsets = ch.regs.nsets;
        p.lds_code_shared = ch.shared;
    } else if (!up(&p.lds_tok, plan.tok) || !up(&p.lds_rowmap, plan.rowmap) || !up(&p.lds_tiles, plan.tiles)) {
        return fail(PYGIM_ERR_HIP, "LDS plan upload");
    }
    p.lds_col_splits = geo.col_splits;
    p.lds_rows = rows_lds < (uint32_t)p.nrows ? rows_lds : 0;
    p.lds_half = half ? half_H : 0;
    p.lds_kc = geo.KC;
    p.lds_nbuf = geo.NBUF;
    p.lds_row_bytes = geo.row_bytes;
    p.lds_ka = geo.KA;
    p.lds_ntiles = plan.ntiles;
    p.lds_nw = geo.NW;
    p.lds_batch = geo.BATCH;
    p.lds_slots = plan.slots;
    p.lds_tokens = plan.ntokens;
    return build_tail_segments(p, h_rowptr);
}

double now_ms() {
    using namespace std::chrono;
    return duration<double, std::milli>(steady_clock::now().time_since_epoch()).count();
}

int need_init() {
    if (!g_ctx.inited) return fail(PYGIM_ERR_NO_DEVICE, "backend not initialised: call dpu_init_ranks / pygim_init_ranks first");
    return 0;
}
```

### pygim_amd/csrc/rt_state.inc

```
thread_local std::string g_err;
int fail(int code, const std::string &msg) {
    g_err = msg;
    return code;
}
#define HIP_TRY(expr)                                                                          \
    do {                                                                                       \
        hipError_t _e = (expr);                                                                \
        if (_e != hipSuccess) {                                                                \
            (void)hipGetLastError();                                                           \
            return fail(PYGIM_ERR_HIP, std::string(#expr) + ": " + hipGetErrorString(_e));     \
        }                                                                                      \
    } while (0)

size_t dtype_size(int dt) {
    switch (dt) {
        case PYGIM_INT8: return 1;
        case PYGIM_INT16: return 2;
        case PYGIM_INT32: return 4;
        case PYGIM_INT64: return 8;
        case PYGIM_FLT32: return 4;
        case PYGIM_DBL64: return 8;
    }
    return 0;
}

struct Tunables {
    int64_t long_row_threshold = 4096;
    int64_t long_segment = 512;
    int64_t force_vec_bytes = 0;
    int64_t csr_kernel = 0;
    int64_t coo_chunk = 512;
    int64_t coo_via_rowptr = 0;
    int64_t panel_mode = 0;
    int64_t panel_bytes = 4 << 20;
    int64_t panel_min_seg = 8;
    int64_t panel_block = 256;
    int64_t panel_lds_pad = 0;
    int64_t panel_coop = 512;
    int64_t panel_pack = 1;
    int64_t slice_group_bytes = 640ll << 20;
    int64_t vec_kernel = 1;
    int64_t vec_lds = 1;
    int64_t vec_lds_min_seg = 14;
    int64_t merge_parts = 1;
    int64_t narrow_vals = 1;
    int64_t split_unit_pattern = 1;
    int64_t panel_locality = 1;
    int64_t panel_col16 = 1;
    int64_t fuse_windows = 1;
    int64_t host_windows = 0;
    int64_t host_direct = 1;
    int64_t kernel_events = 0;
    int64_t lds_mode = 0;
    int64_t lds_min_reuse_x100 = 75;
    int64_t lds_min_width = 5;
    int64_t lds_min_width8 = 33;
    int64_t lds_min_reuse_narrow_x100 = 75;
    int64_t lds_threads = 0;
    int64_t lds_waves = 16;
    int64_t lds_long_slots = 128;
    int64_t lds_code = 1;
    int64_t lds_col_split = 0;
    int64_t lds_col_split_f32 = 1;
    int64_t lds_row_tail = 3;
    int64_t lds_half_split = 1;
    int64_t lds_direct_x = 1;
    int64_t lds_split_order = 1;
    int64_t lds_fill_tiles = 1;
    int64_t lds_code_nbuf = 0;
    int64_t lds_code_waves = 0;
    int64_t lds_code_kc = 0;
    int64_t lds_code_gsize = 0;
    int64_t lds_code_nsets = 0;
    int64_t lds_round_tiles = 1;
    int64_t lds_tile_order = 2;
    int64_t lds_lp_rounds = 12;
    int64_t lds_codegen = 1;
    int64_t lds_xcd_slices = 0;
    int64_t lds_code_boundary = 0;
    int64_t lds_code_exp = 0;
    int64_t lds_hybrid = 1;
    int64_t lds_hybrid_contig = 1;
    int64_t lds_hybrid_min = 128;
    int64_t lds_stamp = 0;
    int64_t lds_fail = 0;
    int64_t lds_ablate = 0;
} g_tune;

struct LongPlan {
    uint32_t n_long = 0, n_tasks = 0, thresh = 0;
    uint32_t *d_tasks = nullptr;
    uint32_t *d_desc = nullptr;
};

struct Part {
    int64_t nrows = 0, ncols = 0, nnz = 0;
    uint32_t *rowptr = nullptr;
    uint32_t *rowind = nullptr;
    uint32_t *colind = nullptr;
    void *vals = nullptr;
    void *vals_narrow = nullptr;
    bool own_rowptr = false, own_rowind = false, own_colind = false, own_vals = false;
    LongPlan lp_base, lp_panel;
    uint32_t *d_items = nullptr;
    size_t n_items = 0;
    std::vector<size_t> panel_off;
    std::vector<uint32_t> panel_coop;
    uint32_t npanels = 0, panel_cols = 0;
    unsigned short *col16 = nullptr;
    std::vector<uint32_t> panel_long128;
    std::vector<uint64_t> panel_nnz;
    SpmvUnit *d_spmv_units = nullptr;
    uint32_t n_spmv_units = 0;
    std::vector<int64_t> dense_cols;
    std::unique_ptr<Part> extra;
    std::unique_ptr<Part> hy_dense, hy_sparse;
    bool lds_forced = false;
    bool lds_contig_tiles = false;
    uint32_t *lds_col_order = nullptr;
    std::string hy_note;
    uint32_t *lds_tok = nullptr, *lds_nb = nullptr, *lds_chunks = nullptr, *lds_rowmap = nullptr;
    LdsTile *lds_tiles = nullptr;
    int cols_sorted = -1;
    uint32_t lds_ntiles = 0, lds_nw = 8, lds_batch = 8, lds_wdelta = 0;
    char *lds_code = nullptr;
    uint64_t *lds_code_start = nullptr;
    uint64_t lds_code_bytes = 0, lds_code_pairs = 0;
    uint32_t lds_rows = 0;
    uint32_t lds_half = 0;
    uint32_t *lds_tail_segs = nullptr;
    uint32_t *lds_tail_rowseg = nullptr;
    uint32_t lds_tail_nseg = 0;
    uint32_t lds_col_splits = 1;
    uint32_t lds_code_piece = 0;
    uint32_t lds_kc = 0, lds_nbuf = 0;
    uint32_t lds_row_bytes = 256, lds_ka = 0;
    uint32_t lds_code_gsize = 0, lds_code_nsets = 0;
    uint64_t lds_code_shared = 0;
    std::string lds_note;
    bool lds_codegen_device = false;
    bool panel_locality_used = false;
    int sim_kind = -1;
    std::vector<uint32_t> sim_order;
    uint32_t sim_labels = 0, sim_largest = 0;
    double sim_agree = 0.0;
    std::string sim_why;
    uint32_t lds_tile_labels = 0, lds_tile_largest = 0;
    std::string lds_codegen_why;
    bool lds_is_code = false;
    uint64_t lds_slots = 0, lds_tokens = 0;
    bool is_extra = false;
    bool no_pack = false;
    bool timed = false;
};

struct Group {
    int format = 0, dtype = 0;
    int64_t h = 0, total_rows = 0, total_cols = 0;
    std::vector<Part> parts;
    std::unique_ptr<Part> merged;
    bool all_ones = true;
    void *scratch = nullptr;
    size_t scratch_bytes = 0;
    void *stage_in = nullptr;
    size_t stage_in_bytes = 0;
    void *stage_out = nullptr;
    size_t stage_out_bytes = 0;
    void *xq = nullptr;
    size_t xq_bytes = 0;
    void *oq = nullptr;
    size_t oq_bytes = 0;
    const void *packed_src = nullptr;
    void *packed_buf = nullptr;
    int64_t packed_ld = 0, packed_w = 0;
    bool x_unchanged = false;
    int64_t serial = 0;
    int64_t lds_runs = 0;
    const void *pre_xs = nullptr;
    float *deq_out = nullptr;
    int64_t deq_ld = 0;
    const uint32_t *deq_amax = nullptr;
    int deq_log2 = 0;
    const float *post_mul = nullptr, *post_add = nullptr;
    int post_relu = 0;
    void **h_ptrs = nullptr;
    size_t h_ptrs_n = 0;
    hipEvent_t ev_ptrs[2] = {nullptr, nullptr};
    int ptr_slot = 0;
    void *xcat = nullptr;
    size_t xcat_bytes = 0;
    void **d_ptrs = nullptr;
    size_t d_ptrs_n = 0;
    int *d_flags = nullptr;
    hipStream_t side = nullptr;
    hipEvent_t ev_fork = nullptr, ev_join = nullptr;
    hipStream_t pipe_up = nullptr, pipe_down = nullptr;
    std::vector<hipEvent_t> pipe_ev;
    int64_t host_windows_used = 0;
    int64_t host_direct_used = 0;
    bool host_copies_slow = false;
    double timers[5] = {0, 0, 0, 0, 0};
    std::vector<std::pair<hipEvent_t, hipEvent_t>> ev_pending;
    bool kernel_events = false;
    double ev_ms = 0;
    int64_t ev_count = 0;
};

struct Context {
    bool inited = false;
    int device = 0;
    int cu_count = 0;
    int64_t nr_ranks = 0;
    std::set<Group *> groups;
    std::mutex mu;
    struct XsBuf {
        void *ptr = nullptr;
// ... 152 lines not shown
        }
        return HSA_STATUS_SUCCESS;
    }, &fp);
    if (!fp.found) return nullptr;
    ep.agent = f.agent;
    ep.pool = fp.pool;
    ep.ok = true;
    return &ep;
}
static void *exec_alloc(size_t bytes, std::string *why = nullptr) {
    auto say = [&](const char *m) { if (why) *why = m; };
    int dev = 0;
    if (hipGetDevice(&dev) != hipSuccess) { say("no current HIP device"); return nullptr; }
    ExecPool *ep;
    {
        std::lock_guard<std::mutex> lk(g_ctx.mu);
        ep = exec_pool_locked(dev);
    }
    if (!ep) { say("the HSA runtime offers no executable device memory pool"); return nullptr; }
    void *ptr = nullptr;
    if (hsa_amd_memory_pool_allocate(ep->pool, bytes, HSA_AMD_MEMORY_POOL_EXECUTABLE_FLAG, &ptr) != HSA_STATUS_SUCCESS) {
        say("the executable pool could not allocate the code");
        return nullptr;
    }
    return ptr;
}
static void *exec_alloc_upload(const void *host, size_t bytes, std::string *why = nullptr) {
    auto say = [&](const char *m) { if (why) *why = m; };
    const size_t piece = std::min<size_t>(bytes, (size_t)64 << 20);
    void *ptr = exec_alloc(bytes, why), *stage = nullptr;
    if (!ptr) return nullptr;
    if (hipMalloc(&stage, std::max<size_t>(piece, 256)) != hipSuccess) {
        (void)hipGetLastError();
        (void)hsa_amd_memory_pool_free(ptr);
        say("out of device memory for the staging buffer of the code upload");
        return nullptr;
    }
    bool ok = true;
    for (size_t off = 0; off < bytes && ok; off += piece) {
        const size_t nb = std::min(piece, bytes - off);
        ok = hipMemcpy(stage, (const char *)host + off, nb, hipMemcpyHostToDevice) == hipSuccess;
        const uint64_t n16 = nb / 16;
        if (ok && n16) {
            hipLaunchKernelGGL(k_copy16, dim3((unsigned)((n16 + 255) / 256)), dim3(256), 0, 0, (const u32x4_t *)stage, (u32x4_t *)((char *)ptr + off), n16);
            ok = hipGetLastError() == hipSuccess && hipDeviceSynchronize() == hipSuccess;
        }
    }
    (void)hipFree(stage);
    if (!ok) {
        (void)hsa_amd_memory_pool_free(ptr);
        say("copying the code to the device failed");
        return nullptr;
    }
    return ptr;
}

void free_part(Part &p) {
    if (p.own_rowptr && p.rowptr) (void)hipFree(p.rowptr);
    if (p.own_rowind && p.rowind) (void)hipFree(p.rowind);
    if (p.own_colind && p.colind) (void)hipFree(p.colind);
    if (p.own_vals && p.vals) (void)hipFree(p.vals);
    if (p.vals_narrow) (void)hipFree(p.vals_narrow);
    p.vals_narrow = nullptr;
    for (LongPlan *lp : {&p.lp_base, &p.lp_panel}) {
        if (lp->d_tasks) (void)hipFree(lp->d_tasks);
        if (lp->d_desc) (void)hipFree(lp->d_desc);
    }
    if (p.d_items) (void)hipFree(p.d_items);
    if (p.col16) (void)hipFree(p.col16);
    if (p.d_spmv_units) (void)hipFree(p.d_spmv_units);
    for (void *q : {(void *)p.lds_tok, (void *)p.lds_nb, (void *)p.lds_chunks, (void *)p.lds_rowmap, (void *)p.lds_tiles})
        if (q) (void)hipFree(q);
    p.lds_tok = p.lds_nb = p.lds_chunks = p.lds_rowmap = nullptr;
    p.lds_tiles = nullptr;
    if (p.lds_code) (void)hsa_amd_memory_pool_free(p.lds_code);
    if (p.lds_code_start) (void)hipFree(p.lds_code_start);
    p.lds_code = nullptr;
    p.lds_code_start = nullptr;
    p.lds_is_code = false;
    p.lds_row_bytes = 256;
    p.lds_col_splits = 1;
    p.lds_rows = 0;
    p.lds_half = 0;
    if (p.lds_tail_segs) (void)hipFree(p.lds_tail_segs);
    if (p.lds_tail_rowseg) (void)hipFree(p.lds_tail_rowseg);
    p.lds_tail_segs = p.lds_tail_rowseg = nullptr;
    p.lds_tail_nseg = 0;
    if (p.extra) free_part(*p.extra);
    if (p.hy_dense) free_part(*p.hy_dense);
    if (p.hy_sparse) free_part(*p.hy_sparse);
    if (p.lds_col_order) {
        std::lock_guard<std::mutex> lk(g_ctx.mu);
        for (auto &kv : g_ctx.xs_bufs)
            if (kv.second.order == (const void *)p.lds_col_order) { kv.second.src = nullptr; kv.second.order = nullptr; }
        (void)hipFree(p.lds_col_order);
    }
    p.lds_col_order = nullptr;
}

void free_group(Group *g) {
    for (auto &p : g->parts) free_part(p);
    if (g->merged) free_part(*g->merged);
    if (g->scratch) (void)hipFree(g->scratch);
    if (g->stage_in) (void)hipFree(g->stage_in);
    if (g->stage_out) (void)hipFree(g->stage_out);
    if (g->xcat) (void)hipFree(g->xcat);
    if (g->xq) (void)hipFree(g->xq);
    if (g->oq) (void)hipFree(g->oq);
    if (g->d_ptrs) (void)hipFree(g->d_ptrs);
    if (g->h_ptrs) (void)hipHostFree(g->h_ptrs);
    for (hipEvent_t e : g->ev_ptrs)
        if (e) (void)hipEventDestroy(e);
    if (g->d_flags) (void)hipFree(g->d_flags);
    if (g->side) (void)hipStreamDestroy(g->side);
    for (hipEvent_t e : g->pipe_ev)
        if (e) (void)hipEventDestroy(e);
    if (g->ev_fork) (void)hipEventDestroy(g->ev_fork);
    if (g->ev_join) (void)hipEventDestroy(g->ev_join);
    for (auto &e : g->ev_pending) {
        (void)hipEventDestroy(e.first);
        (void)hipEventDestroy(e.second);
    }
    delete g;
}

Group *lookup(int64_t handle) {
    Group *g = reinterpret_cast<Group *>(static_cast<uintptr_t>(handle));
    std::lock_guard<std::mutex> lk(g_ctx.mu);
    return g_ctx.groups.count(g) ? g : nullptr;
}
```

Measured before the change: 28740.

## Fill LDS chunks directly from row-major X to skip slice-major packing

```diff
diff --git a/include/pygim_hip.h b/include/pygim_hip.h
--- a/include/pygim_hip.h
+++ b/include/pygim_hip.h
@@ -109,6 +109,7 @@
 int pygim_group_lds_runs(int64_t handle, int64_t *out);
 int pygim_group_host_windows(int64_t handle, int64_t *windows, int64_t *direct);
 int pygim_group_lds_geometry(int64_t handle, int64_t out[8]);
+int pygim_group_lds_rowmajor(int64_t handle, int64_t out[2]);
 int pygim_group_lds_note(int64_t handle, char *out, int64_t cap);
 int64_t pygim_set_tunable(const char *name, int64_t value);
 
diff --git a/pygim_amd/_lib.py b/pygim_amd/_lib.py
--- a/pygim_amd/_lib.py
+++ b/pygim_amd/_lib.py
@@ -11,7 +11,7 @@
     "pygim_group_info", "pygim_set_tunable", "pygim_group_kernel_ms", "pygim_quant_spmm_run",
     "pygim_quant_absmax", "pygim_quantize", "pygim_dequantize", "pygim_spmm_run_group_x", "pygim_block_run_x",
     "pygim_group_kernel_events", "pygim_group_plan", "pygim_spmm_run_dequant",
-    "pygim_quant_spmm_run_post", "pygim_generation", "pygim_group_lds_plan", "pygim_group_lds_code", "pygim_group_lds_geometry", "pygim_group_lds_note",
+    "pygim_quant_spmm_run_post", "pygim_generation", "pygim_group_lds_plan", "pygim_group_lds_code", "pygim_group_lds_geometry", "pygim_group_lds_rowmajor", "pygim_group_lds_note",
     "pygim_group_lds_tiles", "pygim_group_lds_runs", "pygim_group_serial", "pygim_group_host_windows",
     "pygim_group_create_transposed", "pygim_sddmm",
     "pygim_spmm_values", "pygim_spmm_values_workspace", "pygim_edge_softmax", "pygim_edge_softmax_workspace", "pygim_edge_softmax_backward",
@@ -85,6 +85,7 @@
         L.pygim_group_lds_plan.argtypes = [c_i64, p_i64]
         L.pygim_group_lds_code.argtypes = [c_i64, p_i64]
         L.pygim_group_lds_geometry.argtypes = [c_i64, p_i64]
+        L.pygim_group_lds_rowmajor.argtypes = [c_i64, p_i64]
         L.pygim_group_lds_note.argtypes = [c_i64, ctypes.c_char_p, c_i64]
         L.pygim_group_lds_tiles.argtypes = [c_i64, p_i64]
         L.pygim_group_lds_runs.argtypes = [c_i64, p_i64]
@@ -322,7 +323,12 @@
 def group_lds_geometry(handle):
     out = (ctypes.c_int64 * 8)()
     check(lib().pygim_group_lds_geometry(int(handle), out))
-    return dict(zip(["waves", "acc_per_wave", "chunk_cols", "buffers", "group", "x_sets", "shared_entries", "col_splits"], [int(v) for v in out]))
+    geo = dict(zip(["waves", "acc_per_wave", "chunk_cols", "buffers", "group", "x_sets", "shared_entries", "col_splits"], [int(v) for v in out]))
+    rm = (ctypes.c_int64 * 2)()
+    check(lib().pygim_group_lds_rowmajor(int(handle), rm))
+    geo["rowmajor_x"] = int(rm[0])
+    geo["rowmajor_last"] = int(rm[1])
+    return geo
 
 
 def group_lds_note(handle):
diff --git a/pygim_amd/autotune.py b/pygim_amd/autotune.py
--- a/pygim_amd/autotune.py
+++ b/pygim_amd/autotune.py
@@ -17,6 +17,8 @@
 LDS_NS_PER_ENTRY_HALF = 0.5
 LDS_NS_PER_COLUMN_FLOOR = 4.4
 LDS_COL_SPLIT = True
+LDS_ROWMAJOR_X = True
+LDS_NS_PER_COLUMN_ROWMAJOR = 0.6
 LDS_ROW_TAIL = 3
 TAIL_S = 30e-6
 LDS_MIN_LANES = 5
@@ -82,6 +84,9 @@
             tall = tall2
         per_wg = max(cols_x / split * LDS_NS_PER_COLUMN + nnz / tall / split * ns_entry, cols_x / split * LDS_NS_PER_COLUMN_FLOOR) * 1e-9
         reduce_s = (split + 1) * nrows * h * es / RATE_STREAM
+        if LDS_ROWMAJOR_X and cols_x == ncols and (h * es) % 256 == 0:
+            pack_s = 0.0
+            per_wg += cols_x / split * LDS_NS_PER_COLUMN_ROWMAJOR * 1e-9
         return per_wg + reduce_s + pack_s + 2 * LAUNCH + (TAIL_S if tail_rows else 0.0)
     rpt = lds_rows_per_tile(int(nrows), nsl)
     tiles = -(-int(nrows) // rpt)
diff --git a/pygim_amd/csrc/kernels.hpp b/pygim_amd/csrc/kernels.hpp
--- a/pygim_amd/csrc/kernels.hpp
+++ b/pygim_amd/csrc/kernels.hpp
@@ -827,7 +827,7 @@
 constexpr uint32_t LDS_TAIL_SEG = 256;
 template <typename T>
 __global__ __launch_bounds__(512) void k_lds_tail_seg(const uint32_t *__restrict__ segs, uint32_t nseg, const uint32_t *__restrict__ colind, const char *__restrict__ xs,
-                                                      uint64_t slice_stride, typename AccOf<T>::type *__restrict__ parked) {
+                                                      uint64_t slice_stride, uint64_t row_stride, typename AccOf<T>::type *__restrict__ parked) {
     static_assert(sizeof(T) == 4, "4-byte element types");
     using A = typename AccOf<T>::type;
     __shared__ A partial[8][64];
@@ -844,7 +844,7 @@
     }
     T x[32];
 #pragma unroll
-    for (int k = 0; k < 32; k++) x[k] = cols[k] != 0xFFFFFFFFu ? *(const T *)(xsl + (uint64_t)cols[k] * 256) : (T)0;
+    for (int k = 0; k < 32; k++) x[k] = cols[k] != 0xFFFFFFFFu ? *(const T *)(xsl + (uint64_t)cols[k] * row_stride) : (T)0;
     A acc = 0;
 #pragma unroll
     for (int k = 0; k < 32; k++) acc = (A)(acc + to_acc<T>(x[k]));
diff --git a/pygim_amd/csrc/lds_codegen.hpp b/pygim_amd/csrc/lds_codegen.hpp
--- a/pygim_amd/csrc/lds_codegen.hpp
+++ b/pygim_amd/csrc/lds_codegen.hpp
@@ -29,6 +29,7 @@
     uint32_t half_H = 0;
     uint32_t x0 = 6, acc0 = 28, vbase0 = 1, vbase1 = 2, vbase2 = 3, vl16 = 4, vtouch = 4, vjunk = 5;
     uint32_t s_xs = 80, s_ldsw = 82, s_cb = 84, s_ret = 86, s_pa = 92;
+    uint32_t rowmajor = 0, v_rm = 0, s_ck = 88, s_step = 89;
     PYGIM_HD uint32_t vbase(uint32_t blk) const { return blk == 0 ? vbase0 : blk == 1 ? vbase1 : vbase2; }
 };
 
@@ -61,6 +62,9 @@
     if ((geo.half_split != 0) != (half_H != 0)) throw std::runtime_error("lds codegen: a half-split plan names its H (and only such a plan does)");
     if (half_H && (valued || wide || half_H % geo.KC || ncols != half_H)) throw std::runtime_error("lds codegen: half-split plans are unit-weight plans of 4-byte types over H = whole chunks of virtual columns");
     P.half_H = half_H;
+    if (geo.rowmajor && (geo.NW != 8 || wide || half_H || valued || opcode_add != 0x02000000u))
+        throw std::runtime_error("lds codegen: the row-major chunk fill serves unit-weight FLT32 plans of the 8-wave geometry");
+    P.rowmajor = geo.rowmajor ? 1 : 0; P.v_rm = R.v_rm; P.s_ck = R.s_ck; P.s_step = R.s_step;
     P.nrows = nrows; P.ncols = ncols;
     P.nchunks = (ncols + geo.KC - 1) / geo.KC;
     const uint32_t R_rows = geo.rows_per_tile ? std::min(geo.rows_per_tile, geo.NW * geo.KA) : geo.NW * geo.KA;
@@ -351,7 +355,9 @@
         e.since_touch = 0;
         e.vm_touch++;
     };
-    auto dma = [&](uint32_t cid, uint32_t buf) {
+    auto dma = [&](uint32_t cid, uint32_t buf) -> uint32_t {
+        if (P.rowmajor)
+            return lds_emit_dma_rowmajor(e, P.s_pa, P.s_xs, P.s_ldsw, P.s_ck, P.s_step, P.v_rm, P.pieces, P.chunk_bytes, P.ncols, P.KC, P.NW, cid, buf, s % P.NW);
         s_add_lit(P.s_pa, P.s_xs, cid * P.chunk_bytes);
         s_addc0(P.s_pa + 1, P.s_xs + 1);
         for (uint32_t i = 0; i < P.pieces; i++) {
@@ -365,14 +371,14 @@
             }
             e.op(0xDDF48000u | ((i % 4) * 1024), (P.s_pa << 16) | P.vl16);
         }
+        return P.pieces;
     };
     uint64_t dma_issued = 0;
     uint64_t landed_mark[16];
     for (int q = 0; q < 16; q++) landed_mark[q] = 0;
     auto vm_now = [&]() { return dma_issued + e.vm_touch; };
     auto dma_chunk = [&](uint32_t j) {
-        dma(chunk_ids[j], j % P.NBUF);
-        dma_issued += P.pieces;
+        dma_issued += dma(chunk_ids[j], j % P.NBUF);
         landed_mark[j & 15] = vm_now();
     };
     auto wait_landed = [&](uint32_t j) {
diff --git a/pygim_amd/csrc/lds_plan.hpp b/pygim_amd/csrc/lds_plan.hpp
--- a/pygim_amd/csrc/lds_plan.hpp
+++ b/pygim_amd/csrc/lds_plan.hpp
@@ -44,12 +44,13 @@
     uint32_t row_bytes = 256;
     uint32_t boundary = 0;
     uint32_t half_split = 0;
+    uint32_t rowmajor = 0;
     uint32_t NBUF = 2;
 };
 
 struct LdsPlanHost {
     LdsGeometry geo;
-    uint32_t ntiles = 0, nchunks = 0;
+    uint32_t ntiles = 0, nchunks = 0, ncols = 0;
     uint64_t ntokens = 0;
     uint64_t slots = 0;
     std::vector<uint32_t> tok;
@@ -121,6 +122,7 @@
     out.geo = geo;
     out.ntiles = ntiles;
     out.nchunks = nchunks;
+    out.ncols = ncols;
     out.tiles.assign(ntiles, LdsTile());
     out.rowmap.assign((size_t)ntiles * RS, 0xFFFFFFFFu);
 
@@ -290,6 +292,9 @@
     uint32_t s_ret = 86;
     uint32_t s_pa = 92;
     uint32_t wide = 0;
+    uint32_t v_rm = 0;
+    uint32_t s_ck = 88;
+    uint32_t s_step = 89;
     constexpr uint32_t nx() const { return gsize * nsets * (wide ? 2 : 1); }
 };
 constexpr LdsCodeRegs lds_code_regs(uint32_t NW, uint32_t gsize = 0, uint32_t nsets = 0, bool wide = false) {
@@ -315,6 +320,45 @@
 constexpr uint32_t LDS_CODE_AUTO_WAVES = 8, LDS_CODE8_AUTO_NBUF = 5;
 constexpr uint32_t LDS_CODE8_KA64 = 114;
 constexpr uint32_t LDS_CODE8_KA = 228;
+
+PYGIM_LDS_HD_INLINE uint32_t lds_rm_piece_rows(uint32_t ncols, uint32_t KC, uint32_t NW, uint32_t cid, uint32_t wave, uint32_t piece) {
+    const uint64_t r0 = (uint64_t)cid * KC + (uint64_t)wave * (KC / NW) + (uint64_t)piece * 4;
+    return r0 >= ncols ? 0u : (ncols - r0 < 4 ? (uint32_t)(ncols - r0) : 4u);
+}
+template <typename E>
+PYGIM_LDS_HD_INLINE uint32_t lds_emit_dma_rowmajor(E &e, uint32_t s_pa, uint32_t s_xs, uint32_t s_ldsw, uint32_t s_ck, uint32_t s_step, uint32_t v_rm, uint32_t pieces,
+                                                   uint32_t chunk_bytes, uint32_t ncols, uint32_t KC, uint32_t NW, uint32_t cid, uint32_t buf, uint32_t wave) {
+    e.op(0x96000000u | ((s_pa + 1) << 16) | (0xFFu << 8) | s_ck, cid);
+    e.op(0x92000000u | (s_pa << 16) | (0xFFu << 8) | s_ck, cid);
+    e.op(0x80000000u | (s_pa << 16) | (s_xs << 8) | s_pa);
+    e.op(0x82000000u | ((s_pa + 1) << 16) | ((s_xs + 1) << 8) | (s_pa + 1));
+    uint32_t issued = 0;
+    bool masked = false;
+    for (uint32_t i = 0; i < pieces; i++) {
+        const uint32_t rows = lds_rm_piece_rows(ncols, KC, NW, cid, wave, i);
+        if (!rows) break;
+        if (i) {
+            e.op(0x80000000u | (s_pa << 16) | (s_step << 8) | s_pa);
+            e.op(0x82000000u | ((s_pa + 1) << 16) | (0x80u << 8) | (s_pa + 1));
+            if (i % 4 == 0) {
+                e.op(0x80000000u | (s_pa << 16) | (0xFFu << 8) | s_pa, 0x1000u);
+                e.op(0x82000000u | ((s_pa + 1) << 16) | (0x80u << 8) | (s_pa + 1));
+            }
+        }
+        if (i % 4 == 0) {
+            e.op(0x80000000u | (124u << 16) | (0xFFu << 8) | s_ldsw, buf * chunk_bytes + (i / 4) * 0x1000u);
+            e.op(0xBF800000u);
+        }
+        if (rows < 4) {
+            e.op(0x91800000u | (126u << 16) | (128u << 8) | (128u + 16u * rows));
+            masked = true;
+        }
+        e.op(0xDDF48000u | ((i % 4) * 1024), (s_pa << 16) | v_rm);
+        issued++;
+    }
+    if (masked) e.op(0xBEFE01C1u);
+    return issued;
+}
 
 struct LdsWords {
     std::unique_ptr<uint32_t[]> p;
@@ -362,6 +406,8 @@
     const uint32_t G = R.gsize, NS = R.nsets;
     if (R.x0 + R.nx() > R.acc0 || R.acc0 + KA * (wide ? 2 : 1) > 256 || G > 12 || (NS - 1) * G > 15)
         throw std::runtime_error("lds code: the geometry does not fit the register map");
+    if (geo.rowmajor && (NW != 8 || wide || geo.half_split || !plan.wts.empty() || opcode_add != 0x02000000u || experiment))
+        throw std::runtime_error("lds code: the row-major chunk fill serves unit-weight FLT32 plans of the 8-wave geometry");
     const uint32_t pieces = (KC * RB / 1024) / NW;
     if (pieces * NW * 1024 != KC * RB) throw std::runtime_error("lds code: a chunk is not a whole number of pieces per wave");
     const uint32_t chunk_bytes = KC * RB;
@@ -410,7 +456,9 @@
             e.since_touch = 0;
             e.vm_touch++;
         };
-        auto dma = [&](uint32_t cid, uint32_t buf) {
+        auto dma = [&](uint32_t cid, uint32_t buf) -> uint32_t {
+            if (geo.rowmajor)
+                return lds_emit_dma_rowmajor(e, Rr.s_pa, Rr.s_xs, Rr.s_ldsw, Rr.s_ck, Rr.s_step, Rr.v_rm, pieces, chunk_bytes, plan.ncols, KC, NW, cid, buf, wv);
             s_add_lit(Rr.s_pa, Rr.s_xs, cid * chunk_bytes);
             s_addc0(Rr.s_pa + 1, Rr.s_xs + 1);
             for (uint32_t i = 0; i < pieces; i++) {
@@ -424,6 +472,7 @@
                 }
                 if (!(experiment & 2)) e.op(0xDDF48000u | ((i % 4) * 1024), (Rr.s_pa << 16) | Rr.vl16);
             }
+            return (experiment & 2) ? 0u : pieces;
         };
         uint64_t at = (uint64_t)t.tokstart[wv] * B;
         const uint32_t NBUF = geo.NBUF;
@@ -432,8 +481,7 @@
         auto vm_now = [&]() { return dma_issued + e.vm_touch; };
         std::vector<uint64_t> landed_mark(t.nch + NBUF + 1, 0);
         auto dma_chunk = [&](uint32_t j) {
-            dma(plan.chunks[t.chunk_off + j], j % NBUF);
-            dma_issued += (experiment & 2) ? 0 : pieces;
+            dma_issued += dma(plan.chunks[t.chunk_off + j], j % NBUF);
             landed_mark[j] = vm_now();
         };
         const bool spread = (experiment & 4) && pieces <= 4 && !mid;
diff --git a/pygim_amd/csrc/pygim_hip.hip b/pygim_amd/csrc/pygim_hip.hip
--- a/pygim_amd/csrc/pygim_hip.hip
+++ b/pygim_amd/csrc/pygim_hip.hip
@@ -179,6 +179,7 @@
     else if (n == "lds_split_order") slot = &g_tune.lds_split_order;
     else if (n == "lds_half_split") slot = &g_tune.lds_half_split;
     else if (n == "lds_direct_x") slot = &g_tune.lds_direct_x;
+    else if (n == "lds_rowmajor_x") slot = &g_tune.lds_rowmajor_x;
     else if (n == "lds_long_slots") slot = &g_tune.lds_long_slots;
     if (!slot) {
         fail(PYGIM_ERR_INVALID, "unknown tunable: " + n);
@@ -884,6 +885,15 @@
     return 0;
 }
 
+int pygim_group_lds_rowmajor(int64_t handle, int64_t out[2]) {
+    Group *g = lookup(handle);
+    if (!g || !out) return fail(PYGIM_ERR_INVALID, "unknown group handle");
+    const Part &p = (g->merged && g_tune.merge_parts && g->parts.size() > 1) ? *g->merged : g->parts[0];
+    out[0] = (p.lds_tiles && p.lds_rowmajor) ? 1 : 0;
+    out[1] = p.lds_tiles ? p.lds_rm_last : 0;
+    return 0;
+}
+
 int pygim_group_lds_note(int64_t handle, char *out, int64_t cap) {
     Group *g = lookup(handle);
     if (!g) return fail(PYGIM_ERR_INVALID, "unknown group handle");
diff --git a/pygim_amd/csrc/rt_launch.inc b/pygim_amd/csrc/rt_launch.inc
--- a/pygim_amd/csrc/rt_launch.inc
+++ b/pygim_amd/csrc/rt_launch.inc
@@ -271,6 +271,26 @@
     KernelTimer kt(g, st, !p.is_extra || p.timed);
     XsPin pin;
     void *xs_use = const_cast<void *>(lds_xs);
+    uint32_t x_row_bytes = 0;
+    uint64_t x_slice_stride = rows_pad * ROWB;
+    if (p.lds_rowmajor) {
+        const uint64_t ldxb = (uint64_t)ldx * sizeof(T);
+        x_row_bytes = 256;
+        if (!xs_use && X && sizeof(T) == 4 && !HS && ((uintptr_t)X & 15) == 0 && (ldxb & 15) == 0 && ((uint64_t)w * sizeof(T)) % 256 == 0 && (uint64_t)w <= (uint64_t)ldx &&
+            ldxb * (uint64_t)p.lds_kc < (1ull << 32)) {
+            xs_use = const_cast<void *>((const void *)X);
+            x_row_bytes = (uint32_t)ldxb;
+            x_slice_stride = 256;
+            p.lds_rm_last = 1;
+        } else {
+            if (p.lds_rm_last != 2) {
+                const std::string why = "; row-major chunk fill not used by the last product (X staged by the caller, not 16-byte aligned, or rows that are not whole slices at a "
+                                        "stride of whole 16 bytes): it streamed the slice-major copy";
+                if (p.lds_note.find(why) == std::string::npos) p.lds_note += why;
+            }
+            p.lds_rm_last = 2;
+        }
+    }
     if (!xs_use && g_tune.lds_direct_x && nslices == 1 && !HS && !WIDE8 && !p.lds_col_order && (size_t)ldx * sizeof(T) == ROWB && (size_t)w * sizeof(T) == ROWB &&
         ((uintptr_t)X & 255) == 0) {
         void *base = nullptr;
@@ -340,7 +360,8 @@
     a.rowmap = p.lds_rowmap;
     a.xs = (const char *)xs_use;
     a.c = (char *)C;
-    a.slice_stride = rows_pad * ROWB;
+    a.slice_stride = x_slice_stride;
+    a.x_row_bytes = x_row_bytes;
     a.ldc_bytes = (uint32_t)((size_t)ldc * (((WIDE8 || sizeof(T) == 2) && deq_amax) ? 4 : sizeof(T)));
     a.w = w_lanes;
     a.nslices = nslices;
@@ -502,7 +523,7 @@
             A *parked = (A *)((char *)g->scratch + split_bytes);
             if (p.lds_tail_nseg > 0)
                 hipLaunchKernelGGL((k_lds_tail_seg<T>), dim3(p.lds_tail_nseg, nslices), dim3(512), 0, st, p.lds_tail_segs, p.lds_tail_nseg, p.colind, (const char *)xs_use,
-                                   (uint64_t)(rows_pad * ROWB), parked);
+                                   x_slice_stride, (uint64_t)(x_row_bytes ? x_row_bytes : 256u), parked);
             const int64_t ldc_b = (int64_t)ldc * 4;
             if (deq_amax)
                 hipLaunchKernelGGL((k_lds_tail_fin<T, true>), dim3(ntail, nslices), dim3(64), 0, st, p.lds_tail_rowseg, (uint32_t)lds_rows, parked, w, (void *)C, ldc_b, 0, deq_amax,
diff --git a/pygim_amd/csrc/rt_plans.inc b/pygim_amd/csrc/rt_plans.inc
--- a/pygim_amd/csrc/rt_plans.inc
+++ b/pygim_amd/csrc/rt_plans.inc
@@ -231,6 +231,8 @@
                                                   : std::string("token form of the LDS-staged kernel")) : "no LDS-staged plan (rule, type or width): the L2 sweep serves this group";
     if (p.lds_tiles && p.lds_half)
         p.lds_note += "; half-split plan: two column ranges of " + std::to_string(p.lds_half) + " columns in the two halves of a wave (a row's sum = the sum of its ranges' sums)";
+    if (p.lds_tiles && p.lds_rowmajor)
+        p.lds_note += "; row-major chunk fill: products read X in place (no slice-major copy) when X is 16-byte aligned with rows of whole 16 bytes that hold their slices";
     if (p.lds_tiles && p.lds_rows)
         p.lds_note += "; the plan's tiles hold the first " + std::to_string(p.lds_rows) + " of " + std::to_string(p.nrows) + " rows (one workgroup per compute unit), k_lds_tail the others";
     if (p.lds_tiles && p.lds_col_splits > 1 && t_plan_dtype == PYGIM_FLT32)
@@ -488,6 +490,8 @@
         geo.rows_per_tile = lds_rows_per_tile((uint32_t)p.nrows, geo.NW * geo.KA, (uint32_t)nsl_hint, (uint32_t)std::max(g_ctx.cu_count, 1));
     const bool f32_split_ok = g_tune.lds_col_split_f32 == 1 ? p.nnz >= (1 << 20) : g_tune.lds_col_split_f32 != 0;
     uint32_t rows_lds = (uint32_t)p.nrows;
+    const bool rm_ok = want_code && g_tune.lds_rowmajor_x == 1 && t_plan_dtype == PYGIM_FLT32 && es == 4 && geo.NW == 8 && !p.vals && !p.lds_col_order && !p.lds_forced &&
+                       !g_tune.lds_code_exp && g_tune.lds_code_boundary != 2;
     if (g_tune.lds_col_split != 1 && (geo.NW == 16 || want_code) && !el8_code && (t_plan_dtype != PYGIM_FLT32 || f32_split_ok) && !p.vals) {
         const uint32_t cus = (uint32_t)std::max(g_ctx.cu_count, 1);
         const uint64_t nsl = h_hint > 0 ? (uint64_t)nsl_hint : 1;
@@ -532,6 +536,7 @@
         half_H = (uint32_t)(((((uint64_t)p.ncols + 1) / 2 + geo.KC - 1) / geo.KC) * geo.KC);
         geo.half_split = 1;
     }
+    if (rm_ok && geo.col_splits > 1 && !half) geo.rowmajor = 1;
     const bool narrow_hint = es != 8 && lanes_hint > 0 && lanes_hint <= 32;
     const double min_reuse_x100 = !narrow_hint ? (double)g_tune.lds_min_reuse_x100
                                                : std::max((double)g_tune.lds_min_reuse_x100, (double)g_tune.lds_min_reuse_narrow_x100 * (half ? 1.6 : 1.0));
@@ -620,6 +625,7 @@
             p.lds_codegen_device = true;
             p.lds_rows = rows_lds < (uint32_t)p.nrows ? rows_lds : 0;
             p.lds_half = half ? half_H : 0;
+            p.lds_rowmajor = geo.rowmajor != 0;
             lap("code stream generated on the device");
             return build_tail_segments(p, h_rowptr);
         }
@@ -742,6 +748,7 @@
     p.lds_col_splits = geo.col_splits;
     p.lds_rows = rows_lds < (uint32_t)p.nrows ? rows_lds : 0;
     p.lds_half = half ? half_H : 0;
+    p.lds_rowmajor = want_code && geo.rowmajor != 0;
     p.lds_kc = geo.KC;
     p.lds_nbuf = geo.NBUF;
     p.lds_row_bytes = geo.row_bytes;
diff --git a/pygim_amd/csrc/rt_state.inc b/pygim_amd/csrc/rt_state.inc
--- a/pygim_amd/csrc/rt_state.inc
+++ b/pygim_amd/csrc/rt_state.inc
@@ -65,6 +65,7 @@
     int64_t lds_row_tail = 3;
     int64_t lds_half_split = 1;
     int64_t lds_direct_x = 1;
+    int64_t lds_rowmajor_x = 1;
     int64_t lds_split_order = 1;
     int64_t lds_fill_tiles = 1;
     int64_t lds_code_nbuf = 0;
@@ -132,6 +133,8 @@
     uint32_t *lds_tail_rowseg = nullptr;
     uint32_t lds_tail_nseg = 0;
     uint32_t lds_col_splits = 1;
+    bool lds_rowmajor = false;
+    int lds_rm_last = 0;
     uint32_t lds_code_piece = 0;
     uint32_t lds_kc = 0, lds_nbuf = 0;
     uint32_t lds_row_bytes = 256, lds_ka = 0;
@@ -450,6 +453,8 @@
     p.lds_col_splits = 1;
     p.lds_rows = 0;
     p.lds_half = 0;
+    p.lds_rowmajor = false;
+    p.lds_rm_last = 0;
     if (p.lds_tail_segs) (void)hipFree(p.lds_tail_segs);
     if (p.lds_tail_rowseg) (void)hipFree(p.lds_tail_rowseg);
     p.lds_tail_segs = p.lds_tail_rowseg = nullptr;
```

New measurement: 28750, median of 3. About the same (+0.0%).
